# luvk1412/RoaringBitmap

Hardware: AMD Instinct MI355X
Metric: wide-OR/pairwise-AND input GB/s + % of HBM peak at 1/2/4/8 MI355X (higher is better)
Workload: dtype u64; 1 GPU; C2: RoaringBitmap.and(x1, x2), two full 2^32-universe bitmaps of 65536 mixed array/bitmap/run containers each (configs[1]); per_rank=the whole pair, parallelism=key-range sharding over 1 GPU(s)

## Files before the change

roaringbitmap_amd/csrc/engine.cpp:

```cpp
#include <hip/hip_runtime.h>

#include <algorithm>
#include <atomic>
#include <cstdio>
#include <cstdlib>
#include <cstring>
#include <initializer_list>
#include <memory>
#include <mutex>
#include <string>
#include <thread>
#include <chrono>
#include <unordered_map>
#include <vector>

#include <sys/mman.h>

#include "engine.hpp"
#include "format.hpp"

namespace rbg {

static thread_local std::string g_err;
void set_err(const std::string& s) { g_err = s; }

static bool debug_sync() {
  static int v = -1;
  if (v < 0) {
    const char* e = std::getenv("RBG_DEBUG_SYNC");
    v = (e && e[0] == '1') ? 1 : 0;
  }
  return v == 1;
}
void dbg(hipStream_t s, const char* what) {
  if (!debug_sync()) return;
  static auto last = std::chrono::steady_clock::now();
  hipError_t e = hipStreamSynchronize(s);
  const auto now = std::chrono::steady_clock::now();
  std::fprintf(stderr, "[rbg] %s done: %s (+%.3f ms)\n", what, hipGetErrorString(e),
               std::chrono::duration<double, std::milli>(now - last).count());
  last = now;
  std::fflush(stderr);
}

static size_t ro_flags_off(size_t groups) { return (64 + 32 * groups + 255) & ~(size_t)255; }

static std::mutex g_ctx_mu;
static std::vector<Ctx*> g_ctxs;

Ctx::~Ctx() {
  {
    std::lock_guard<std::mutex> g(g_ctx_mu);
    g_ctxs.erase(std::remove(g_ctxs.begin(), g_ctxs.end(), this), g_ctxs.end());
  }
  prof_free();
  if (pinned) (void)hipHostFree(pinned);
  batches.clear();
  if (stream) (void)hipStreamDestroy(stream);
}

size_t pool_clear(Ctx* c) {
  std::lock_guard<std::mutex> g(c->pool_mu);
  const size_t n = c->pool.size();
  c->pool.clear();
  c->pool_bytes = 0;
  return n;
}

static thread_local Ctx* t_cur_ctx = nullptr;
static std::atomic<uint64_t> g_pool_evictions{0};

static size_t release_pools_on(int device, int stage) {
  std::lock_guard<std::mutex> g(g_ctx_mu);
  size_t n = 0;
  const bool own = t_cur_ctx && std::find(g_ctxs.begin(), g_ctxs.end(), t_cur_ctx) != g_ctxs.end();
  if (stage == 0) {
    if (own && t_cur_ctx->device == device) n = pool_clear(t_cur_ctx);
  } else {
    for (Ctx* c : g_ctxs)
      if (c->device == device && !(own && c == t_cur_ctx)) n += pool_clear(c);
  }
  g_pool_evictions += n;
  return n;
}

int DevBuf::ensure(size_t bytes) {
  if (cap >= bytes && p) return RBG_OK;
  if (p) (void)hipFree(p);
  p = nullptr;
  cap = 0;
  hipError_t e = hipMalloc(&p, bytes + kSlack);
  if (e == hipErrorOutOfMemory) {
    int dev = 0;
    (void)hipGetLastError();
    for (int stage = 0; stage < 2 && e == hipErrorOutOfMemory; stage++) {
      if (hipGetDevice(&dev) != hipSuccess) break;
      if (release_pools_on(dev, stage) > 0) {
        e = hipMalloc(&p, bytes + kSlack);
        if (e == hipErrorOutOfMemory) (void)hipGetLastError();
      }
    }
  }
  if (e != hipSuccess) {
    p = nullptr;
    set_err(std::string("hipMalloc(") + std::to_string(bytes) + ") failed: " + hipGetErrorString(e));
    return e == hipErrorOutOfMemory ? RBG_ERR_OUT_OF_MEMORY : RBG_ERR_DEVICE;
  }
  cap = bytes;
  return RBG_OK;
}

int enter(Ctx* c) {
  t_cur_ctx = c;
  HIPCHK(hipSetDevice(c->device));
  return RBG_OK;
}

int ctx_init(Ctx* c, int device) {
  int n = 0;
  HIPCHK(hipGetDeviceCount(&n));
  if (device < 0 || device >= n) {
    set_err("no HIP device " + std::to_string(device));
    return RBG_ERR_DEVICE;
  }
  HIPCHK(hipSetDevice(device));
  hipDeviceProp_t prop;
  HIPCHK(hipGetDeviceProperties(&prop, device));
  if (std::strncmp(prop.gcnArchName, "gfx950", 6) != 0) {
    set_err(std::string("engine is built for gfx950, device is ") + prop.gcnArchName);
    return RBG_ERR_DEVICE;
  }
  c->device = device;
  {
    std::lock_guard<std::mutex> g(g_ctx_mu);
    g_ctxs.push_back(c);
  }
  HIPCHK(hipStreamCreateWithFlags(&c->stream, hipStreamNonBlocking));
  CHK(c->by_key.ensure(sizeof(PTask) * kMaxKeys));
  CHK(c->flag.ensure(kMaxKeys));
  CHK(c->tasks.ensure(sizeof(PTask) * (kMaxKeys + 32768)));
  CHK(c->ntasks.ensure(64));
  CHK(c->wg_count.ensure(4 * 256));
  CHK(c->wg_epoch.ensure(8 * 256));
  HIPCHK(hipMemset(c->wg_epoch.p, 0, 8 * 256));
  CHK(c->lb.ensure(kLbHeader + 8 * (kMaxKeys + 2 * kMaxTiles + kMaxAggTiles)));
  CHK(c->recs.ensure(sizeof(ORec) * kMaxKeys));
  CHK(c->kind_by_out.ensure(kMaxKeys));
  CHK(c->scalar.ensure(64));
  CHK(c->info.ensure(sizeof(ResultInfo)));
  CHK(c->task_card.ensure(4 * kMaxKeys));
  return RBG_OK;
}

int pinned_ensure(Ctx* c, size_t bytes) {
  if (c->pinned_cap >= bytes) return RBG_OK;
  if (c->pinned) (void)hipHostFree(c->pinned);
  c->pinned = nullptr;
  c->pinned_cap = 0;
  HIPCHK(hipHostMalloc(&c->pinned, bytes, hipHostMallocDefault));
  c->pinned_cap = bytes;
  return RBG_OK;
}

static uint32_t next_epoch(Ctx* c) {
  if (++c->epoch == 0) ++c->epoch;
  return c->epoch;
}
static PlanOut plan_out(Ctx* c, bool compacts = true) {
  return PlanOut{c->wg_epoch.as<uint64_t>(), compacts ? next_epoch(c) : 0, c->tasks.as<PTask>(),
                 c->ntasks.as<uint32_t>(), c->zlb, c->ztile};
}

int find_batch(Ctx* c, int32_t id, Batch** out) {
  if (id < 0 || (size_t)id >= c->batches.size() || !c->batches[id] || !c->batches[id]->live) {
    set_err("invalid batch id " + std::to_string(id));
    return RBG_ERR_ILLEGAL_ARGUMENT;
  }
  *out = c->batches[id].get();
  return RBG_OK;
}

static int ensure_stats(Ctx* c, Batch* b) {
  if (!b->stats_pending) return RBG_OK;
  const size_t n = b->n_bm, g = b->ro_groups, foff = ro_flags_off(g);
  uint32_t* flags = reinterpret_cast<uint32_t*>(b->ro_stats.as<uint8_t>() + foff);
  if (n) {
    HIPCHK(hipMemsetAsync(flags, 0, 4 * n, c->stream));
    launch_runopt_flags(c->stream, b->desc.as<CDesc>(), b->bm.as<uint32_t>(), b->n_ctr, flags);
  }
  std::vector<unsigned long long> hs(8 + 4 * g);
  std::vector<uint32_t> hf(n);
  HIPCHK(hipMemcpyAsync(hs.data(), b->ro_stats.p, 8 * hs.size(), hipMemcpyDeviceToHost, c->stream));
  if (n) HIPCHK(hipMemcpyAsync(hf.data(), flags, 4 * n, hipMemcpyDeviceToHost, c->stream));
  HIPCHK(hipStreamSynchronize(c->stream));
  b->stats_pending = false;
  unsigned long long h[4] = {0, 0, 0, 0};
  for (size_t w = 0; w < g; w++)
    for (int k = 0; k < 4; k++) h[k] += hs[8 + 4 * w + k];
  for (int k = 0; k < 3; k++) b->n_kind[k] = (int64_t)h[k];
  int64_t ser = (int64_t)h[3];
  b->h_has_run.assign(n, 0);
  for (size_t i = 0; i < n; i++) {
    const size_t nc = b->h_bm_nctr.empty() ? 0 : b->h_bm_nctr[i];
    ser += (int64_t)header_size(nc, hf[i] != 0);
    b->h_has_run[i] = hf[i] != 0;
  }
  if (b->ser_bytes) b->ser_bytes = ser;
  return RBG_OK;
}

int get_batch(Ctx* c, int32_t id, Batch** out) {
  CHK(find_batch(c, id, out));
  return ensure_stats(c, *out);
}

int32_t new_batch(Ctx* c) {
  for (size_t i = 0; i < c->batches.size(); i++)
    if (!c->batches[i]) {
      c->batches[i].reset(new Batch());
      return (int32_t)i;
    }
  c->batches.emplace_back(new Batch());
  return (int32_t)(c->batches.size() - 1);
}

constexpr size_t kPoolMax = 2ull << 30;
constexpr size_t kPoolMaxBuf = 1ull << 30;

void pool_put(Ctx* c, DevBuf& b) {
  if (!b.p) return;
  std::lock_guard<std::mutex> g(c->pool_mu);
  if (b.cap > kPoolMaxBuf) {
    b = DevBuf();
    return;
  }
  while (!c->pool.empty() && c->pool_bytes + b.cap > kPoolMax) {
    c->pool_bytes -= c->pool.front().cap;
    c->pool.erase(c->pool.begin());
  }
  c->pool_bytes += b.cap;
  c->pool.push_back(std::move(b));
}

int pool_take(Ctx* c, DevBuf& dst, size_t bytes) {
  if (dst.p && dst.cap >= bytes) return RBG_OK;
  std::unique_lock<std::mutex> lk(c->pool_mu);
  size_t best = c->pool.size();
  for (size_t i = 0; i < c->pool.size(); i++) {
    const size_t cap = c->pool[i].cap;
    if (cap >= bytes && cap <= 2 * bytes + (1u << 20) && (best == c->pool.size() || cap < c->pool[best].cap))
      best = i;
  }
  if (best == c->pool.size()) {
    lk.unlock();
    return dst.ensure(bytes);
  }
  c->pool_bytes -= c->pool[best].cap;
  dst = std::move(c->pool[best]);
  c->pool.erase(c->pool.begin() + (std::ptrdiff_t)best);
  return RBG_OK;
}

static uint64_t header_reserve(size_t max_tasks) {
  return round16(8 + (max_tasks + 7) / 8 + 8 * (uint64_t)max_tasks + 16);
}

int grid_for(size_t tasks, size_t cap) {
  size_t g = std::min(tasks, cap);
  return (int)std::max<size_t>(g, 1);
}

int prepare_output(Ctx* c, size_t max_tasks, size_t max_payload, OutCtx* oc, bool card_only) {
  uint8_t* lb = c->lb.as<uint8_t>();
  *oc = OutCtx{};
  oc->err = reinterpret_cast<uint32_t*>(lb + 64);
  oc->status = reinterpret_cast<uint64_t*>(lb + kLbHeader);
  oc->tile_status = reinterpret_cast<uint64_t*>(lb + kLbHeader + 8 * kMaxKeys);
  oc->tile_card = reinterpret_cast<uint64_t*>(lb + kLbHeader + 8 * (kMaxKeys + kMaxTiles));
  oc->recs = c->recs.as<ORec>();
  c->serialized = false;
  c->place_pending = false;
  c->agg_ok = false;
  c->ri_valid = false;
  c->pending_ub = 0;
  c->zlb = c->ztile = nullptr;
  c->pending_src.clear();
  if (card_only) {
    c->zlb = reinterpret_cast<uint64_t*>(lb);
    return RBG_OK;
  }
  const uint64_t P0 = header_reserve(max_tasks);
  CHK(c->result.ensure(P0 + max_payload + 64));
  c->result_cap = P0 + max_payload;
  CHK(c->scratch.ensure((size_t)kSlotBytes * std::max<size_t>(max_tasks, 1) + 64));
  c->zlb = reinterpret_cast<uint64_t*>(lb);
  c->ztile = reinterpret_cast<uint64_t*>(lb + kLbHeader + 8 * kMaxKeys);
  oc->out = c->result.as<uint8_t>();
  oc->payload_base = P0;
  oc->scratch = c->scratch.as<uint8_t>();
  oc->kind_by_out = c->kind_by_out.as<uint8_t>();
  c->pending = *oc;
  c->pending_ub = max_tasks;
  return RBG_OK;
}

void defer_place(Ctx* c) {
  c->place_pending = true;
  c->last = 1;
}
int ensure_placed(Ctx* c) {
  if (!c->place_pending) return RBG_OK;
  launch_place(c->stream, c->ntasks.as<uint32_t>(), c->pending, c->info.as<ResultInfo>());
  HIPCHK(hipGetLastError());
  c->place_pending = false;
  return RBG_OK;
}

int ctx_serialize(Ctx* c) {
  if (c->last != 1) {
    set_err("no materialised result pending");
    return RBG_ERR_ILLEGAL_ARGUMENT;
  }
  if (c->serialized) return RBG_OK;
  if (c->place_pending && c->agg_ok && !c->pending.spec && c->pending_ub <= (size_t)kMaxAggTiles * kAggTile) {
    launch_serialize_agg(c->stream, c->ntasks.as<uint32_t>(), c->pending, c->info.as<ResultInfo>(), c->pending_ub);
    HIPCHK(hipGetLastError());
    c->place_pending = false;
    c->serialized = true;
    return RBG_OK;
  }
  CHK(ensure_placed(c));
  if (c->pending.spec) launch_spec_fix(c->stream, c->ntasks.as<uint32_t>(), c->pending);
  launch_serialize(c->stream, c->ntasks.as<uint32_t>(), c->pending);
  HIPCHK(hipGetLastError());
  c->serialized = true;
  return RBG_OK;
}

int resolve(Ctx* c, int32_t id, size_t i, Operand* op) {
  Batch* b;
  CHK(get_batch(c, id, &b));
  if (i >= b->n_bm) {
    set_err("bitmap index out of range");
    return RBG_ERR_ILLEGAL_ARGUMENT;
  }
  if (b->n_bm != 1 || !b->key_major || b->packed) {
    set_err("pairwise operands must be single-bitmap key-major batches with slot-aligned payloads");
    return RBG_ERR_ILLEGAL_ARGUMENT;
  }
  *op = Operand{{b->key_off.as<uint32_t>(), b->desc.as<CDesc>(), b->payload.as<uint8_t>(), (int)b->n_ctr}, b};
  return RBG_OK;
}

static void op_begin(Ctx* c, std::initializer_list<int32_t> src) {
  c->pending_src = src;
  c->mark(0);
  c->mark(1);
}
int op_end(Ctx* c) {
  c->mark(2);
  defer_place(c);
  c->mark(3);
  HIPCHK(hipGetLastError());
  return RBG_OK;
}

static int ctx_rankdir(Ctx* c, Batch* b) {
  if (b->rd_ready) return RBG_OK;
  const size_t n = b->n_ctr;
  hipStream_t s = c->stream;
  CHK(pool_take(c, b->rd_cum, 8 * (n + 1)));
  CHK(pool_take(c, b->rd_off, 8 * (n + 1)));
  CHK(c->rd_part.ensure(8 * (scan_parts(std::max<uint64_t>(n, 1)) + 1)));
  uint64_t* cum = b->rd_cum.as<uint64_t>();
  uint64_t* off = b->rd_off.as<uint64_t>();
  launch_rd_sizes(s, b->desc.as<CDesc>(), b->payload.as<uint8_t>(), n, cum, off);
  launch_exclusive_scan(s, cum, cum, n, c->rd_part.as<uint64_t>(), cum + n);
  launch_exclusive_scan(s, off, off, n, c->rd_part.as<uint64_t>(), off + n);
  HIPCHK(hipGetLastError());
  uint64_t aux_bytes = 0;
  HIPCHK(hipMemcpyAsync(&aux_bytes, off + n, 8, hipMemcpyDeviceToHost, s));
  HIPCHK(hipStreamSynchronize(s));
  CHK(pool_take(c, b->rd_aux, aux_bytes + 16));
  launch_rd_fill(s, b->desc.as<CDesc>(), b->payload.as<uint8_t>(), n, off, b->rd_aux.as<uint8_t>());
  HIPCHK(hipGetLastError());
  b->rd_ready = true;
  return RBG_OK;
}

int ctx_point(Ctx* c, int op, int32_t batch, size_t i, const uint32_t* q_dev, size_t n, long long* out_dev) {
  Operand o;
  CHK(resolve(c, batch, i, &o));
  Batch* B = o.b;
  CHK(ctx_rankdir(c, B));
  const PointArgs pa{B->key_off.as<uint32_t>(), o.desc, B->payload.as<uint8_t>(), B->rd_cum.as<uint64_t>(),
                     B->rd_off.as<uint64_t>(), B->rd_aux.as<uint8_t>(), (uint32_t)o.n};
  launch_point(c->stream, op, pa, q_dev, n, out_dev);
  HIPCHK(hipGetLastError());
  return RBG_OK;
}

int ctx_point_host(Ctx* c, int op, int32_t batch, size_t i, const uint32_t* q, size_t n, int64_t* out) {
  CHK(pinned_ensure(c, 12 * n + 64));
  CHK(c->pt_q.ensure(4 * n));
  CHK(c->pt_out.ensure(8 * n));
  uint8_t* pin = reinterpret_cast<uint8_t*>(c->pinned);
  hipStream_t s = c->stream;
  HIPCHK(hipStreamSynchronize(s));
  std::memcpy(pin + 8 * n, q, 4 * n);
  HIPCHK(hipMemcpyAsync(c->pt_q.p, pin + 8 * n, 4 * n, hipMemcpyHostToDevice, s));
  CHK(ctx_point(c, op, batch, i, c->pt_q.as<uint32_t>(), n, c->pt_out.as<long long>()));
  HIPCHK(hipMemcpyAsync(pin, c->pt_out.p, 8 * n, hipMemcpyDeviceToHost, s));
  HIPCHK(hipStreamSynchronize(s));
  std::memcpy(out, pin, 8 * n);
  return RBG_OK;
}

int ctx_to_values(Ctx* c, int32_t batch, size_t i, uint64_t first, uint64_t count, bool out64, void* out_dev,
                  uint64_t* n_out) {
  Operand o;
  CHK(resolve(c, batch, i, &o));
  Batch* B = o.b;
  const uint64_t card = (uint64_t)B->long_card;
  const uint64_t cnt = first < card ? std::min<uint64_t>(count, card - first) : 0;
  if (n_out) *n_out = cnt;
  if (!cnt || (!out_dev && n_out)) return RBG_OK;
  if (!out_dev) {
    set_err("to_values: no output buffer");
    return RBG_ERR_ILLEGAL_ARGUMENT;
  }
  CHK(ctx_rankdir(c, B));
  const PointArgs pa{B->key_off.as<uint32_t>(), o.desc, B->payload.as<uint8_t>(), B->rd_cum.as<uint64_t>(),
                     B->rd_off.as<uint64_t>(), B->rd_aux.as<uint8_t>(), (uint32_t)o.n};
  launch_to_values(c->stream, pa, first, cnt, out64, out_dev);
  HIPCHK(hipGetLastError());
  return RBG_OK;
}

// ... 158 lines not shown
  if (layout != RBG_BITS_PACKED && layout != RBG_BITS_BYTES) {
    set_err("bitset: unknown layout (RBG_BITS_PACKED or RBG_BITS_BYTES)");
    return RBG_ERR_ILLEGAL_ARGUMENT;
  }
  if (layout == RBG_BITS_PACKED && (first & 63)) {
    set_err("bitset: a packed window starts at a multiple of 64");
    return RBG_ERR_ILLEGAL_ARGUMENT;
  }
  if (first > kBitsetMaxBits || n > kBitsetMaxBits - first) {
    set_err("bitset: the window reaches past 2^32");
    return RBG_ERR_ILLEGAL_ARGUMENT;
  }
  return RBG_OK;
}

int ctx_from_bitset(Ctx* c, const void* bits_dev, uint64_t n, int layout, bool run_opt, int32_t* out_id) {
  if (!n) return build_batch(c, nullptr, 0, nullptr, 0, run_opt, out_id);
  if (layout == RBG_BITS_PACKED)
    return build_batch(c, nullptr, 0, reinterpret_cast<const uint8_t*>(bits_dev), n, run_opt, out_id);
  const uint64_t nbytes = 8 * ((n + 63) / 64);
  DevBuf words;
  CHK(pool_take(c, words, nbytes + 16));
  launch_bits_pack(c->stream, reinterpret_cast<const uint8_t*>(bits_dev), n, words.as<uint64_t>());
  HIPCHK(hipGetLastError());
  const int st = build_batch(c, nullptr, 0, words.as<uint8_t>(), nbytes, run_opt, out_id);
  pool_put(c, words);
  return st;
}

int ctx_from_bitset_host(Ctx* c, const void* bits, uint64_t n, int layout, bool run_opt, int32_t* out_id) {
  DevBuf in;
  CHK(pool_take(c, in, n + 16));
  CHK(upload_bytes(c, in.p, bits, n));
  const int st = ctx_from_bitset(c, in.p, n, layout, run_opt, out_id);
  pool_put(c, in);
  return st;
}

int ctx_to_bitset(Ctx* c, int32_t batch, size_t i, uint64_t first, uint64_t n, int layout, void* out_dev) {
  Operand o;
  CHK(resolve(c, batch, i, &o));
  if (!n) return RBG_OK;
  if (!out_dev || (layout == RBG_BITS_PACKED && (reinterpret_cast<uintptr_t>(out_dev) & 7))) {
    set_err("bitset: no output buffer, or packed words not 8-byte aligned");
    return RBG_ERR_ILLEGAL_ARGUMENT;
  }
  launch_bits_expand(c->stream, o.key_off, o.desc, o.payload, first, n, layout == RBG_BITS_BYTES, out_dev);
  HIPCHK(hipGetLastError());
  return RBG_OK;
}

int ctx_to_bitset_host(Ctx* c, int32_t batch, size_t i, uint64_t first, uint64_t n, int layout, void* out) {
  CHK(ctx_to_bitset(c, batch, i, first, 0, layout, nullptr));
  if (!n) return RBG_OK;
  if (!out) {
    set_err("bitset: no output buffer");
    return RBG_ERR_ILLEGAL_ARGUMENT;
  }
  const bool mask = layout == RBG_BITS_BYTES;
  const uint64_t window = mask ? 1ull << 28 : 1ull << 31;
  auto bytes_of = [&](uint64_t bits) { return mask ? bits : 8 * ((bits + 63) / 64); };
  CHK(c->tv_out.ensure(bytes_of(std::min(n, window))));
  for (uint64_t done = 0; done < n; done += window) {
    const uint64_t w = std::min(window, n - done);
    CHK(ctx_to_bitset(c, batch, i, first + done, w, layout, c->tv_out.p));
    HIPCHK(hipMemcpyAsync(reinterpret_cast<uint8_t*>(out) + bytes_of(done), c->tv_out.p, bytes_of(w),
                          hipMemcpyDeviceToHost, c->stream));
    HIPCHK(hipStreamSynchronize(c->stream));
  }
  return RBG_OK;
}

static int ctx_pairwise_buffer(Ctx* c, int op, int32_t ia, size_t ma, int32_t ib, size_t mb, int key_lo, int key_hi) {
  key_lo = std::max(0, key_lo);
  key_hi = std::min(kMaxKeys, key_hi);
  Operand A, B;
  CHK(resolve(c, ia, ma, &A));
  CHK(resolve(c, ib, mb, &B));
  hipStream_t s = c->stream;
  const size_t ub = std::max<size_t>(1, op == OP_AND ? (size_t)std::min(A.n, B.n) : (size_t)A.n);
  return with_big_runs(c, true, "buffer and / andNot", [&](const BigRuns& big) -> int {
    OutCtx oc;
    CHK(prepare_output(c, ub, A.b->payload_bytes + B.b->payload_bytes + kStagedMax * ub + big.cap, &oc, false));
    c->pending_src = {ia, ib};
    c->mark(0);
    const PlanOut po = plan_out(c);
    launch_plan_pairwise(s, op, key_lo, key_hi, A, B, po, oc.err);
    c->mark(1);
    launch_pair_buf(s, op, grid_for(ub, 65536), po.tasks, po.n_tasks, A.payload, B.payload, oc, big);
    return op_end(c);
  });
}

int ctx_ornot(Ctx* c, int32_t ia, size_t ma, int32_t ib, size_t mb, int64_t range_end, int flags) {
  if (range_end < 0 || range_end > (int64_t)0x100000000ll) {
    set_err("rangeEnd should be in [0, 0xffffffff + 1]");
    return RBG_ERR_ILLEGAL_ARGUMENT;
  }
  Operand A, B;
  CHK(resolve(c, ia, ma, &A));
  CHK(resolve(c, ib, mb, &B));
  const int max_key = range_end == 0 ? -1 : (int)((range_end - 1) >> 16);
  const int last_run = (range_end & 0xFFFF) == 0 ? 0x10000 : (int)(range_end & 0xFFFF);
  hipStream_t s = c->stream;
  const size_t ub = std::max<size_t>(1, std::min<size_t>(kMaxKeys, (size_t)(max_key + 1) + (size_t)A.n));
  if (!c->ornot_plan.p) CHK(c->ornot_plan.ensure(sizeof(OrNotPlan)));
  OutCtx oc;
  CHK(prepare_output(c, ub, A.b->payload_bytes + B.b->payload_bytes + kStagedMax * ub, &oc, false));
  op_begin(c, {ia, ib});
  launch_ornot(s, A, B, max_key, last_run, flags, c->ornot_plan.as<OrNotPlan>(), plan_out(c), oc,
               grid_for(ub, 65536));
  CHK(op_end(c));
  if (max_key < 0 && A.n == 0 && B.n > 0) {
    OrNotPlan pl;
    HIPCHK(hipMemcpyAsync(&pl, c->ornot_plan.p, sizeof(pl), hipMemcpyDeviceToHost, s));
    HIPCHK(hipStreamSynchronize(s));
    if (pl.neg) {
      c->last = 0;
      set_err("orNot: negative maxSize (the reference throws NegativeArraySizeException)");
      return RBG_ERR_ILLEGAL_ARGUMENT;
    }
  }
  return RBG_OK;
}

int check_range(int64_t start, int64_t end) {
  if (start < 0 || start > 0xFFFFFFFFll || end < 0 || end > 0x100000000ll) {
    set_err("rangeStart=" + std::to_string(start) + " should be in [0, 0xffffffff], rangeEnd=" + std::to_string(end) +
            " in [0, 0xffffffff + 1]");
    return RBG_ERR_ILLEGAL_ARGUMENT;
  }
  return RBG_OK;
}

static int run_rmut(Ctx* c, int32_t ia, const Operand& A, RmutArgs ra, bool buf, size_t ub, bool use_arena,
                    const char* what) {
  return with_big_runs(c, use_arena, what, [&](const BigRuns& big) -> int {
    OutCtx oc;
    CHK(prepare_output(c, ub, A.b->payload_bytes + kStagedMax * ub + big.cap, &oc, false));
    op_begin(c, {ia});
    launch_rmut(c->stream, A, ra, buf, plan_out(c), oc, big, grid_for(ub, 65536));
    return op_end(c);
  });
}

int ctx_range_mut(Ctx* c, int op, int32_t ia, size_t ma, int64_t start, int64_t end, bool buf) {
  if (op < RMUT_ADD || (op > RMUT_ADD_INPLACE && op != RMUT_RANGE)) return RBG_ERR_ILLEGAL_ARGUMENT;
  CHK(check_range(start, end));
  Operand A;
  CHK(resolve(c, ia, ma, &A));
  RmutArgs ra{op, 1, 0, 0, 0};
  if (end > start) {
    ra.hbs = (int)((uint64_t)start >> 16 & 0xFFFF);
    ra.lbs = (int)(start & 0xFFFF);
    ra.hbl = (int)((uint64_t)(end - 1) >> 16 & 0xFFFF);
    ra.lbl = (int)((end - 1) & 0xFFFF);
  }
  const size_t in_range = end > start ? (size_t)(ra.hbl - ra.hbs + 1) : 0;
  const size_t ub = std::max<size_t>(1, std::min<size_t>(kMaxKeys, (size_t)A.n + in_range));
  return run_rmut(c, ia, A, ra, buf, ub, true, "range add / remove");
}

int ctx_remove_run_compression(Ctx* c, int32_t ia, size_t ma) {
  Operand A;
  CHK(resolve(c, ia, ma, &A));
  return run_rmut(c, ia, A, RmutArgs{RMUT_DERUN, 1, 0, 0, 0}, false, std::max<size_t>(1, (size_t)A.n), false,
                  "removeRunCompression");
}

int ctx_limit(Ctx* c, int32_t ia, size_t ma, int cut_key, int leftover) {
  Operand A;
  CHK(resolve(c, ia, ma, &A));
  return run_rmut(c, ia, A, RmutArgs{RMUT_LIMIT, cut_key, leftover, 0, 0}, false, std::max<size_t>(1, (size_t)A.n),
                  true, "limit");
}

int ctx_add_offset(Ctx* c, int32_t ia, size_t ma, int64_t offset) {
  Operand A;
  CHK(resolve(c, ia, ma, &A));
  const int64_t co = offset < 0 ? (offset - 65535) / 65536 : offset / 65536;
  AoffArgs aa{0, 0, 1};
  if (co >= -65536 && co < 65536) aa = AoffArgs{(int)co, (int)(offset - co * 65536), 0};
  const size_t ub = std::max<size_t>(1, std::min<size_t>(kMaxKeys, 2 * (size_t)A.n));
  OutCtx oc;
  CHK(prepare_output(c, ub, A.b->payload_bytes + kStagedMax * ub, &oc, false));
  op_begin(c, {ia});
  launch_aoff(c->stream, A, aa, plan_out(c), oc, grid_for(ub, 65536));
  return op_end(c);
}

int ctx_pairwise(Ctx* c, int op, int32_t ia, size_t ma, int32_t ib, size_t mb, bool card_only, int key_lo,
                 int key_hi) {
  if (op == RBG_AND_BUFFER || op == RBG_ANDNOT_BUFFER) {
    if (card_only) return RBG_ERR_ILLEGAL_ARGUMENT;
    return ctx_pairwise_buffer(c, op == RBG_AND_BUFFER ? OP_AND : OP_ANDNOT, ia, ma, ib, mb, key_lo, key_hi);
  }
  if (op == RBG_OR_INPLACE && !card_only) {
    CHK(ctx_pairwise(c, OP_OR, ia, ma, ib, mb, false, key_lo, key_hi));
    if (!c->ones.p) {
      CHK(c->ones.ensure(8192));
      HIPCHK(hipMemsetAsync(c->ones.p, 0xFF, 8192, c->stream));
    }
    Operand A, B;
    CHK(resolve(c, ia, ma, &A));
    CHK(resolve(c, ib, mb, &B));
    launch_ior_fix(c->stream, c->ntasks.as<uint32_t>(), c->recs.as<ORec>(), A, B, c->ones.as<uint8_t>());
    HIPCHK(hipGetLastError());
    c->agg_ok = false;
    return RBG_OK;
  }
  if (op < 0 || op > 3) return RBG_ERR_ILLEGAL_ARGUMENT;
  key_lo = std::max(0, key_lo);
  key_hi = std::min(kMaxKeys, key_hi);
  Operand A, B;
  CHK(resolve(c, ia, ma, &A));
  CHK(resolve(c, ib, mb, &B));
  hipStream_t s = c->stream;
  const int plan_op = card_only ? OP_AND : op;
  size_t ub;
  switch (plan_op) {
    case OP_AND: ub = std::min(A.n, B.n); break;
    case OP_ANDNOT: ub = A.n; break;
    default: ub = std::min<size_t>((size_t)A.n + B.n, kMaxKeys); break;
  }
  const size_t nkeys = key_hi > key_lo ? (size_t)(key_hi - key_lo) : 0;
  const bool dense = nkeys > 0 && 2 * ub >= nkeys;
  OutCtx oc;
  CHK(prepare_output(c, dense ? std::max(ub, nkeys) : ub, A.b->payload_bytes + B.b->payload_bytes + kStagedMax * ub,
                     &oc, card_only));
  c->pending_src = {ia, ib};
  c->mark(0);
  const PwDirect pd{key_lo};
  const PlanOut po = plan_out(c, !dense);
  if (dense) {
    launch_plan_balanced(s, plan_op, card_only ? 1 : 0, key_lo, (uint32_t)nkeys, A, B, po, oc,
                         c->task_card.as<uint32_t>());
  } else {
    launch_plan_pairwise(s, plan_op, key_lo, key_hi, A, B, po, oc.err);
    dbg(s, "plan");
  }
  c->mark(1);
  if (!card_only) {
    oc.tile_agg = reinterpret_cast<unsigned long long*>(oc.tile_status + 2 * kMaxTiles);
    c->pending.tile_agg = oc.tile_agg;
    c->agg_ok = true;
  }
  const int grid = grid_for(((dense ? nkeys : ub) + 3) / 4, 16384);
  launch_pairwise(s, op, card_only ? 1 : 0, grid, po.tasks, po.n_tasks, A.payload, B.payload, oc,
                  c->task_card.as<uint32_t>(), dense ? &pd : nullptr);
  dbg(s, "pairwise");
  c->mark(2);
  if (card_only) {
    launch_reduce_card(s, c->task_card.as<uint32_t>(), c->ntasks.as<uint32_t>(), c->info.as<ResultInfo>(), oc.err);
    c->last = 2;
  } else {
    defer_place(c);
  }
  c->mark(3);
  HIPCHK(hipGetLastError());
  return RBG_OK;
}


int batch_host_index(Ctx* c, Batch* b) {
  if (b->h_index) return RBG_OK;
  HIPCHK(hipStreamSynchronize(c->stream));
  b->h_desc.resize(b->n_ctr);
  if (b->n_ctr) HIPCHK(hipMemcpy(b->h_desc.data(), b->desc.p, sizeof(CDesc) * b->n_ctr, hipMemcpyDeviceToHost));
  b->h_pos_off.assign(b->n_bm + 1, 0);
  b->h_pos.resize(b->n_ctr);
  if ((b->n_bm == 1 || !b->key_major) && b->h_bm_off.size() == b->n_bm + 1) {
    for (size_t i = 0; i <= b->n_bm; i++) b->h_pos_off[i] = b->h_bm_off[i];
    for (size_t p = 0; p < b->n_ctr; p++) b->h_pos[p] = (uint32_t)p;
  } else {
    std::vector<uint32_t> bm(b->n_ctr);
    if (b->n_ctr) HIPCHK(hipMemcpy(bm.data(), b->bm.p, 4 * b->n_ctr, hipMemcpyDeviceToHost));
    for (uint32_t x : bm) b->h_pos_off[x + 1]++;
    for (size_t i = 0; i < b->n_bm; i++) b->h_pos_off[i + 1] += b->h_pos_off[i];
    std::vector<uint32_t> fill(b->h_pos_off.begin(), b->h_pos_off.end() - 1);
    for (size_t p = 0; p < b->n_ctr; p++) b->h_pos[fill[bm[p]]++] = (uint32_t)p;
  }
  b->h_index = true;
  return RBG_OK;
}

int ctx_info(Ctx* c, ResultInfo* ri) {
  if (c->last == 1) CHK(ensure_placed(c));
  HIPCHK(hipMemcpyAsync(ri, c->info.p, sizeof(ResultInfo), hipMemcpyDeviceToHost, c->stream));
  uint64_t card = 0;
  uint32_t err = 0;
  if (c->last == 1)
    HIPCHK(hipMemcpyAsync(&card, c->lb.as<uint8_t>() + 64 + 8 * kCardWord, 8, hipMemcpyDeviceToHost, c->stream));
  if (c->last == 1 || c->last == 2)
    HIPCHK(hipMemcpyAsync(&err, c->lb.as<uint8_t>() + 64, 4, hipMemcpyDeviceToHost, c->stream));
  HIPCHK(hipStreamSynchronize(c->stream));
  if (c->last == 1) {
    ri->long_card = (int64_t)card;
    ri->card32 = (uint32_t)card;
  }
  ri->err |= err;
  if ((c->last == 1 || c->last == 2) && ri->err) {
    set_err("a look-back spin of the op's plan or placement timed out: the result is invalid");
    return RBG_ERR_DEVICE;
  }
  if (c->last == 1) {
    c->last_ri = *ri;
    c->ri_valid = true;
  }
  return RBG_OK;
}

static int download_staged(Ctx* c, const uint8_t* dev, uint64_t bytes, uint8_t* dst) {
  constexpr uint64_t kGroup = 32ull << 20;
  hipStream_t s = c->stream;
  if (bytes <= kGroup) {
    HIPCHK(hipMemcpyAsync(dst, dev, bytes, hipMemcpyDeviceToHost, s));
    HIPCHK(hipStreamSynchronize(s));
    return RBG_OK;
  }
  CHK(pinned_ensure(c, bytes + 64));
  uint8_t* pin = reinterpret_cast<uint8_t*>(c->pinned);
  const uint32_t groups = (uint32_t)((bytes + kGroup - 1) / kGroup);
  std::vector<hipEvent_t> ev(groups);
  for (auto& e : ev) HIPCHK(hipEventCreateWithFlags(&e, hipEventDisableTiming));
  int st = RBG_OK;
  for (uint32_t g = 0; g < groups; g++) {
    const uint64_t lo = (uint64_t)g * kGroup, hi = std::min<uint64_t>(bytes, lo + kGroup);
    if (hipMemcpyAsync(pin + lo, dev + lo, hi - lo, hipMemcpyDeviceToHost, s) != hipSuccess ||
        hipEventRecord(ev[g], s) != hipSuccess) {
      set_err("device-to-host copy of the result failed");
      st = RBG_ERR_DEVICE;
      break;
    }
  }
  if (st == RBG_OK) {
    std::atomic<uint32_t> next{0};
    std::atomic<int> bad{0};
    const int nthr = (int)std::min<unsigned>(8, std::max(1u, std::thread::hardware_concurrency()));
    std::vector<std::thread> th;
    for (int t = 0; t < nthr; t++)
      th.emplace_back([&]() {
        for (uint32_t g; (g = next.fetch_add(1)) < groups;) {
          if (hipEventSynchronize(ev[g]) != hipSuccess) {
            bad.store(1);
            continue;
          }
          const uint64_t lo = (uint64_t)g * kGroup, hi = std::min<uint64_t>(bytes, lo + kGroup);
          std::memcpy(dst + lo, pin + lo, hi - lo);
        }
      });
    for (auto& x : th) x.join();
    if (bad.load()) {
      set_err("device-to-host copy of the result failed");
      st = RBG_ERR_DEVICE;
    }
  }
  (void)hipStreamSynchronize(s);
  for (auto& e : ev) (void)hipEventDestroy(e);
  return st;
}

static std::mutex g_out_mu;
static std::unordered_map<void*, size_t> g_out_live;
static std::vector<std::pair<void*, size_t>> g_out_cache;
constexpr size_t kOutLarge = 8ull << 20, kOutCacheMax = 2, kOutCacheBytes = 1ull << 30, kOutAlign = 2ull << 20;
static size_t out_cache_bytes() {
  size_t b = 0;
  for (const auto& e : g_out_cache) b += e.second;
  return b;
}
uint8_t* out_alloc(size_t n) {
  if (n < kOutLarge) return (uint8_t*)std::malloc(n ? n : 1);
  std::lock_guard<std::mutex> g(g_out_mu);
  for (size_t i = 0; i < g_out_cache.size(); i++) {
    const auto e = g_out_cache[i];
    if (e.second >= n && e.second <= 2 * n + kOutAlign) {
      g_out_cache.erase(g_out_cache.begin() + (std::ptrdiff_t)i);
      g_out_live[e.first] = e.second;
      return (uint8_t*)e.first;
    }
  }
  const size_t cap = (n + kOutAlign - 1) & ~(kOutAlign - 1);
  void* p = nullptr;
  if (posix_memalign(&p, kOutAlign, cap) != 0) return nullptr;
  (void)madvise(p, cap, MADV_HUGEPAGE);
  g_out_live[p] = cap;
  return (uint8_t*)p;
}

int ctx_fetch(Ctx* c, rbg_buffer* out) {
  if (c->last != 1) {
    set_err("no serialized result pending");
    return RBG_ERR_ILLEGAL_ARGUMENT;
  }
  CHK(ctx_serialize(c));
  ResultInfo ri;
  CHK(ctx_info(c, &ri));
  uint8_t* p = out_alloc(ri.total);
  if (!p) return RBG_ERR_OUT_OF_MEMORY;
  out->data = p;
  out->len = ri.total;
  const int st = download_staged(c, c->result.as<uint8_t>() + ri.start, ri.total, p);
  if (st != RBG_OK) {
    rbg_free(out);
    return st;
  }
  return RBG_OK;
}

int ctx_batch_fetch_range(Ctx* c, int32_t batch, size_t i0, size_t i1, rbg_buffer* outs) {
  Batch* b;
  CHK(get_batch(c, batch, &b));
  if (i0 > i1 || i1 > b->n_bm || (i1 > i0 && !outs)) return RBG_ERR_ILLEGAL_ARGUMENT;
  CHK(batch_host_index(c, b));
  const std::vector<CDesc>& D = b->h_desc;
  auto slot_end = [&](uint32_t p) -> uint64_t { return p + 1 < b->n_ctr ? D[p + 1].slot : b->payload_bytes; };
  std::vector<GatherItem> items;
  uint64_t tot = 0;
  for (size_t i = i0; i < i1; i++)
    for (uint32_t k = b->h_pos_off[i]; k < b->h_pos_off[i + 1]; k++) {
      const uint32_t p = b->h_pos[k];
      const uint64_t len = slot_end(p) - D[p].slot;
      items.push_back(GatherItem{D[p].slot, tot, len});
      tot = round16(tot + len);
    }
  std::vector<uint8_t> pay(tot + 16);
  if (!items.empty()) {
    CHK(c->gather_items.ensure(sizeof(GatherItem) * items.size()));
    CHK(c->gather_out.ensure(tot + 16));
    HIPCHK(hipMemcpyAsync(c->gather_items.p, items.data(), sizeof(GatherItem) * items.size(), hipMemcpyHostToDevice,
                          c->stream));
    launch_gather(c->stream, c->gather_items.as<GatherItem>(), items.size(), b->payload.as<uint8_t>(),
                  c->gather_out.as<uint8_t>());
    HIPCHK(hipGetLastError());
    HIPCHK(hipMemcpyAsync(pay.data(), c->gather_out.p, tot, hipMemcpyDeviceToHost, c->stream));
    HIPCHK(hipStreamSynchronize(c->stream));
  }
  size_t it = 0;
  for (size_t i = i0; i < i1; i++) {
    const uint32_t k0 = b->h_pos_off[i], n = b->h_pos_off[i + 1] - k0;
    bool has_run = false;
    std::vector<uint32_t> lens(n);
    for (uint32_t k = 0; k < n; k++) {
      const CDesc& d = D[b->h_pos[k0 + k]];
      has_run |= d.kind == KR;
      if (d.kind == KA) lens[k] = 2 * d.card;
      else if (d.kind == KB) lens[k] = 8192;
      else {
        const uint8_t* q = pay.data() + items[it + k].dst + 2;
        lens[k] = 2 + 4 * (uint32_t)(q[0] | (q[1] << 8));
      }
    }
    std::vector<uint8_t> o;
    auto put16 = [&](uint32_t v) { o.push_back((uint8_t)v); o.push_back((uint8_t)(v >> 8)); };
    auto put32 = [&](uint32_t v) { for (int j = 0; j < 4; j++) o.push_back((uint8_t)(v >> (8 * j))); };
    if (has_run) {
      put32(12347u | (uint32_t)((n - 1) << 16));
      std::vector<uint8_t> fl((n + 7) / 8, 0);
      for (uint32_t k = 0; k < n; k++)
        if (D[b->h_pos[k0 + k]].kind == KR) fl[k / 8] |= (uint8_t)(1u << (k % 8));
      o.insert(o.end(), fl.begin(), fl.end());
    } else {
      put32(12346u);
      put32(n);
    }
    for (uint32_t k = 0; k < n; k++) {
      const CDesc& d = D[b->h_pos[k0 + k]];
      put16(d.key);
      put16(d.card - 1);
    }
    if (!has_run || n >= 4) {
      uint32_t start = (uint32_t)header_size(n, has_run);
      for (uint32_t k = 0; k < n; k++) {
        put32(start);
        start += lens[k];
      }
    }
    for (uint32_t k = 0; k < n; k++) {
      const uint8_t* q = pay.data() + items[it + k].dst + (D[b->h_pos[k0 + k]].kind == KR ? 2 : 0);
      o.insert(o.end(), q, q + lens[k]);
    }
    it += n;
    const int st = emit_host(o, &outs[i - i0]);
    if (st != RBG_OK) {
      for (size_t j = i0; j < i; j++) rbg_free(&outs[j - i0]);
      return st;
    }
  }
  return RBG_OK;
}

int ctx_batch_card(Ctx* c, int32_t id) {
  Batch* B;
  CHK(get_batch(c, id, &B));
  if (B->packed) {
    set_err("batched andCardinality needs slot-aligned payloads");
    return RBG_ERR_ILLEGAL_ARGUMENT;
  }
  if (B->n_bm % 2 != 0) {
    set_err("batched andCardinality needs an even number of bitmaps");
    return RBG_ERR_ILLEGAL_ARGUMENT;
  }
  const size_t np = B->n_bm / 2;
  CHK(c->cards.ensure(4 * std::max<size_t>(np, 1)));
  if (B->key_major && B->n_bm > 1) {
    set_err("batched andCardinality needs a bitmap-major batch");
    return RBG_ERR_ILLEGAL_ARGUMENT;
  }
  c->mark(0);
  c->mark(1);
  if (!B->pair_cap_known) {
    B->pair_items_cap = batch_pair_items_cap(B->h_bm_nctr.data(), np);
    B->pair_cap_known = true;
  }
  CHK(c->pc_cnt.ensure(8 * ((np + 255) / 256) + std::max<size_t>(np, 1) + 16));
  CHK(c->pc_part.ensure(8 * (scan_parts(std::max<size_t>(np, 1)) + 1)));
  CHK(c->pc_items.ensure(sizeof(PairItem) * std::max<uint64_t>(B->pair_items_cap, 1)));
  CHK(c->pc_large.ensure(4 * std::max<size_t>(np, 1)));
  CHK(c->scalar.ensure(64));
  launch_batch_and_card(c->stream, np, B->bm_off.as<uint32_t>(), B->keys.as<uint16_t>(), B->desc.as<CDesc>(),
                        B->payload.as<uint8_t>(), c->cards.as<int32_t>(), c->pc_cnt.as<uint64_t>(),
                        c->pc_part.as<uint64_t>(), c->scalar.as<uint64_t>() + 7, c->pc_items.as<PairItem>(),
                        c->pc_large.as<uint32_t>());
  c->mark(2);
  c->mark(3);
  HIPCHK(hipGetLastError());
  c->n_cards = np;
  c->last = 3;
  return RBG_OK;
}

int ctx_fetch_shard_device(Ctx* c, int64_t total_containers, int has_run, int64_t payload_base, void* desc_dst,
                           void* offsets_dst, void* runflag_dst, void* payload_dst) {
  if (c->last != 1) {
    set_err("no materialised result pending");
    return RBG_ERR_ILLEGAL_ARGUMENT;
  }
  if (total_containers < 0 || total_containers > kMaxKeys || payload_base < 0 || !desc_dst || !payload_dst) {
    set_err("fetch_shard: bad layout or null destination");
    return RBG_ERR_ILLEGAL_ARGUMENT;
  }
  const bool offsets = !has_run || total_containers >= 4;
  if (offsets && !offsets_dst) {
    set_err("fetch_shard: the global bitmap has an offset table; offsets_dst is required");
    return RBG_ERR_ILLEGAL_ARGUMENT;
  }
  ResultInfo ri;
  if (c->ri_valid) {
    ri = c->last_ri;
    CHK(ensure_placed(c));
  } else {
    CHK(ctx_info(c, &ri));
  }
  const uint64_t off0 = header_size((size_t)total_containers, has_run != 0) + (uint64_t)payload_base;
  if (off0 > 0xFFFFFFFFull) {
    set_err("fetch_shard: payload offsets exceed 32 bits");
    return RBG_ERR_ILLEGAL_ARGUMENT;
  }
  uint8_t* emit_dst = (uint8_t*)payload_dst;
  if (c->serialized) {
    if (ri.payload)
      HIPCHK(hipMemcpyAsync(payload_dst, c->result.as<uint8_t>() + c->pending.payload_base, ri.payload,
                            hipMemcpyDeviceToDevice, c->stream));
    emit_dst = nullptr;
  }
  launch_serialize_shard(c->stream, grid_for((c->pending_ub + 255) / 256, 256), c->ntasks.as<uint32_t>(), c->pending,
                         emit_dst, off0, (uint8_t*)desc_dst, offsets ? (uint8_t*)offsets_dst : nullptr,
                         has_run ? (uint8_t*)runflag_dst : nullptr);
  HIPCHK(hipGetLastError());
  return RBG_OK;
}


int ctx_run_optimize(Ctx* c, int32_t id, int32_t* out_id, uint8_t* answers) {
  Batch* a;
  CHK(get_batch(c, id, &a));
  if (a->packed) {
    set_err("runOptimize needs slot-aligned payloads (not a packed synthetic batch)");
    return RBG_ERR_ILLEGAL_ARGUMENT;
  }
  hipStream_t s = c->stream;
  const size_t C = a->n_ctr, n = a->n_bm;
  const int32_t bid = new_batch(c);
  Batch& b = *c->batches[bid];
  struct Drop {
    Ctx* c;
    int32_t id;
    bool keep = false;
    ~Drop() {
      if (!keep) c->batches[id].reset();
    }
  } drop{c, bid};
  CHK(pool_take(c, b.desc, sizeof(CDesc) * C + 16));
  CHK(pool_take(c, b.payload, a->payload_bytes + 64));
  b.ro_groups = runopt_groups(C);
  CHK(pool_take(c, b.ro_stats, ro_flags_off(b.ro_groups) + 4 * n + 16));
  CHK(pool_take(c, b.keys, a->keys.cap));
  CHK(pool_take(c, b.bm, a->bm.cap));
  CHK(pool_take(c, b.key_off, a->key_off.cap));
  CHK(pool_take(c, b.bm_off, a->bm_off.cap));
  const RoCopy cp{a->keys.as<uint16_t>(), b.keys.as<uint16_t>(), a->bm.as<uint32_t>(), b.bm.as<uint32_t>(),
                  a->key_off.as<uint32_t>(), b.key_off.as<uint32_t>(), a->key_off.cap / 4,
                  a->bm_off.as<uint32_t>(), b.bm_off.as<uint32_t>(), a->bm_off.cap / 4};
  if (C)
    launch_runopt(s, a->desc.as<CDesc>(), a->payload.as<uint8_t>(), C, b.desc.as<CDesc>(), b.payload.as<uint8_t>(), cp,
                  b.ro_stats.as<unsigned long long>() + 8);
  HIPCHK(hipGetLastError());
  b.n_bm = n;
  b.n_ctr = C;
  b.key_major = a->key_major;
  b.h_bm_off = a->h_bm_off;
  b.h_bm_nctr = a->h_bm_nctr;
  b.h_bm_card = a->h_bm_card;
  b.long_card = a->long_card;
  b.bsi_min = a->bsi_min;
  b.bsi_max = a->bsi_max;
  b.payload_bytes = a->payload_bytes;
  b.gapped = a->gapped || a->n_kind[DK_R] > 0;
  b.max_ser = 0;
  b.ser_bytes = a->ser_bytes ? 1 : 0;
  b.stats_pending = true;
  b.live = true;
  drop.keep = true;
  *out_id = bid;
  if (answers) {
    CHK(ensure_stats(c, &b));
    for (size_t i = 0; i < n; i++) answers[i] = b.h_has_run[i];
  }
  return RBG_OK;
}

int ctx_select_range(Ctx* c, int32_t id, int64_t start, int64_t end, int32_t* out_id, bool buf) {
  if (start < 0 || end < 0) {
    set_err("selectRange: rangeStart and rangeEnd must not be negative");
    return RBG_ERR_ILLEGAL_ARGUMENT;
  }
  if (end > start && ((uint64_t)start >> 16 & 0xFFFF) > ((uint64_t)(end - 1) >> 16 & 0xFFFF)) {
    set_err("selectRange: the range's key casts are out of order (the reference would build an unsorted bitmap)");
    return RBG_ERR_ILLEGAL_ARGUMENT;
  }
  Batch* a;
  CHK(get_batch(c, id, &a));
  if (!a->key_major || a->packed) {
    set_err("range selection needs a key-major batch with slot-aligned payloads");
    return RBG_ERR_ILLEGAL_ARGUMENT;
  }
  hipStream_t s = c->stream;
  const size_t C = a->n_ctr, n = a->n_bm;
  RselArgs ra{1, 0, 0, 0, buf ? 1 : 0};
  if (end > start) {
    ra.hbs = (int)((uint64_t)start >> 16 & 0xFFFF);
    ra.lbs = (int)(start & 0xFFFF);
    ra.hbl = (int)((uint64_t)(end - 1) >> 16 & 0xFFFF);
    ra.lbl = (int)((end - 1) & 0xFFFF);
  }
  CHK(c->ro_info.ensure(4 * C + 16));
  CHK(c->ro_size.ensure(8 * C + 16));
  CHK(c->ro_part.ensure(8 * (scan_parts(std::max<size_t>(C, 1)) + 1)));
  CHK(c->rs_card.ensure(4 * C + 16));
  CHK(c->rs_keep.ensure(8 * C + 16));
  CHK(c->rs_bm.ensure(16 * n + 64 + 16));
  const int32_t bid = new_batch(c);
  Batch& b = *c->batches[bid];
  BatchGuard guard{c, {bid}};
  CHK(pool_take(c, b.desc, sizeof(CDesc) * C + 16));
  CHK(pool_take(c, b.payload, a->payload_bytes + 64));
  CHK(b.keys.ensure(2 * C + 16));
  CHK(b.bm.ensure(4 * C + 16));
  CHK(b.key_off.ensure(4 * (kMaxKeys + 1)));
  CHK(b.bm_off.ensure(4 * (n + 1)));
  unsigned long long* bm_cnt = c->rs_bm.as<unsigned long long>();
  unsigned long long* bm_card = bm_cnt + n;
  unsigned long long* tot = bm_cnt + 2 * n;
  HIPCHK(hipMemsetAsync(c->rs_bm.p, 0, 16 * n + 64, s));
  launch_rsel_plan(s, a->desc.as<CDesc>(), a->bm.as<uint32_t>(), a->payload.as<uint8_t>(), C, ra,
                   c->ro_info.as<uint32_t>(), c->rs_card.as<uint32_t>(), c->ro_size.as<uint64_t>(),
                   c->rs_keep.as<uint64_t>(), bm_cnt, bm_card, tot);
  launch_exclusive_scan(s, c->ro_size.as<uint64_t>(), c->ro_size.as<uint64_t>(), C, c->ro_part.as<uint64_t>(),
                        reinterpret_cast<uint64_t*>(tot + 4));
  launch_exclusive_scan(s, c->rs_keep.as<uint64_t>(), c->rs_keep.as<uint64_t>(), C, c->ro_part.as<uint64_t>(),
                        reinterpret_cast<uint64_t*>(tot + 5));
  launch_rsel_write(s, a->desc.as<CDesc>(), a->bm.as<uint32_t>(), a->payload.as<uint8_t>(), C, ra,
                    c->ro_info.as<uint32_t>(), c->rs_card.as<uint32_t>(), c->ro_size.as<uint64_t>(),
                    c->rs_keep.as<uint64_t>(), b.desc.as<CDesc>(), b.keys.as<uint16_t>(), b.bm.as<uint32_t>(),
                    b.payload.as<uint8_t>());
  HIPCHK(hipGetLastError());
  std::vector<unsigned long long> h(2 * n + 8);
  HIPCHK(hipMemcpyAsync(h.data(), c->rs_bm.p, 8 * (2 * n + 6), hipMemcpyDeviceToHost, s));
  HIPCHK(hipStreamSynchronize(s));
  const unsigned long long* t = h.data() + 2 * n;
  const uint64_t C2 = t[5];
  launch_dec_key_off(s, b.keys.as<uint16_t>(), C2, b.key_off.as<uint32_t>());
  b.n_bm = n;
  b.n_ctr = C2;
  b.key_major = true;
  for (int k = 0; k < 3; k++) b.n_kind[k] = (int64_t)t[k];
  b.max_ser = t[3];
  b.payload_bytes = t[4];
  b.h_bm_off.assign(n + 1, 0);
  b.h_bm_nctr.resize(n);
  b.h_bm_card.resize(n);
  for (size_t i = 0; i < n; i++) {
    b.h_bm_nctr[i] = (uint32_t)h[i];
    b.h_bm_off[i + 1] = b.h_bm_off[i] + (uint32_t)h[i];
    b.h_bm_card[i] = (int64_t)h[n + i];
    b.long_card += (int64_t)h[n + i];
  }
  HIPCHK(hipMemcpyAsync(b.bm_off.p, b.h_bm_off.data(), 4 * (n + 1), hipMemcpyHostToDevice, s));
  HIPCHK(hipStreamSynchronize(s));
  HIPCHK(hipGetLastError());
  b.live = true;
  guard.ids.clear();
  *out_id = bid;
  return RBG_OK;
}

int ctx_profile(Ctx* c, int max_ops, bool compute_only) {
  HIPCHK(hipStreamSynchronize(c->stream));
  c->prof_free();
  c->prof_compute_only = compute_only;
  if (max_ops <= 0) return RBG_OK;
  c->prof_ev.resize(4 * (size_t)max_ops);
  for (hipEvent_t& e : c->prof_ev) HIPCHK(hipEventCreate(&e));
  c->prof_cap = (size_t)max_ops;
  c->prof_n = 0;
  CHK(c->rd_ctr.ensure(8));
  HIPCHK(hipMemsetAsync(c->rd_ctr.p, 0, 8, c->stream));
  return RBG_OK;
}

static std::mutex g_dev_mu;
static uint64_t g_dev_mask = 1;

struct TLCtx {
  std::unique_ptr<Ctx> ctx;
  int device = -1;
};
static thread_local TLCtx tl;

int tl_ctx(Ctx** out) {
  int dev;
  {
    std::lock_guard<std::mutex> g(g_dev_mu);
    uint64_t m = g_dev_mask;
    dev = m ? __builtin_ctzll(m) : 0;
  }
  if (!tl.ctx || tl.device != dev) {
    std::unique_ptr<Ctx> c(new Ctx());
    CHK(ctx_init(c.get(), dev));
    tl.ctx = std::move(c);
    tl.device = dev;
  }
  CHK(enter(tl.ctx.get()));
  *out = tl.ctx.get();
  return RBG_OK;
}

}

using namespace rbg;

extern "C" {

void rbg_trim(void) {
  std::lock_guard<std::mutex> g(g_out_mu);
  for (const auto& e : g_out_cache) std::free(e.first);
  g_out_cache.clear();
}

uint64_t rbg_pool_evictions(void) { return g_pool_evictions.load(); }
const char* rbg_last_error(void) { return g_err.c_str(); }

void rbg_free(rbg_buffer* buf) {
  if (!buf) return;
  if (buf->data) {
    std::lock_guard<std::mutex> g(g_out_mu);
    const auto it = g_out_live.find(buf->data);
    if (it != g_out_live.end()) {
      g_out_cache.emplace_back(it->first, it->second);
      g_out_live.erase(it);
      while (g_out_cache.size() > kOutCacheMax || (!g_out_cache.empty() && out_cache_bytes() > kOutCacheBytes)) {
        std::free(g_out_cache.front().first);
        g_out_cache.erase(g_out_cache.begin());
      }
      buf->data = nullptr;
      buf->len = 0;
      return;
    }
  }
  std::free(buf->data);
  buf->data = nullptr;
  buf->len = 0;
}

int rbg_set_devices(uint64_t mask) {
  int n = 0;
  if (hipGetDeviceCount(&n) != hipSuccess || n == 0) {
    set_err("no HIP device");
    return RBG_ERR_DEVICE;
  }
  uint64_t usable = mask & ((n >= 64) ? ~0ULL : ((1ULL << n) - 1));
// ... 11 lines not shown
```

roaringbitmap_amd/csrc/engine.hpp:

```cpp
#pragma once
#include <hip/hip_runtime.h>

#include <cstddef>
#include <cstdint>
#include <cstdlib>
#include <cstring>
#include <memory>
#include <mutex>
#include <string>
#include <vector>

#include "../../include/roaring_mi355x.h"
#include "kernels.hpp"

namespace rbg {

void set_err(const std::string& s);

#define HIPCHK(x)                                                            \
  do {                                                                       \
    hipError_t e_ = (x);                                                     \
    if (e_ != hipSuccess) {                                                  \
      set_err(std::string(#x) + " failed: " + hipGetErrorString(e_));        \
      return e_ == hipErrorOutOfMemory ? RBG_ERR_OUT_OF_MEMORY : RBG_ERR_DEVICE; \
// ... 6 lines not shown
    if (st_ != RBG_OK) return st_; \
  } while (0)

constexpr size_t kSlack = 256;
constexpr int kMaxKeys = 65536;
constexpr size_t kLbHeader = 256;
constexpr size_t kStagedMax = 8194;

struct DevBuf {
  void* p = nullptr;
  size_t cap = 0;
  DevBuf() = default;
  DevBuf(const DevBuf&) = delete;
  DevBuf& operator=(const DevBuf&) = delete;
  DevBuf(DevBuf&& o) noexcept : p(o.p), cap(o.cap) {
    o.p = nullptr;
    o.cap = 0;
  }
  DevBuf& operator=(DevBuf&& o) noexcept {
    if (this != &o) {
      if (p) (void)hipFree(p);
      p = o.p;
      cap = o.cap;
      o.p = nullptr;
      o.cap = 0;
    }
    return *this;
  }
  ~DevBuf() {
    if (p) (void)hipFree(p);
  }
  int ensure(size_t bytes);
  template <class T>
  T* as() const {
    return reinterpret_cast<T*>(p);
  }
};

struct Batch {
  bool live = false;
  bool key_major = false;
  bool gapped = false;
  bool packed = false;
  size_t n_bm = 0, n_ctr = 0;
  DevBuf keys, desc, bm, key_off, bm_off, payload;
  size_t payload_bytes = 0;
  std::vector<uint32_t> h_bm_off;
  std::vector<uint32_t> h_bm_nctr;
  std::vector<int64_t> h_bm_card;
  int64_t n_kind[3] = {0, 0, 0};
  int64_t ser_bytes = 0;
  int64_t long_card = 0;
  size_t max_ser = 0;
  int32_t bsi_min = 0, bsi_max = 0;
  bool pair_cap_known = false;
  bool stats_pending = false;
  DevBuf ro_stats;
  size_t ro_groups = 0;
  std::vector<uint8_t> h_has_run;
  bool bsi_cached = false;
  DevBuf bsi_tasks, bsi_nt, bsi_table;
  bool rd_ready = false;
  DevBuf rd_cum, rd_off, rd_aux;
  uint64_t pair_items_cap = 0;
  bool h_index = false;
  bool h_chain_identity = false;
  std::vector<CDesc> h_desc;
  std::vector<uint32_t> h_pos, h_pos_off;
};

struct RangeIndex {
  uint32_t nslices = 0, n_blocks = 0;
  uint64_t max_rid = 0, mask = 0;
  uint64_t payload_bytes = 0;
  uint64_t arena_bytes = 0;
  DevBuf dir, masks, arena;
};

struct DecBufs {
  DevBuf meta, head, nctr, base, nch, chbase, chmap, flag, err, card, cons, part, q, qkey, sort, skey, iota, perm,
      size, cpart;
};

struct Ctx {
  int device = 0;
  DecBufs dec;
  DevBuf wg_epoch;
  uint32_t epoch = 0;
  DevBuf pc_cnt, pc_part, pc_items, pc_large;
  hipStream_t stream = nullptr;
  std::vector<std::unique_ptr<Batch>> batches;
  std::vector<std::unique_ptr<RangeIndex>> range_indexes;
  uint64_t* zlb = nullptr;
  uint64_t* ztile = nullptr;
  DevBuf bsi_defer, bsi_cnts, bsi_kin, bsi_table;
  DevBuf bsi_claims;
  DevBuf bsi_sums;
  void* bsi_sums_dst = nullptr;
  DevBuf owen_tb, owen_keys, owen_ord, big, big_ctl;
  DevBuf ones;
  DevBuf ornot_plan;
  DevBuf rd_part;
  DevBuf pt_q, pt_out;
  DevBuf bld_info, bld_size, bld_part;
  DevBuf tv_out;
  DevBuf bsib_pkeys, bsib_pkoff, bsib_info, bsib_size, bsib_part, bsib_per;
  DevBuf rbb_info, rbb_size, rbb_part;
  DevBuf bsia_run;
  DevBuf bsit_ckeys, bsit_ckoff, bsit_rflag, bsit_kcard, bsit_full;
  DevBuf bsiv_cards, bsiv_part;
  DevBuf gather_items, gather_out;
  DevBuf order;
  DevBuf ro_info, ro_size, ro_part;
  DevBuf rs_card, rs_keep, rs_bm;
  std::vector<DevBuf> pool;
  size_t pool_bytes = 0;
  std::mutex pool_mu;
  ResultInfo last_ri{};
  bool ri_valid = false;
  int bsi_nbits = 0;
  DevBuf by_key, flag, tasks, ntasks, wg_count, lb, recs, kind_by_out, info, task_card, result, cards, skip, raw,
      scalar, scratch;
  size_t result_cap = 0;
  OutCtx pending{};
  std::vector<int32_t> pending_src;
  size_t pending_ub = 0;
  bool serialized = false;
  bool place_pending = false;
  bool agg_ok = false;
  size_t n_cards = 0;
  int last = 0;
  void* pinned = nullptr;
  size_t pinned_cap = 0;
  std::vector<hipEvent_t> prof_ev;
  size_t prof_cap = 0, prof_n = 0;
  DevBuf rd_ctr;
  void prof_free() {
    for (hipEvent_t e : prof_ev) (void)hipEventDestroy(e);
    prof_ev.clear();
    prof_cap = prof_n = 0;
  }
  bool prof_compute_only = false;
  void mark(int phase) {
    if (prof_compute_only && (phase == 0 || phase == 3)) {
      if (phase == 3 && prof_n < prof_cap) prof_n++;
      return;
    }
    if (prof_n < prof_cap) (void)hipEventRecord(prof_ev[4 * prof_n + phase], stream);
    if (phase == 3 && prof_n < prof_cap) prof_n++;
  }
  ~Ctx();
};

struct BatchGuard {
  Ctx* c;
  std::vector<int32_t> ids;
  ~BatchGuard() {
    for (int32_t id : ids)
      if (id >= 0 && (size_t)id < c->batches.size()) c->batches[id].reset();
  }
};

static inline uint64_t round16(uint64_t x) { return (x + 15) & ~15ULL; }

void dbg(hipStream_t s, const char* what);
int ctx_init(Ctx* c, int device);
int enter(Ctx* c);
int tl_ctx(Ctx** out);
int find_batch(Ctx* c, int32_t id, Batch** out);
int get_batch(Ctx* c, int32_t id, Batch** out);
int32_t new_batch(Ctx* c);
int batch_host_index(Ctx* c, Batch* b);
void pool_put(Ctx* c, DevBuf& b);
int pool_take(Ctx* c, DevBuf& dst, size_t bytes);
size_t pool_clear(Ctx* c);
int pinned_ensure(Ctx* c, size_t bytes);
int upload_words(Ctx* c, void* dst, const void* src, size_t n);
int ctx_profile(Ctx* c, int max_ops, bool compute_only);
int prepare_output(Ctx* c, size_t max_tasks, size_t max_payload, OutCtx* oc, bool card_only);
void defer_place(Ctx* c);
int ensure_placed(Ctx* c);
int grid_for(size_t tasks, size_t cap = 4096);
int op_end(Ctx* c);
int ctx_serialize(Ctx* c);
int ctx_info(Ctx* c, ResultInfo* ri);
uint8_t* out_alloc(size_t n);
int ctx_fetch(Ctx* c, rbg_buffer* out);
int ctx_batch_fetch_range(Ctx* c, int32_t batch, size_t i0, size_t i1, rbg_buffer* outs);
int ctx_fetch_shard_device(Ctx* c, int64_t total_containers, int has_run, int64_t payload_base, void* desc_dst,
                           void* offsets_dst, void* runflag_dst, void* payload_dst);
struct Operand : BmView {
  Batch* b;
};
int resolve(Ctx* c, int32_t id, size_t i, Operand* op);
int ctx_empty_bitmap(Ctx* c, int32_t* out_id);
int ctx_point(Ctx* c, int op, int32_t batch, size_t i, const uint32_t* q_dev, size_t n, long long* out_dev);
int ctx_point_host(Ctx* c, int op, int32_t batch, size_t i, const uint32_t* q, size_t n, int64_t* out);
int ctx_to_values(Ctx* c, int32_t batch, size_t i, uint64_t first, uint64_t count, bool out64, void* out_dev,
                  uint64_t* n_out);
int ctx_to_values_host(Ctx* c, int32_t batch, size_t i, uint64_t first, uint64_t count, uint32_t* out,
                       uint64_t* n_out);
int ctx_from_values(Ctx* c, const uint32_t* v_dev, size_t n, bool run_opt, int32_t* out_id);
int ctx_from_values_host(Ctx* c, const uint32_t* v, size_t n, bool run_opt, int32_t* out_id);
int check_bitset_build(const void* bits, uint64_t n, int layout, bool device);
int check_bitset_window(uint64_t first, uint64_t n, int layout);
int ctx_from_bitset(Ctx* c, const void* bits_dev, uint64_t n, int layout, bool run_opt, int32_t* out_id);
int ctx_from_bitset_host(Ctx* c, const void* bits, uint64_t n, int layout, bool run_opt, int32_t* out_id);
int ctx_to_bitset(Ctx* c, int32_t batch, size_t i, uint64_t first, uint64_t n, int layout, void* out_dev);
int ctx_to_bitset_host(Ctx* c, int32_t batch, size_t i, uint64_t first, uint64_t n, int layout, void* out);
int ctx_pairwise(Ctx* c, int op, int32_t ia, size_t ma, int32_t ib, size_t mb, bool card_only, int key_lo = 0,
                 int key_hi = kMaxKeys);
int ctx_ornot(Ctx* c, int32_t ia, size_t ma, int32_t ib, size_t mb, int64_t range_end, int flags);
int check_range(int64_t start, int64_t end);
int ctx_range_mut(Ctx* c, int op, int32_t ia, size_t ma, int64_t start, int64_t end, bool buf);
int ctx_remove_run_compression(Ctx* c, int32_t ia, size_t ma);
int ctx_limit(Ctx* c, int32_t ia, size_t ma, int cut_key, int leftover);
int ctx_add_offset(Ctx* c, int32_t ia, size_t ma, int64_t offset);
int ctx_batch_card(Ctx* c, int32_t id);
int ctx_run_optimize(Ctx* c, int32_t id, int32_t* out_id, uint8_t* answers);
int ctx_select_range(Ctx* c, int32_t id, int64_t start, int64_t end, int32_t* out_id, bool buf = false);
int ctx_load_impl(Ctx* c, const uint8_t* const* bufs, const size_t* lens, size_t n, bool key_major, int32_t* out_id,
                  bool pack_arrays = false);
int ctx_load(Ctx* c, const uint8_t* const* bufs, const size_t* lens, size_t n, int32_t* out_id,
             bool pack_arrays = false);
int ctx_load_separate(Ctx* c, const uint8_t* const* bufs, const size_t* lens, size_t n, int32_t* ids);
bool wide_reads_packed(int op, size_t n);
int ctx_wide(Ctx* c, int op, int32_t id, int key_lo, int key_hi, const int32_t* ids, bool card_only,
             int* host_card_out, bool* host_card_valid, int32_t start_override = -1);
int check_rb_query(int op, bool has_ctx, bool count);
int ctx_rb_load(Ctx* c, const uint8_t* buf, size_t len, int32_t* out_index);
int check_rb_build(const void* values, uint64_t n, const void* out);
int ctx_rb_build(Ctx* c, const uint64_t* dev_values, uint64_t n, uint64_t max_value, bool max_from_data, int32_t* index);
int ctx_rb_build_host(Ctx* c, const uint64_t* values, uint64_t n, uint64_t max_value, bool max_from_data,
                      int32_t* index);
int ctx_rb_serialize(Ctx* c, int32_t index, rbg_buffer* out);
int ctx_rb_release(Ctx* c, int32_t index);
int ctx_rb_info(Ctx* c, int32_t index, uint64_t* info);
int ctx_rb_query(Ctx* c, int32_t index, int op, uint64_t a, uint64_t b, int32_t ctx_batch, size_t ctx_i,
                 int32_t* out_batch);
int ctx_rb_count(Ctx* c, int32_t index, int op, uint64_t a, uint64_t b, int32_t ctx_batch, size_t ctx_i, int64_t* out);
int synth_c2(Ctx* c, int kind, uint64_t seed, int32_t* out_id);
int synth_c3(Ctx* c, int kind, uint64_t seed, size_t n, int key_lo, int key_hi, int32_t* out_id);
int synth_c4(Ctx* c, uint64_t seed, size_t n_pairs, int32_t* out_id);
int synth_c5(Ctx* c, uint64_t seed, size_t rows, int key_lo, int key_hi, int32_t* out_id);

static int emit_bytes(const uint8_t* src, size_t n, rbg_buffer* out) {
  uint8_t* p = (uint8_t*)std::malloc(n ? n : 1);
  if (!p) return RBG_ERR_OUT_OF_MEMORY;
  if (n) std::memcpy(p, src, n);
  out->data = p;
  out->len = n;
  return RBG_OK;
}
static int emit_host(const std::vector<uint8_t>& v, rbg_buffer* out) { return emit_bytes(v.data(), v.size(), out); }

template <class Pass>
static int with_big_runs(Ctx* c, bool use_arena, const char* what, Pass&& pass) {
  if (!use_arena) return pass(BigRuns{nullptr, nullptr, 0});
  if (!c->big_ctl.p) CHK(c->big_ctl.ensure(16));
  if (!c->big.p) CHK(c->big.ensure(16ull << 20));
  for (int attempt = 0;; attempt++) {
    HIPCHK(hipMemsetAsync(c->big_ctl.p, 0, 16, c->stream));
    CHK(pass(BigRuns{c->big.as<uint8_t>(), c->big_ctl.as<unsigned long long>(), c->big.cap}));
    unsigned long long used[2] = {0, 0};
    HIPCHK(hipMemcpyAsync(used, c->big_ctl.p, 16, hipMemcpyDeviceToHost, c->stream));
    HIPCHK(hipStreamSynchronize(c->stream));
    if (!used[1]) return RBG_OK;
    if (attempt) {
      set_err(std::string(what) + ": the run-container arena overflowed twice");
      return RBG_ERR_DEVICE;
    }
    CHK(c->big.ensure(used[0] + (used[0] >> 3) + 4096));
  }
}

namespace {
struct HPtr {
  uint32_t bm, i, key, card, pos;
};
static int hcmp(const HPtr& x, const HPtr& y) {
  if (x.key != y.key) return (int)x.key - (int)y.key;
  return (int)y.card - (int)x.card;
}
struct JHeap {
  std::vector<HPtr> q;
  void add(const HPtr& x) {
    size_t k = q.size();
    q.push_back(x);
    while (k > 0) {
      const size_t p = (k - 1) >> 1;
      if (hcmp(x, q[p]) >= 0) break;
      q[k] = q[p];
      k = p;
    }
    q[k] = x;
  }
  HPtr poll() {
    const HPtr r = q[0];
    const HPtr x = q.back();
    q.pop_back();
    const size_t n = q.size();
    if (n) {
      size_t k = 0;
      const size_t half = n >> 1;
      while (k < half) {
        size_t ch = 2 * k + 1;
        if (ch + 1 < n && hcmp(q[ch], q[ch + 1]) > 0) ch++;
        if (hcmp(x, q[ch]) <= 0) break;
        q[k] = q[ch];
        k = ch;
      }
      q[k] = x;
    }
    return r;
  }
};
}

struct OneShot {
  Ctx* c = nullptr;
  BatchGuard g{nullptr, {}};
  int open() {
    CHK(tl_ctx(&c));
    g.c = c;
    return RBG_OK;
  }
  void adopt(int32_t id) { g.ids.push_back(id); }
  int load(const uint8_t* const* bufs, const size_t* lens, size_t n, int32_t* id, bool pack_arrays = false,
           bool key_major = true) {
    CHK(ctx_load_impl(c, bufs, lens, n, key_major, id, pack_arrays));
    adopt(*id);
    return RBG_OK;
  }
  int load_separate(const uint8_t* const* bufs, const size_t* lens, size_t n, int32_t* ids) {
    CHK(ctx_load_separate(c, bufs, lens, n, ids));
    g.ids.insert(g.ids.end(), ids, ids + n);
    return RBG_OK;
  }
};

}

struct __attribute__((visibility("hidden"))) rbg_ctx {
  rbg::Ctx c;
};

namespace rbg {
int session(rbg_ctx* ctx, Ctx** c);
}
```

roaringbitmap_amd/csrc/engine_api.cpp:

```cpp
#include <algorithm>

#include "engine.hpp"
#include "format.hpp"

namespace rbg {

static const uint8_t kEmpty[8] = {0x3A, 0x30, 0, 0, 0, 0, 0, 0};
static int emit_empty(rbg_buffer* out) { return emit_bytes(kEmpty, sizeof(kEmpty), out); }

static int ctx_batch_fetch(Ctx* c, int32_t batch, size_t i, rbg_buffer* out) {
  if (!out) return RBG_ERR_ILLEGAL_ARGUMENT;
  return ctx_batch_fetch_range(c, batch, i, i + 1, out);
}

static bool point_op_ok(int op) { return op >= RBG_PQ_RANK && op <= RBG_PQ_PREV; }

template <class Op>
static int one_shot_unary(const uint8_t* a, size_t a_len, rbg_buffer* out, Op&& op) {
  OneShot os;
  CHK(os.open());
  int32_t id;
  CHK(os.load_separate(&a, &a_len, 1, &id));
  CHK(op(os.c, id));
  return ctx_fetch(os.c, out);
}

template <class Op>
static int one_shot_binary(const uint8_t* a, size_t a_len, const uint8_t* b, size_t b_len, rbg_buffer* out, Op&& op) {
  OneShot os;
  CHK(os.open());
  const uint8_t* bufs[2] = {a, b};
  const size_t lens[2] = {a_len, b_len};
  int32_t ids[2];
  CHK(os.load_separate(bufs, lens, 2, ids));
  CHK(op(os.c, ids[0], ids[1]));
  return ctx_fetch(os.c, out);
}

}

using namespace rbg;

int rbg::session(rbg_ctx* ctx, Ctx** c) {
  if (!ctx) return RBG_ERR_ILLEGAL_ARGUMENT;
  *c = &ctx->c;
  return enter(*c);
}

extern "C" {

int rbg_version(void) { return 1; }

int rbg_pairwise(int op, const uint8_t* a, size_t a_len, const uint8_t* b, size_t b_len, rbg_buffer* out) {
  if (!out || op < 0 || op > RBG_ANDNOT_BUFFER) return RBG_ERR_ILLEGAL_ARGUMENT;
  return one_shot_binary(a, a_len, b, b_len, out, [&](Ctx* c, int32_t ia, int32_t ib) {
    return ctx_pairwise(c, op, ia, 0, ib, 0, false);
  });
}

int rbg_pairwise_inplace(int op, const uint8_t* a, size_t a_len, const uint8_t* b, size_t b_len, int same_object,
                         rbg_buffer* out) {
  if (!out || op < 0 || op > 3) return RBG_ERR_ILLEGAL_ARGUMENT;
  if (same_object) {
    if (op == RBG_XOR || op == RBG_ANDNOT) return emit_empty(out);
    HostBitmap hb;
    std::string err;
    const int st = parse(a, a_len, &hb, &err);
    if (st) {
      set_err(err);
      return st;
    }
    uint8_t* p = out_alloc(hb.consumed);
    if (!p) return RBG_ERR_OUT_OF_MEMORY;
    std::memcpy(p, a, hb.consumed);
    out->data = p;
    out->len = hb.consumed;
    return RBG_OK;
  }
  return rbg_pairwise(op == RBG_OR ? RBG_OR_INPLACE : op, a, a_len, b, b_len, out);
}

int rbg_ornot(const uint8_t* a, size_t a_len, const uint8_t* b, size_t b_len, int64_t range_end, int flags,
              rbg_buffer* out) {
  if (!out || flags < 0 || flags > 3) return RBG_ERR_ILLEGAL_ARGUMENT;
  return one_shot_binary(a, a_len, b, b_len, out, [&](Ctx* c, int32_t ia, int32_t ib) {
    return ctx_ornot(c, ia, 0, ib, 0, range_end, flags);
  });
}

int rbg_ctx_ornot(rbg_ctx* ctx, int32_t a, size_t ia, int32_t b, size_t ib, int64_t range_end, int flags) {
  Ctx* c;
  CHK(session(ctx, &c));
  if (flags < 0 || flags > 3) return RBG_ERR_ILLEGAL_ARGUMENT;
  return ctx_ornot(c, a, ia, b, ib, range_end, flags);
}

int rbg_range_mut(int op, const uint8_t* a, size_t a_len, int64_t range_start, int64_t range_end, rbg_buffer* out) {
  if (!out || op < 0 || op > (RBG_RMUT_ADD_INPLACE | RBG_RMUT_BUFFER))
    return RBG_ERR_ILLEGAL_ARGUMENT;
  return one_shot_unary(a, a_len, out, [&](Ctx* c, int32_t id) {
    return ctx_range_mut(c, op & 3, id, 0, range_start, range_end, (op & RBG_RMUT_BUFFER) != 0);
  });
}

int rbg_ctx_range_mut(rbg_ctx* ctx, int op, int32_t batch, size_t i, int64_t range_start, int64_t range_end) {
  Ctx* c;
  CHK(session(ctx, &c));
  if (op < 0 || op > (RBG_RMUT_ADD_INPLACE | RBG_RMUT_BUFFER)) return RBG_ERR_ILLEGAL_ARGUMENT;
  return ctx_range_mut(c, op & 3, batch, i, range_start, range_end, (op & RBG_RMUT_BUFFER) != 0);
}

int rbg_add_offset(const uint8_t* a, size_t a_len, int64_t offset, rbg_buffer* out) {
  if (!out) return RBG_ERR_ILLEGAL_ARGUMENT;
  return one_shot_unary(a, a_len, out, [&](Ctx* c, int32_t id) { return ctx_add_offset(c, id, 0, offset); });
}


int rbg_ctx_point_query(rbg_ctx* ctx, int op, int32_t batch, size_t i, const uint32_t* q, size_t n, int64_t* out) {
  Ctx* c;
  CHK(session(ctx, &c));
  if (!point_op_ok(op)) return RBG_ERR_ILLEGAL_ARGUMENT;
  if (n == 0) return RBG_OK;
  if (!q || !out) return RBG_ERR_ILLEGAL_ARGUMENT;
  return ctx_point_host(c, op, batch, i, q, n, out);
}

int rbg_ctx_point_query_device(rbg_ctx* ctx, int op, int32_t batch, size_t i, const void* q_dev, size_t n,
                               void* out_dev) {
  Ctx* c;
// ... 329 lines not shown
    lens[2 * i] = a_lens[i];
    bufs[2 * i + 1] = b_bufs[i];
    lens[2 * i + 1] = b_lens[i];
  }
  int32_t id;
  CHK(os.load(bufs.data(), lens.data(), 2 * n_pairs, &id, false, false));
  CHK(ctx_batch_card(c, id));
  HIPCHK(hipMemcpyAsync(out, c->cards.p, 4 * n_pairs, hipMemcpyDeviceToHost, c->stream));
  HIPCHK(hipStreamSynchronize(c->stream));
  return RBG_OK;
}


int rbg_from_values(const uint32_t* values, size_t n, int run_optimize, rbg_buffer* out) {
  if (!out || (n && !values)) return RBG_ERR_ILLEGAL_ARGUMENT;
  return emit_host(build_from_values(values, n, run_optimize != 0), out);
}

int rbg_run_optimize(const uint8_t* buf, size_t len, rbg_buffer* out) {
  if (!out || (!buf && len)) return RBG_ERR_ILLEGAL_ARGUMENT;
  uint8_t answer = 0;
  return rbg_run_optimize_many(&buf, &len, 1, out, &answer);
}

int rbg_to_values(const uint8_t* buf, size_t len, rbg_buffer* out) {
  if (!out) return RBG_ERR_ILLEGAL_ARGUMENT;
  std::vector<uint32_t> v;
  std::string err;
  int st = values_of_serialized(buf, len, &v, &err);
  if (st) {
    set_err(err);
    return st;
  }
  return emit_bytes(reinterpret_cast<const uint8_t*>(v.data()), v.size() * 4, out);
}

int rbg_inspect(const uint8_t* buf, size_t len, size_t* consumed, int64_t* cardinality, int64_t* stats3) {
  HostBitmap hb;
  std::string err;
  int st = parse(buf, len, &hb, &err);
  if (st) {
    set_err(err);
    return st;
  }
  if (consumed) *consumed = hb.consumed;
  if (cardinality) *cardinality = hb.card;
  if (stats3) {
    stats3[0] = stats3[1] = stats3[2] = 0;
    for (const HostCtr& c : hb.ctrs) stats3[c.kind]++;
  }
  return RBG_OK;
}

int rbg_ctx_create(int device, rbg_ctx** out) {
  if (!out) return RBG_ERR_ILLEGAL_ARGUMENT;
  std::unique_ptr<rbg_ctx> c(new rbg_ctx());
  CHK(ctx_init(&c->c, device));
  *out = c.release();
  return RBG_OK;
}
void rbg_ctx_destroy(rbg_ctx* ctx) {
  if (!ctx) return;
  (void)hipSetDevice(ctx->c.device);
  delete ctx;
}
void* rbg_ctx_stream(rbg_ctx* ctx) { return ctx ? (void*)ctx->c.stream : nullptr; }
int rbg_ctx_profile(rbg_ctx* ctx, int max_ops) {
  Ctx* c;
  CHK(session(ctx, &c));
  return ctx_profile(c, max_ops, false);
}
int rbg_ctx_profile_compute(rbg_ctx* ctx, int max_ops) {
  Ctx* c;
  CHK(session(ctx, &c));
  return ctx_profile(c, max_ops, true);
}
int rbg_ctx_profile_bytes(rbg_ctx* ctx, int64_t* bytes) {
  if (!ctx || !bytes) {
    set_err("profile_bytes: null argument");
    return RBG_ERR_ILLEGAL_ARGUMENT;
  }
  Ctx* c;
  CHK(session(ctx, &c));
  HIPCHK(hipStreamSynchronize(c->stream));
  unsigned long long v = 0;
  if (c->rd_ctr.p) HIPCHK(hipMemcpy(&v, c->rd_ctr.p, 8, hipMemcpyDeviceToHost));
  *bytes = (int64_t)v;
  return RBG_OK;
}
int rbg_ctx_profile_read(rbg_ctx* ctx, double* ms3, int* n_ops) {
  Ctx* c;
  CHK(session(ctx, &c));
  HIPCHK(hipStreamSynchronize(c->stream));
  ms3[0] = ms3[1] = ms3[2] = 0.0;
  for (size_t i = 0; i < c->prof_n; i++) {
    for (int ph = 0; ph < 3; ph++) {
      if (c->prof_compute_only && ph != 1) continue;
      float ms = 0.f;
      HIPCHK(hipEventElapsedTime(&ms, c->prof_ev[4 * i + ph], c->prof_ev[4 * i + ph + 1]));
      ms3[ph] += ms;
    }
  }
  *n_ops = (int)c->prof_n;
  c->prof_n = 0;
  return RBG_OK;
}
int rbg_ctx_sync(rbg_ctx* ctx) {
  Ctx* c;
  CHK(session(ctx, &c));
  HIPCHK(hipStreamSynchronize(c->stream));
  return RBG_OK;
}
int rbg_ctx_load_separate(rbg_ctx* ctx, const uint8_t* const* bufs, const size_t* lens, size_t n, int32_t* ids) {
  Ctx* c;
  CHK(session(ctx, &c));
  if (!ids) return RBG_ERR_ILLEGAL_ARGUMENT;
  return ctx_load_separate(c, bufs, lens, n, ids);
}
int rbg_ctx_load(rbg_ctx* ctx, const uint8_t* const* bufs, const size_t* lens, size_t n, int32_t* batch) {
  Ctx* c;
  CHK(session(ctx, &c));
  return ctx_load(c, bufs, lens, n, batch);
}
int rbg_ctx_load_packed(rbg_ctx* ctx, const uint8_t* const* bufs, const size_t* lens, size_t n, int32_t* batch) {
  Ctx* c;
  CHK(session(ctx, &c));
  if (!batch) return RBG_ERR_ILLEGAL_ARGUMENT;
  return ctx_load(c, bufs, lens, n, batch, true);
}
int rbg_ctx_release(rbg_ctx* ctx, int32_t batch) {
  if (!ctx) return RBG_ERR_ILLEGAL_ARGUMENT;
  Ctx& c = ctx->c;
  Batch* b;
  CHK(find_batch(&c, batch, &b));
  CHK(enter(&c));
  if (c.last == 1 && !c.serialized &&
      std::find(c.pending_src.begin(), c.pending_src.end(), batch) != c.pending_src.end())
    CHK(ctx_serialize(&c));
  for (DevBuf* d : {&b->keys, &b->desc, &b->bm, &b->key_off, &b->bm_off, &b->payload, &b->ro_stats,
                    &b->bsi_tasks, &b->bsi_nt, &b->bsi_table, &b->rd_cum, &b->rd_off, &b->rd_aux})
    pool_put(&c, *d);
  c.batches[batch].reset();
  return RBG_OK;
}
int rbg_ctx_batch_stats(rbg_ctx* ctx, int32_t batch, int64_t* st) {
  if (!ctx) return RBG_ERR_ILLEGAL_ARGUMENT;
  Batch* b;
  CHK(get_batch(&ctx->c, batch, &b));
  st[0] = (int64_t)b->n_bm;
  st[1] = (int64_t)b->n_ctr;
  st[2] = b->n_kind[0];
  st[3] = b->n_kind[1];
  st[4] = b->n_kind[2];
  st[5] = 0;
  st[6] = b->long_card;
  st[7] = b->ser_bytes;
  if (b->n_ctr) {
    CHK(enter(&ctx->c));
    hipStream_t s = ctx->c.stream;
    HIPCHK(hipMemsetAsync(ctx->c.scalar.p, 0, 8, s));
    launch_batch_bytes(s, b->desc.as<CDesc>(), b->n_ctr, b->payload.as<uint8_t>(),
                       ctx->c.scalar.as<unsigned long long>());
    unsigned long long pay = 0;
    HIPCHK(hipMemcpyAsync(&pay, ctx->c.scalar.p, 8, hipMemcpyDeviceToHost, s));
    HIPCHK(hipStreamSynchronize(s));
    st[5] = (int64_t)pay;
  }
  return RBG_OK;
}
int rbg_ctx_batch_fetch(rbg_ctx* ctx, int32_t batch, size_t i, rbg_buffer* out) {
  Ctx* c;
  CHK(session(ctx, &c));
  return ctx_batch_fetch(c, batch, i, out);
}
int rbg_ctx_batch_fetch_range(rbg_ctx* ctx, int32_t batch, size_t first, size_t count, rbg_buffer* outs) {
  Ctx* c;
  CHK(session(ctx, &c));
  return ctx_batch_fetch_range(c, batch, first, first + count, outs);
}
int rbg_ctx_pairwise(rbg_ctx* ctx, int op, int32_t a, size_t ia, int32_t b, size_t ib) {
  Ctx* c;
  CHK(session(ctx, &c));
  return ctx_pairwise(c, op, a, ia, b, ib, false);
}
int rbg_ctx_pairwise_serialized(rbg_ctx* ctx, int op, int32_t a, size_t ia, int32_t b, size_t ib) {
  Ctx* c;
  CHK(session(ctx, &c));
  if (op < 0 || op > 3) return RBG_ERR_ILLEGAL_ARGUMENT;
  CHK(ctx_pairwise(c, op, a, ia, b, ib, false));
  return ctx_serialize(c);
}
int rbg_ctx_pairwise_range(rbg_ctx* ctx, int op, int32_t a, size_t ia, int32_t b, size_t ib, int key_lo, int key_hi) {
  Ctx* c;
  CHK(session(ctx, &c));
  if (key_lo > key_hi) return RBG_ERR_ILLEGAL_ARGUMENT;
  return ctx_pairwise(c, op, a, ia, b, ib, false, key_lo, key_hi);
}
int rbg_ctx_pairwise_card(rbg_ctx* ctx, int op, int32_t a, size_t ia, int32_t b, size_t ib) {
  Ctx* c;
  CHK(session(ctx, &c));
  if (op != RBG_CARD_AND) {
    set_err("the session API computes andCardinality; derive the others from the input cardinalities");
    return RBG_ERR_ILLEGAL_ARGUMENT;
  }
  return ctx_pairwise(c, OP_AND, a, ia, b, ib, true);
}
int rbg_ctx_wide(rbg_ctx* ctx, int op, int32_t batch, int key_lo, int key_hi, const int32_t* ids) {
  Ctx* c;
  CHK(session(ctx, &c));
  return ctx_wide(c, op, batch, key_lo, key_hi, ids, false, nullptr, nullptr);
}
int rbg_ctx_wide_start(rbg_ctx* ctx, int op, int32_t batch, int key_lo, int key_hi, const int32_t* ids,
                       int32_t start_bm) {
  Ctx* c;
  CHK(session(ctx, &c));
  return ctx_wide(c, op, batch, key_lo, key_hi, ids, false, nullptr, nullptr, start_bm);
}
int rbg_ctx_batch_counts(rbg_ctx* ctx, int32_t batch, uint32_t* out, size_t n) {
  if (!ctx) return RBG_ERR_ILLEGAL_ARGUMENT;
  Batch* b;
  CHK(get_batch(&ctx->c, batch, &b));
  if (!out || n != b->n_bm) return RBG_ERR_ILLEGAL_ARGUMENT;
  for (size_t i = 0; i < n; i++) out[i] = b->h_bm_nctr[i];
  return RBG_OK;
}
int rbg_ctx_pair_bytes(rbg_ctx* ctx, int32_t batch, int64_t* out2) {
  if (!ctx) return RBG_ERR_ILLEGAL_ARGUMENT;
  Batch* b;
  CHK(get_batch(&ctx->c, batch, &b));
  if (!out2 || b->key_major || b->n_bm % 2) {
    set_err("needs a bitmap-major batch of pairs");
    return RBG_ERR_ILLEGAL_ARGUMENT;
  }
  CHK(enter(&ctx->c));
  HIPCHK(hipStreamSynchronize(ctx->c.stream));
  std::vector<CDesc> d(b->n_ctr);
  if (b->n_ctr) HIPCHK(hipMemcpy(d.data(), b->desc.p, sizeof(CDesc) * b->n_ctr, hipMemcpyDeviceToHost));
  auto pay = [](const CDesc& x) -> int64_t { return x.kind == KA ? 2 * (int64_t)x.card : x.kind == KB ? 8192 : 0; };
  int64_t matched = 0, all = 0;
  for (size_t p = 0; p < b->n_bm / 2; p++) {
    uint32_t i = b->h_bm_off[2 * p], ie = b->h_bm_off[2 * p + 1], j = ie, je = b->h_bm_off[2 * p + 2];
    all += 4 * (int64_t)(je - i);
    while (i < ie && j < je) {
      if (d[i].key == d[j].key) {
        matched += pay(d[i++]) + pay(d[j++]);
      } else if (d[i].key < d[j].key) {
        i++;
      } else {
        j++;
      }
    }
  }
  out2[0] = matched + all;
  int64_t tot = 0;
  for (const CDesc& x : d) tot += pay(x) + 4;
  out2[1] = tot;
  return RBG_OK;
}
int rbg_ctx_wide_card(rbg_ctx* ctx, int op, int32_t batch, int key_lo, int key_hi) {
  Ctx* c;
  CHK(session(ctx, &c));
  int hc;
  bool hv;
  CHK(ctx_wide(c, op, batch, key_lo, key_hi, nullptr, true, &hc, &hv));
  if (hv) {
    ResultInfo ri = {};
    ri.card32 = (uint32_t)hc;
    ri.long_card = hc;
    HIPCHK(hipMemcpyAsync(c->info.p, &ri, sizeof(ri), hipMemcpyHostToDevice, c->stream));
    HIPCHK(hipStreamSynchronize(c->stream));
  }
  return RBG_OK;
}
int rbg_ctx_batch_and_card(rbg_ctx* ctx, int32_t batch) {
  Ctx* c;
  CHK(session(ctx, &c));
  return ctx_batch_card(c, batch);
}
int rbg_ctx_card(rbg_ctx* ctx, int32_t* out) {
  Ctx* c;
  CHK(session(ctx, &c));
  ResultInfo ri;
  CHK(ctx_info(c, &ri));
  *out = (int32_t)ri.card32;
  return RBG_OK;
}
int rbg_ctx_cards(rbg_ctx* ctx, int32_t* out, size_t n) {
  Ctx* c;
  CHK(session(ctx, &c));
  if (n > c->n_cards) return RBG_ERR_ILLEGAL_ARGUMENT;
  HIPCHK(hipMemcpyAsync(out, c->cards.p, 4 * n, hipMemcpyDeviceToHost, c->stream));
  HIPCHK(hipStreamSynchronize(c->stream));
  return RBG_OK;
}
int rbg_ctx_result_stats(rbg_ctx* ctx, int64_t* st) {
  Ctx* c;
  CHK(session(ctx, &c));
  ResultInfo ri;
  CHK(ctx_info(c, &ri));
  st[0] = ri.n_out;
  st[1] = (int64_t)ri.payload;
  st[2] = ri.has_run;
  st[3] = ri.long_card;
  return RBG_OK;
}
int rbg_ctx_serialize(rbg_ctx* ctx) {
  Ctx* c;
  CHK(session(ctx, &c));
  return ctx_serialize(c);
}
int rbg_ctx_fetch(rbg_ctx* ctx, rbg_buffer* out) {
  Ctx* c;
  CHK(session(ctx, &c));
  return ctx_fetch(c, out);
}
int rbg_ctx_result_layout_device(rbg_ctx* ctx, void* dst3) {
  Ctx* c;
  CHK(session(ctx, &c));
  if (!dst3) return RBG_ERR_ILLEGAL_ARGUMENT;
  if (c->last != 1) {
    set_err("no materialised result pending");
    return RBG_ERR_ILLEGAL_ARGUMENT;
  }
  if (c->place_pending) {
    OutCtx o = c->pending;
    o.layout_out = reinterpret_cast<int64_t*>(dst3);
    launch_place(c->stream, c->ntasks.as<uint32_t>(), o, c->info.as<ResultInfo>());
    c->place_pending = false;
  } else {
    launch_layout_out(c->stream, c->info.as<ResultInfo>(), reinterpret_cast<int64_t*>(dst3));
  }
  HIPCHK(hipGetLastError());
  return RBG_OK;
}
int rbg_ctx_fetch_shard_device_dyn(rbg_ctx* ctx, const void* layout, int rank, int world, void* out, void* runb) {
  Ctx* c;
  CHK(session(ctx, &c));
  if (!layout || !out || world < 1 || world > 1024 || rank < 0 || rank >= world)
    return RBG_ERR_ILLEGAL_ARGUMENT;
  if (c->last != 1) {
    set_err("no materialised result pending");
    return RBG_ERR_ILLEGAL_ARGUMENT;
  }
  CHK(ensure_placed(c));
  if (c->serialized) {
    set_err("fetch_shard_device_dyn: the result was already serialized; fetch it before releasing operands "
            "or use rbg_ctx_fetch_shard_device");
    return RBG_ERR_ILLEGAL_ARGUMENT;
  }
  launch_serialize_shard_dyn(c->stream, grid_for((c->pending_ub + 255) / 256, 256), c->ntasks.as<uint32_t>(), c->pending,
                             reinterpret_cast<const int64_t*>(layout), rank, world, (uint8_t*)out, (uint8_t*)runb, true);
  HIPCHK(hipGetLastError());
  return RBG_OK;
}
int rbg_ctx_fetch_shard_device(rbg_ctx* ctx, int64_t total_containers, int has_run, int64_t payload_base,
                               void* desc_dst, void* offsets_dst, void* runflag_dst, void* payload_dst) {
  Ctx* c;
  CHK(session(ctx, &c));
  return ctx_fetch_shard_device(c, total_containers, has_run, payload_base, desc_dst, offsets_dst, runflag_dst,
                                payload_dst);
}

int rbg_ctx_fetch_shard(rbg_ctx* ctx, int64_t total_containers, int has_run, int64_t first_container,
                        int64_t payload_base, rbg_buffer* out_desc, rbg_buffer* out_offsets, rbg_buffer* out_payload) {
  Ctx* c;
  CHK(session(ctx, &c));
  if (!out_desc || !out_offsets || !out_payload) return RBG_ERR_ILLEGAL_ARGUMENT;
  (void)first_container;
  ResultInfo ri;
  CHK(ctx_info(c, &ri));
  const size_t n = ri.n_out;
  const bool offsets = !has_run || total_containers >= 4;
  DevBuf d;
  CHK(d.ensure(9 * n + ri.payload + 64));
  uint8_t* base = d.as<uint8_t>();
  CHK(ctx_fetch_shard_device(c, total_containers, has_run, payload_base, base, base + 4 * n, base + 8 * n,
                             base + 9 * n));
  std::vector<uint8_t> h(9 * n + ri.payload);
  if (!h.empty()) HIPCHK(hipMemcpyAsync(h.data(), base, h.size(), hipMemcpyDeviceToHost, c->stream));
  HIPCHK(hipStreamSynchronize(c->stream));
  CHK(emit_bytes(h.data(), 4 * n, out_desc));
  CHK(emit_bytes(h.data() + 4 * n, offsets ? 4 * n : 0, out_offsets));
  return emit_bytes(h.data() + 9 * n, ri.payload, out_payload);
}

int rbg_run_optimize_many(const uint8_t* const* bufs, const size_t* lens, size_t n, rbg_buffer* outs,
                          uint8_t* answers) {
  if (n && !outs) return RBG_ERR_ILLEGAL_ARGUMENT;
  OneShot os;
  CHK(os.open());
  Ctx* c = os.c;
  int32_t in = -1, opt = -1;
  CHK(os.load(bufs, lens, n, &in));
  CHK(ctx_run_optimize(c, in, &opt, answers));
  os.adopt(opt);
  for (size_t i = 0; i < n; i++) {
    outs[i] = rbg_buffer{};
    const int st = ctx_batch_fetch(c, opt, i, &outs[i]);
    if (st) {
      for (size_t j = 0; j < i; j++) rbg_free(&outs[j]);
      return st;
    }
  }
  return RBG_OK;
}

int rbg_ctx_run_optimize(rbg_ctx* ctx, int32_t batch, int32_t* out_batch, uint8_t* answers) {
  Ctx* c;
  CHK(session(ctx, &c));
  if (!out_batch) return RBG_ERR_ILLEGAL_ARGUMENT;
  return ctx_run_optimize(c, batch, out_batch, answers);
}

int rbg_ctx_batch_minmax(rbg_ctx* ctx, int32_t batch, int32_t* out2) {
  if (!ctx) return RBG_ERR_ILLEGAL_ARGUMENT;
  Batch* b;
  CHK(get_batch(&ctx->c, batch, &b));
  if (!out2) return RBG_ERR_ILLEGAL_ARGUMENT;
  out2[0] = b->bsi_min;
  out2[1] = b->bsi_max;
  return RBG_OK;
}

int rbg_ctx_synth(rbg_ctx* ctx, int kind, uint64_t seed, size_t n, int key_lo, int key_hi, int32_t* batch) {
  Ctx* c;
  CHK(session(ctx, &c));
  if (kind == 4) return synth_c5(c, seed, n, key_lo, key_hi, batch);
  if (kind == 1 || kind == 2) return synth_c3(c, kind, seed, n, key_lo, key_hi, batch);
  if (kind == 3) return synth_c4(c, seed, n, batch);
  if (kind == 0 || (kind >= 16 && kind <= 18)) return synth_c2(c, kind, seed, batch);
  set_err("synthetic kind not available");
  return RBG_ERR_ILLEGAL_ARGUMENT;
}
// ... 3 lines not shown
```

roaringbitmap_amd/csrc/engine_bsi.cpp:

```cpp
#include <algorithm>
#include <cstdlib>
#include <cstring>

#include "engine.hpp"
#include "format.hpp"

namespace rbg {

static const int32_t kMinMaxSeedI32[2] = {INT32_MAX, INT32_MIN};
static const uint32_t kMinMaxSeedU32[2] = {0xFFFFFFFFu, 0u};

constexpr size_t kBsibBudget = 1ull << 30;
static size_t bsib_budget() {
  const char* e = std::getenv("RBG_BSI_BUILD_WS");
  const unsigned long long v = e ? std::strtoull(e, nullptr, 10) : 0;
  return (size_t)std::min<unsigned long long>(v ? v : kBsibBudget, 4ull << 30);
}

struct BsibPlan {
  Ctx* c;
  size_t K = 0;
  int m = 0;
  size_t key_bytes = 0;
  size_t P = 0;
// ... 692 lines not shown
      p.n_pairs = sc + 4;
      p.out_rank = dr.as<uint32_t>();
      p.out_val = dv.as<uint32_t>();
      p.cap = cap;
      launch_bsitr_sweep(s, 2, a, has_found, c->bsit_ckeys.as<uint16_t>(), sc, grid, p);
      HIPCHK(hipGetLastError());
      unsigned long long np = 0;
      std::vector<uint16_t> rkeys(K);
      std::vector<uint8_t> run(K, 0);
      HIPCHK(hipMemcpyAsync(&np, sc + 4, 8, hipMemcpyDeviceToHost, s));
      HIPCHK(hipMemcpyAsync(rkeys.data(), c->bsib_pkeys.p, 2 * K, hipMemcpyDeviceToHost, s));
      HIPCHK(hipStreamSynchronize(s));
      const size_t n = (size_t)std::min<unsigned long long>(np, cap);
      std::vector<uint32_t> hr(n), hv(n);
      if (n) {
        HIPCHK(hipMemcpyAsync(hr.data(), dr.p, 4 * n, hipMemcpyDeviceToHost, s));
        HIPCHK(hipMemcpyAsync(hv.data(), dv.p, 4 * n, hipMemcpyDeviceToHost, s));
        HIPCHK(hipStreamSynchronize(s));
      }
      pool_put(c, dr);
      pool_put(c, dv);
      std::vector<int32_t> slot(65536, -1);
      for (size_t ki = 0; ki < K; ki++)
        if (isfull[ki]) slot[rkeys[ki]] = (int32_t)ki;
      bsit_full_runs(hr, hv, n, slot, (uint64_t)batch_size, run);
      if (std::find(run.begin(), run.end(), (uint8_t)1) != run.end()) {
        CHK(pinned_ensure(c, K));
        std::memcpy(c->pinned, run.data(), K);
        HIPCHK(hipMemcpyAsync(c->bsia_run.p, c->pinned, K, hipMemcpyHostToDevice, s));
        CHK(plan.sweep(false, fill));
        dbg(s, "bsi_transpose: full keys (host)");
      }
    }
  }
  const uint32_t mn = (uint32_t)h3[0], mx = (uint32_t)(h3[0] >> 32);
  const int nb = mx ? 32 - __builtin_clz(mx) : 0;
  CHK(plan.emit(1 + nb, fill, "bsi_transpose: write", out_id));
  out3[0] = nb;
  out3[1] = (int32_t)mn;
  out3[2] = (int32_t)mx;
  return RBG_OK;
}

static int bsi_minmax(int op, int32_t s, int32_t e, int32_t lo, int32_t hi) {
  switch (op) {
    case BSI_LT: return s > hi ? 1 : s <= lo ? 2 : 0;
    case BSI_LE: return s >= hi ? 1 : s < lo ? 2 : 0;
    case BSI_GT: return s < lo ? 1 : s >= hi ? 2 : 0;
    case BSI_GE: return s <= lo ? 1 : s > hi ? 2 : 0;
    case BSI_EQ:
      if (lo == hi && lo == s) return 1;
      return (s < lo || s > hi) ? 2 : 0;
    case BSI_NEQ:
      if (lo == hi) return lo == s ? 2 : 1;
      return 0;
    case BSI_RANGE:
      if (s <= lo && e >= hi) return 1;
      return (s > hi || e < lo) ? 2 : 0;
    default: return 0;
  }
}

static int ctx_bsi(Ctx* c, int32_t id, int op, int nbits, int has_found, int32_t start, int32_t end,
                   int32_t min_value, int32_t max_value, int want_sum) {
  Batch* B;
  CHK(get_batch(c, id, &B));
  if (!B->key_major || B->packed || nbits < 0 || nbits + 2 > kBsiMaxInputs || B->n_bm != (size_t)(1 + nbits + (has_found ? 1 : 0)) ||
      op < 0 || op > BSI_SUM_ONLY || (op == BSI_SUM_ONLY && !has_found)) {
    set_err("bsi: batch must hold ebM, nbits slices and the optional foundSet; bad op");
    return RBG_ERR_ILLEGAL_ARGUMENT;
  }
  hipStream_t s = c->stream;
  CHK(c->bsi_sums.ensure(8 * kBsiSumAll));
  c->bsi_nbits = nbits;
  int mode = op;
  if (op != BSI_SUM_ONLY) {
    const int mm = bsi_minmax(op, start, end, min_value, max_value);
    if (mm == 1) mode = BSI_ALL;
    if (mm == 2) mode = -1;
  }
  const size_t ub = std::min<size_t>(kMaxKeys, std::max<size_t>(B->n_ctr, 1));
  OutCtx oc;
  CHK(prepare_output(c, ub, kStagedMax * ub + B->max_ser, &oc, op == BSI_SUM_ONLY));
  c->pending_src = {id};
  const uint32_t need = mode == -1 ? 0xFFFFFFFFu : (op == BSI_SUM_ONLY ? (uint32_t)(nbits + 1) : 0u);
  BsiScratch sc{};
  if (mode >= 0 && mode <= BSI_RANGE) {
    CHK(c->bsi_defer.ensure(4 * (ub + 1)));
    CHK(c->bsi_cnts.ensure((size_t)4 * 128 * 4 * ub));
    CHK(c->bsi_kin.ensure((size_t)16 * 34 * ub));
    CHK(c->bsi_table.ensure((size_t)16 * 34 * ub));
    sc = BsiScratch{c->bsi_defer.as<uint32_t>(), c->bsi_cnts.as<int>(), c->bsi_kin.p, ub, c->bsi_table.p};
    if (!c->bsi_claims.p) {
      CHK(c->bsi_claims.ensure(4 * kBsiClaimWords));
      HIPCHK(hipMemsetAsync(c->bsi_claims.p, 0, 4 * kBsiClaimWords, s));
    }
    sc.claims = c->bsi_claims.as<unsigned int>();
  }
  WideArgs wa{};
  wa.desc = B->desc.as<CDesc>();
  wa.bm = B->bm.as<uint32_t>();
  wa.payload = B->payload.as<uint8_t>();
  c->mark(0);
  Task* tasks = c->tasks.as<Task>();
  uint32_t* nt = c->ntasks.as<uint32_t>();
  if (sc.defer && bsi_reg_path(mode, nbits)) {
    if (!B->bsi_cached) {
      CHK(B->bsi_tasks.ensure(sizeof(Task) * kMaxKeys));
      CHK(B->bsi_nt.ensure(64));
      CHK(B->bsi_table.ensure((size_t)16 * 34 * ub));
      launch_plan_bsi(s, B->key_off.as<uint32_t>(), B->bm.as<uint32_t>(), need, c->by_key.as<Task>(),
                      c->flag.as<uint8_t>(), c->wg_count.as<uint32_t>(), nullptr, nullptr, nullptr, nullptr);
      launch_compact(s, c->flag.as<uint8_t>(), c->by_key.as<Task>(), c->wg_count.as<uint32_t>(),
                     B->bsi_tasks.as<Task>(), B->bsi_nt.as<uint32_t>());
      launch_bsi_table(s, B->bsi_tasks.as<Task>(), B->bsi_nt.as<uint32_t>(), wa, B->bsi_table.p, ub);
      B->bsi_cached = true;
    }
    tasks = B->bsi_tasks.as<Task>();
    nt = B->bsi_nt.as<uint32_t>();
    sc.table = B->bsi_table.p;
    sc.table_ready = true;
    sc.zlb = c->zlb;
    sc.ztile = c->ztile;
    sc.zsums = c->bsi_sums.as<unsigned long long>();
    sc.nt_src = nt;
    sc.nt_dst = c->ntasks.as<uint32_t>();
  } else {
    launch_plan_bsi(s, B->key_off.as<uint32_t>(), B->bm.as<uint32_t>(), need, c->by_key.as<Task>(),
                    c->flag.as<uint8_t>(), c->wg_count.as<uint32_t>(), c->zlb, c->ztile,
                    c->bsi_sums.as<unsigned long long>(), sc.defer);
    launch_compact(s, c->flag.as<uint8_t>(), c->by_key.as<Task>(), c->wg_count.as<uint32_t>(), tasks, nt);
  }
  c->mark(1);
  BsiArgs p{mode < 0 ? BSI_EQ : mode, nbits, has_found, (uint32_t)start, (uint32_t)end};
  launch_bsi(s, grid_for(ub, 65536), tasks, nt, wa, p, oc, want_sum ? c->bsi_sums.as<unsigned long long>() : nullptr,
             sc.defer ? &sc : nullptr, want_sum ? c->bsi_sums_dst : nullptr);
  c->mark(2);
  if (op == BSI_SUM_ONLY) {
    c->last = 0;
  } else {
    defer_place(c);
  }
  c->mark(3);
  HIPCHK(hipGetLastError());
  return RBG_OK;
}


static int owen_order(Ctx* c, int M, uint32_t nt) {
  hipStream_t s = c->stream;
  std::vector<uint32_t> keys(nt);
  std::vector<int32_t> tb((size_t)nt * 32 * 4);
  if (nt) {
    HIPCHK(hipMemcpyAsync(keys.data(), c->owen_keys.p, 4 * (size_t)nt, hipMemcpyDeviceToHost, s));
    HIPCHK(hipMemcpyAsync(tb.data(), c->owen_tb.p, 16 * 32 * (size_t)nt, hipMemcpyDeviceToHost, s));
  }
  HIPCHK(hipStreamSynchronize(s));
  std::vector<std::vector<uint32_t>> lists(M);
  for (uint32_t t = 0; t < nt; t++)
    for (int j = 0; j < M; j++)
      if (tb[((size_t)t * 32 + j) * 4 + 1] > 0) lists[j].push_back(t);
  std::vector<uint8_t> ord((size_t)std::max<uint32_t>(nt, 1) * kOwenOrder, 0);
  auto ptr = [&](uint32_t j, uint32_t i) {
    const uint32_t t = lists[j][i];
    return HPtr{j, i, keys[t], (uint32_t)tb[((size_t)t * 32 + j) * 4 + 1], t};
  };
  auto push = [&](const HPtr& x) {
    uint8_t* o = ord.data() + (size_t)x.pos * kOwenOrder;
    o[1 + o[0]++] = (uint8_t)x.bm;
  };
  JHeap pq;
  for (int j = 0; j < M; j++)
    if (!lists[j].empty()) pq.add(ptr((uint32_t)j, 0));
  auto advance_add = [&](const HPtr& x) {
    if (x.i + 1 < lists[x.bm].size()) pq.add(ptr(x.bm, x.i + 1));
  };
  while (!pq.q.empty()) {
    const HPtr x1 = pq.poll();
    push(x1);
    if (pq.q.empty() || pq.q[0].key != x1.key) {
      advance_add(x1);
      continue;
    }
    const HPtr x2 = pq.poll();
    push(x2);
    while (!pq.q.empty() && pq.q[0].key == x1.key) {
      const HPtr x = pq.poll();
      push(x);
      if (x.i + 1 < lists[x.bm].size()) pq.add(ptr(x.bm, x.i + 1));
      else if (pq.q.empty()) break;
    }
    advance_add(x1);
    advance_add(x2);
  }
  CHK(c->owen_ord.ensure(ord.size()));
  HIPCHK(hipMemcpyAsync(c->owen_ord.p, ord.data(), ord.size(), hipMemcpyHostToDevice, s));
  HIPCHK(hipStreamSynchronize(s));
  return RBG_OK;
}

static int ctx_bsi_buffer(Ctx* c, int32_t id, int op, int nbits, int has_found, int32_t start, int32_t end,
                          int32_t min_value, int32_t max_value) {
  Batch* B;
  CHK(get_batch(c, id, &B));
  if (!B->key_major || B->packed || nbits < 0 || nbits + 2 > kBsiMaxInputs ||
      B->n_bm != (size_t)(1 + nbits + (has_found ? 1 : 0)) || op < 0 || op > RBG_BSI_RANGE_NEQ_DIRECT) {
    set_err("bsi: batch must hold ebM, nbits slices and the optional foundSet; bad op");
    return RBG_ERR_ILLEGAL_ARGUMENT;
  }
  hipStream_t s = c->stream;
  int mode, nb_eff = nbits, found_eff = has_found;
  if (op == RBG_BSI_RANGE_NEQ_DIRECT || op == BSI_NEQ) {
    const int mm = op == BSI_NEQ ? bsi_minmax(BSI_NEQ, start, end, min_value, max_value) : 0;
    if (mm) {
      mode = mm == 1 ? BSI_ALL : -1;
    } else {
      const int em = bsi_minmax(BSI_EQ, start, 0, min_value, max_value);
      mode = BSI_NEQ;
      if (em == 2) {
        mode = BSI_ALL;
        found_eff = 0;
      } else if (em == 1) {
        nb_eff = 0;
      }
    }
  } else {
    const int mm = bsi_minmax(op, start, end, min_value, max_value);
    mode = mm == 1 ? BSI_ALL : mm == 2 ? -1 : op;
  }
  uint32_t zeros = 0, ones = 0;
  if (mode == BSI_GE || mode == BSI_RANGE) {
    const int32_t b = (int32_t)((uint32_t)start - 1u);
    const uint32_t nbx = ~(uint32_t)b;
    const int lsz = nbx == 0 ? 64 : __builtin_ctz(nbx);
    for (int w = nbits - 1; w >= lsz; w--) {
      if ((((uint32_t)b >> w) & 1u) == 0) zeros |= 1u << w;
      else ones |= 1u << w;
    }
  }
  const int M = __builtin_popcount(zeros);
  const size_t ub = std::min<size_t>(kMaxKeys, std::max<size_t>(B->n_ctr, 1));
  return with_big_runs(c, true, "bsi", [&](const BigRuns& big) -> int {
    OutCtx oc;
    CHK(prepare_output(c, ub, kStagedMax * ub + B->max_ser + big.cap, &oc, false));
    c->pending_src = {id};
    const uint32_t need = mode == -1 ? 0xFFFFFFFFu : 0xFFFFFFFEu;
    c->mark(0);
    launch_plan_bsi(s, B->key_off.as<uint32_t>(), B->bm.as<uint32_t>(), need, c->by_key.as<Task>(),
                    c->flag.as<uint8_t>(), c->wg_count.as<uint32_t>(), c->zlb, c->ztile, nullptr, nullptr);
    launch_compact(s, c->flag.as<uint8_t>(), c->by_key.as<Task>(), c->wg_count.as<uint32_t>(), c->tasks.as<Task>(),
                   c->ntasks.as<uint32_t>());
    c->mark(1);
    WideArgs wa{};
    wa.desc = B->desc.as<CDesc>();
    wa.bm = B->bm.as<uint32_t>();
    wa.payload = B->payload.as<uint8_t>();
    BsiArgs p{};
    p.op = mode < 0 ? BSI_EQ : mode;
    p.nbits = nb_eff;
    p.has_found = found_eff;
    p.pred0 = (uint32_t)start;
    p.pred1 = (uint32_t)end;
    p.buffer = 1;
    p.found_input = nbits + 1;
    p.owen_zeros = zeros;
    p.owen_ones = ones;
    p.big = big;
    const int grid = grid_for(ub, 65536);
    if (mode >= 0 && M >= 3) {
      CHK(c->owen_tb.ensure((size_t)16 * 32 * ub));
      CHK(c->owen_keys.ensure(4 * ub));
      p.owen_tb = c->owen_tb.p;
      p.task_keys = c->owen_keys.as<uint32_t>();
      launch_bsi_owen_pre(s, grid, c->tasks.as<Task>(), c->ntasks.as<uint32_t>(), wa, p);
      HIPCHK(hipGetLastError());
      uint32_t nt = 0;
      HIPCHK(hipMemcpyAsync(&nt, c->ntasks.p, 4, hipMemcpyDeviceToHost, s));
      HIPCHK(hipStreamSynchronize(s));
      CHK(owen_order(c, M, nt));
      p.owen_order = c->owen_ord.as<uint8_t>();
    }
    if (mode >= 0) launch_bsi_buf(s, grid, c->tasks.as<Task>(), c->ntasks.as<uint32_t>(), wa, p, oc);
    return op_end(c);
  });
}

static int ctx_bsi_sums(Ctx* c, int64_t* out2) {
  if (!c->bsi_sums.p) {
    out2[0] = out2[1] = 0;
    return RBG_OK;
  }
  HIPCHK(hipMemcpyAsync(out2, c->bsi_sums.as<uint64_t>() + kBsiSumOut, 16, hipMemcpyDeviceToHost, c->stream));
  HIPCHK(hipStreamSynchronize(c->stream));
  return RBG_OK;
}

static int bsi_load(OneShot& os, const uint8_t* ebm, size_t ebm_len, const uint8_t* const* slices, const size_t* lens,
                    size_t nbits, const uint8_t* found, size_t found_len, int32_t* id) {
  if (!ebm || (nbits && (!slices || !lens)) || nbits + 2 > (size_t)kBsiMaxInputs) return RBG_ERR_ILLEGAL_ARGUMENT;
  std::vector<const uint8_t*> bufs{ebm};
  std::vector<size_t> ls{ebm_len};
  for (size_t i = 0; i < nbits; i++) {
    bufs.push_back(slices[i]);
    ls.push_back(lens[i]);
  }
  if (found) {
    bufs.push_back(found);
    ls.push_back(found_len);
  }
  return os.load(bufs.data(), ls.data(), bufs.size(), id);
}

static int oneshot_fetch(OneShot& os, int32_t id, size_t n, rbg_buffer* outs) {
  os.adopt(id);
  return ctx_batch_fetch_range(os.c, id, 0, n, outs);
}

}

using namespace rbg;

extern "C" {

int rbg_ctx_bsi(rbg_ctx* ctx, int32_t batch, int op, int nbits, int has_found, int32_t start, int32_t end,
                int32_t min_value, int32_t max_value, int want_sum) {
  Ctx* c;
  CHK(session(ctx, &c));
  return ctx_bsi(c, batch, op, nbits, has_found, start, end, min_value, max_value, want_sum);
}
int rbg_ctx_bsi_sums(rbg_ctx* ctx, int64_t* out2) {
  Ctx* c;
  CHK(session(ctx, &c));
  if (!out2) return RBG_ERR_ILLEGAL_ARGUMENT;
  return ctx_bsi_sums(c, out2);
}
int rbg_ctx_bsi_sums_target(rbg_ctx* ctx, void* dst2) {
  if (!ctx) return RBG_ERR_ILLEGAL_ARGUMENT;
  ctx->c.bsi_sums_dst = dst2;
  return RBG_OK;
}
int rbg_ctx_bsi_sums_device(rbg_ctx* ctx, void* dst2) {
  Ctx* c;
  CHK(session(ctx, &c));
  if (!dst2 || !c->bsi_sums.p) return RBG_ERR_ILLEGAL_ARGUMENT;
  launch_bsi_sums_out(c->stream, c->bsi_sums.as<unsigned long long>(), dst2);
  HIPCHK(hipGetLastError());
  return RBG_OK;
}
int rbg_bsi_compare(int op, int32_t start, int32_t end, const uint8_t* ebm, size_t ebm_len,
                    const uint8_t* const* slices, const size_t* slice_lens, size_t nbits, int32_t min_value,
                    int32_t max_value, const uint8_t* found, size_t found_len, rbg_buffer* out) {
  if (!out || op < 0 || op > BSI_RANGE) return RBG_ERR_ILLEGAL_ARGUMENT;
  OneShot os;
  CHK(os.open());
  Ctx* c = os.c;
  int32_t id;
  CHK(bsi_load(os, ebm, ebm_len, slices, slice_lens, nbits, found, found_len, &id));
  CHK(ctx_bsi(c, id, op, (int)nbits, found ? 1 : 0, start, end, min_value, max_value, 0));
  return ctx_fetch(c, out);
}
int rbg_bsi_compare_buffer(int op, int32_t start, int32_t end, const uint8_t* ebm, size_t ebm_len,
                           const uint8_t* const* slices, const size_t* slice_lens, size_t nbits, int32_t min_value,
                           int32_t max_value, const uint8_t* found, size_t found_len, rbg_buffer* out) {
  if (!out || op < 0 || op > RBG_BSI_RANGE_NEQ_DIRECT) return RBG_ERR_ILLEGAL_ARGUMENT;
  OneShot os;
// ... 211 lines not shown
```

roaringbitmap_amd/csrc/engine_synth.cpp:

```cpp
#include <algorithm>

#include "engine.hpp"

namespace rbg {

int synth_c2(Ctx* c, int kind, uint64_t seed, int32_t* out_id) {
  const int32_t id = new_batch(c);
  Batch& b = *c->batches[id];
  const size_t C = kMaxKeys;
  b.n_bm = 1;
  b.n_ctr = C;
  b.key_major = true;
  b.payload_bytes = (size_t)kSlotBytes * C;
  CHK(b.keys.ensure(2 * C + 16));
  CHK(b.desc.ensure(sizeof(CDesc) * C + 16));
  CHK(b.bm.ensure(4 * C + 16));
  CHK(b.key_off.ensure(4 * (kMaxKeys + 1)));
  CHK(b.bm_off.ensure(8));
  CHK(b.payload.ensure(b.payload_bytes + 64));
  std::vector<uint32_t> key_off(kMaxKeys + 1);
  for (int k = 0; k <= kMaxKeys; k++) key_off[k] = (uint32_t)k;
  b.h_bm_off = {0u, (uint32_t)C};
  b.h_bm_nctr = {(uint32_t)C};
  hipStream_t s = c->stream;
  HIPCHK(hipMemsetAsync(b.bm.p, 0, 4 * C, s));
  HIPCHK(hipMemcpyAsync(b.key_off.p, key_off.data(), 4 * (kMaxKeys + 1), hipMemcpyHostToDevice, s));
  HIPCHK(hipMemcpyAsync(b.bm_off.p, b.h_bm_off.data(), 8, hipMemcpyHostToDevice, s));
  launch_synth_c2(s, seed, kind == 0 ? -1 : kind - 16, b.desc.as<CDesc>(), b.keys.as<uint16_t>(), b.payload.as<uint8_t>());
  HIPCHK(hipGetLastError());
  std::vector<CDesc> d(C);
  HIPCHK(hipMemcpyAsync(d.data(), b.desc.p, sizeof(CDesc) * C, hipMemcpyDeviceToHost, s));
  HIPCHK(hipStreamSynchronize(s));
  int64_t card = 0;
  for (const CDesc& x : d) {
    b.n_kind[x.kind]++;
    card += x.card;
  }
  b.long_card = card;
  b.h_bm_card = {card};
  b.ser_bytes = 0;
  b.live = true;
  *out_id = id;
  return RBG_OK;
}

int synth_c3(Ctx* c, int kind, uint64_t seed, size_t n, int key_lo, int key_hi, int32_t* out_id) {
  key_lo = std::max(0, key_lo);
  key_hi = std::min(kMaxKeys, key_hi);
  if (n == 0 || n > 0x7FFFFFFF || key_hi < key_lo) {
    set_err("synthetic C3 needs 0 < n and key_lo <= key_hi");
    return RBG_ERR_ILLEGAL_ARGUMENT;
  }
  const int nkeys = key_hi - key_lo;
  hipStream_t s = c->stream;
  std::vector<uint32_t> key_off(kMaxKeys + 1, 0);
  std::vector<uint16_t> h_keys;
  std::vector<uint32_t> h_bm, nctr(n, 0);
  if (kind == 1) {
    for (int k = 0; k < kMaxKeys; k++) {
      const bool in = k >= key_lo && k < key_hi;
      key_off[k + 1] = key_off[k] + (in ? (uint32_t)n : 0u);
    }
    for (size_t i = 0; i < n; i++) nctr[i] = (uint32_t)nkeys;
  } else {
    std::vector<uint32_t> base(n);
    for (size_t i = 0; i < n; i++) {
      base[i] = c3c_base(seed, (uint32_t)i);
      for (uint32_t k = base[i]; k < base[i] + 16; k++)
        if ((int)k >= key_lo && (int)k < key_hi) {
          key_off[k + 1]++;
          nctr[i]++;
        }
    }
    for (int k = 0; k < kMaxKeys; k++) key_off[k + 1] += key_off[k];
    h_keys.resize(key_off[kMaxKeys]);
    h_bm.resize(key_off[kMaxKeys]);
    std::vector<uint32_t> cur(key_off.begin(), key_off.end() - 1);
    for (size_t i = 0; i < n; i++)
      for (uint32_t k = base[i]; k < base[i] + 16; k++)
        if ((int)k >= key_lo && (int)k < key_hi) {
          h_keys[cur[k]] = (uint16_t)k;
          h_bm[cur[k]++] = (uint32_t)i;
        }
  }
  const size_t C = key_off[kMaxKeys];
  const int32_t id = new_batch(c);
  Batch& b = *c->batches[id];
  b.n_bm = n;
  b.n_ctr = C;
  b.key_major = true;
  b.h_bm_nctr = nctr;
  b.h_bm_card.assign(n, 0);
  CHK(b.keys.ensure(2 * C + 16));
  CHK(b.desc.ensure(sizeof(CDesc) * C + 16));
  CHK(b.bm.ensure(4 * C + 16));
  CHK(b.key_off.ensure(4 * (kMaxKeys + 1)));
  CHK(b.bm_off.ensure(8));
  HIPCHK(hipMemcpyAsync(b.key_off.p, key_off.data(), 4 * (kMaxKeys + 1), hipMemcpyHostToDevice, s));
  if (kind == 1) {
    CHK(c->scratch.ensure(16 * (size_t)kMaxKeys));
    unsigned long long* kb = c->scratch.as<unsigned long long>();
    launch_synth_c3u(s, seed, (uint32_t)n, key_lo, nkeys, kb, nullptr, nullptr, nullptr, nullptr, nullptr, 0);
    std::vector<unsigned long long> bytes(nkeys + 1, 0);
    if (nkeys) HIPCHK(hipMemcpyAsync(bytes.data(), kb, 8 * nkeys, hipMemcpyDeviceToHost, s));
    HIPCHK(hipStreamSynchronize(s));
    unsigned long long tot = 0;
    for (int k = 0; k < nkeys; k++) {
      const unsigned long long x = bytes[k];
      bytes[k] = tot;
      tot += x;
    }
    b.payload_bytes = tot;
    CHK(b.payload.ensure(tot + 64));
    HIPCHK(hipMemcpyAsync(kb, bytes.data(), 8 * std::max(nkeys, 1), hipMemcpyHostToDevice, s));
    launch_synth_c3u(s, seed, (uint32_t)n, key_lo, nkeys, nullptr, kb, b.desc.as<CDesc>(), b.keys.as<uint16_t>(),
                     b.bm.as<uint32_t>(), b.payload.as<uint8_t>(), 1);
    b.n_kind[DK_A] = (int64_t)C;
    b.packed = true;
  } else {
    b.payload_bytes = 8192 * C;
    CHK(b.payload.ensure(b.payload_bytes + 64));
    if (C) {
      HIPCHK(hipMemcpyAsync(b.keys.p, h_keys.data(), 2 * C, hipMemcpyHostToDevice, s));
      HIPCHK(hipMemcpyAsync(b.bm.p, h_bm.data(), 4 * C, hipMemcpyHostToDevice, s));
    }
    launch_synth_c3c(s, seed, C, b.keys.as<uint16_t>(), b.bm.as<uint32_t>(), b.desc.as<CDesc>(),
                     b.payload.as<uint8_t>());
    b.n_kind[DK_B] = (int64_t)C;
  }
  HIPCHK(hipGetLastError());
  HIPCHK(hipMemsetAsync(c->scalar.p, 0, 8, s));
  launch_sum_cards(s, b.desc.as<CDesc>(), C, c->scalar.as<unsigned long long>());
  unsigned long long card = 0;
  HIPCHK(hipMemcpyAsync(&card, c->scalar.p, 8, hipMemcpyDeviceToHost, s));
  HIPCHK(hipStreamSynchronize(s));
  b.long_card = (int64_t)card;
  b.ser_bytes = 0;
  b.live = true;
  *out_id = id;
  return RBG_OK;
}

int synth_c4(Ctx* c, uint64_t seed, size_t n_pairs, int32_t* out_id) {
  const size_t nb = 2 * n_pairs;
  if (nb == 0 || nb > 0x7FFFFFFF) return RBG_ERR_ILLEGAL_ARGUMENT;
  const int32_t id = new_batch(c);
  Batch& b = *c->batches[id];
  b.n_bm = nb;
  b.key_major = false;
  b.h_bm_off.assign(nb + 1, 0);
  b.h_bm_nctr.resize(nb);
  b.h_bm_card.resize(nb);
  std::vector<CDesc> d;
  d.reserve(nb * 5 / 2 + 16);
  uint64_t off = 0;
  for (size_t j = 0; j < nb; j++) {
    const uint64_t h = splitmix64(seed ^ (0xC4000000ULL + j));
    const int K = 1 + (int)(h % 4);
    uint64_t used = 0;
    int got = 0;
    for (uint64_t t = 1; got < K; t++) {
      const int k = (int)(splitmix64(h + t) & 63);
      if (!((used >> k) & 1)) {
        used |= 1ULL << k;
        got++;
      }
    }
    int64_t card_sum = 0;
    for (int k = 0; k < 64; k++)
      if ((used >> k) & 1) {
        const uint32_t card = 16 + (uint32_t)(splitmix64(h ^ ((uint64_t)k << 40)) % 497);
        d.push_back(CDesc{off, card, (uint16_t)k, DK_A, 0});
        off += (2 * card + 15) & ~15ull;
        card_sum += card;
      }
    b.h_bm_nctr[j] = (uint32_t)K;
    b.h_bm_off[j + 1] = b.h_bm_off[j] + (uint32_t)K;
    b.h_bm_card[j] = card_sum;
    b.long_card += card_sum;
  }
  const size_t C = d.size();
  b.n_ctr = C;
  b.n_kind[DK_A] = (int64_t)C;
  b.payload_bytes = off;
  CHK(b.desc.ensure(sizeof(CDesc) * C + 16));
  CHK(b.keys.ensure(2 * C + 16));
  CHK(b.bm.ensure(4 * C + 16));
  CHK(b.bm_off.ensure(4 * (nb + 1)));
  CHK(b.payload.ensure(off + 64));
  hipStream_t s = c->stream;
  std::vector<uint16_t> hk(C);
  std::vector<uint32_t> hbm(C);
  for (size_t j = 0; j < nb; j++)
    for (uint32_t p = b.h_bm_off[j]; p < b.h_bm_off[j + 1]; p++) {
      hk[p] = d[p].key;
      hbm[p] = (uint32_t)j;
    }
  HIPCHK(hipMemcpyAsync(b.desc.p, d.data(), sizeof(CDesc) * C, hipMemcpyHostToDevice, s));
  HIPCHK(hipMemcpyAsync(b.keys.p, hk.data(), 2 * C, hipMemcpyHostToDevice, s));
  HIPCHK(hipMemcpyAsync(b.bm.p, hbm.data(), 4 * C, hipMemcpyHostToDevice, s));
  HIPCHK(hipMemcpyAsync(b.bm_off.p, b.h_bm_off.data(), 4 * (nb + 1), hipMemcpyHostToDevice, s));
  launch_synth_arrays(s, seed, b.desc.as<CDesc>(), C, b.payload.as<uint8_t>());
  HIPCHK(hipGetLastError());
  HIPCHK(hipStreamSynchronize(s));
  b.live = true;
  *out_id = id;
  return RBG_OK;
}

int synth_c5(Ctx* c, uint64_t seed, size_t rows, int key_lo, int key_hi, int32_t* out_id) {
  const int nbits = 31, nin = nbits + 1;
  if (rows == 0 || rows > (1ull << 32)) return RBG_ERR_ILLEGAL_ARGUMENT;
  key_lo = std::max(0, key_lo);
  key_hi = (int)std::min<uint64_t>((uint64_t)std::min(key_hi, kMaxKeys), (rows + 65535) / 65536);
  const int nkeys = std::max(0, key_hi - key_lo);
  hipStream_t s = c->stream;
  const size_t G = (size_t)nkeys * nin;
  CHK(c->scratch.ensure(8 * G + 64));
  uint32_t* cards = c->scratch.as<uint32_t>();
  uint32_t* pos = cards + G;
  unsigned int* mm = reinterpret_cast<unsigned int*>(c->scalar.p);
  const unsigned int mm0[2] = {0xFFFFFFFFu, 0u};
  HIPCHK(hipMemcpyAsync(mm, mm0, 8, hipMemcpyHostToDevice, s));
  launch_synth_c5(s, seed, rows, key_lo, nbits, nkeys, 0, cards, nullptr, mm, nullptr, nullptr, nullptr, nullptr);
  std::vector<uint32_t> h(G);
  unsigned int mmh[2];
  HIPCHK(hipMemcpyAsync(h.data(), cards, 4 * G, hipMemcpyDeviceToHost, s));
  HIPCHK(hipMemcpyAsync(mmh, mm, 8, hipMemcpyDeviceToHost, s));
  HIPCHK(hipStreamSynchronize(s));
  std::vector<uint32_t> key_off(kMaxKeys + 1, 0), hp(G, 0);
  uint32_t C = 0;
  for (int k = 0; k < kMaxKeys; k++) {
    const int j = k - key_lo;
    if (j >= 0 && j < nkeys)
      for (int i = 0; i < nin; i++)
        if (h[(size_t)j * nin + i]) hp[(size_t)j * nin + i] = C++;
    key_off[k + 1] = C;
  }
  const int32_t id = new_batch(c);
  Batch& b = *c->batches[id];
  b.n_bm = nin;
  b.n_ctr = C;
  b.key_major = true;
  b.payload_bytes = (size_t)kSlotBytes * C;
  b.h_bm_nctr.assign(nin, 0);
  b.h_bm_card.assign(nin, 0);
  for (int k = 0; k < nkeys; k++)
    for (int i = 0; i < nin; i++)
      if (h[(size_t)k * nin + i]) {
        b.h_bm_nctr[i]++;
        b.h_bm_card[i] += h[(size_t)k * nin + i];
      }
  for (int i = 0; i < nin; i++) b.long_card += b.h_bm_card[i];
  CHK(b.keys.ensure(2 * (size_t)C + 16));
  CHK(b.desc.ensure(sizeof(CDesc) * (size_t)C + 16));
  CHK(b.bm.ensure(4 * (size_t)C + 16));
  CHK(b.key_off.ensure(4 * (kMaxKeys + 1)));
  CHK(b.bm_off.ensure(8));
  CHK(b.payload.ensure(b.payload_bytes + 64));
  HIPCHK(hipMemcpyAsync(b.key_off.p, key_off.data(), 4 * (kMaxKeys + 1), hipMemcpyHostToDevice, s));
  HIPCHK(hipMemcpyAsync(pos, hp.data(), 4 * G, hipMemcpyHostToDevice, s));
  launch_synth_c5(s, seed, rows, key_lo, nbits, nkeys, 1, nullptr, pos, nullptr, b.desc.as<CDesc>(),
                  b.keys.as<uint16_t>(),
                  b.bm.as<uint32_t>(), b.payload.as<uint8_t>());
  HIPCHK(hipGetLastError());
  std::vector<CDesc> d(C);
  if (C) HIPCHK(hipMemcpyAsync(d.data(), b.desc.p, sizeof(CDesc) * C, hipMemcpyDeviceToHost, s));
  HIPCHK(hipStreamSynchronize(s));
  for (const CDesc& x : d) b.n_kind[x.kind]++;
  b.bsi_min = (int32_t)mmh[0];
  b.bsi_max = (int32_t)mmh[1];
  b.live = true;
  *out_id = id;
  return RBG_OK;
}

}

using namespace rbg;

extern "C" {

int rbg_synth_key_bytes(int kind, uint64_t seed, size_t n, uint64_t* out) {
  if (!out || (kind != 1 && kind != 2)) return RBG_ERR_ILLEGAL_ARGUMENT;
  for (int k = 0; k < kMaxKeys; k++) out[k] = 0;
  for (size_t i = 0; i < n; i++) {
    if (kind == 1) {
      for (int k = 0; k < kMaxKeys; k++) out[k] += 4 + 2 * (uint64_t)c3u_card(seed, (uint32_t)i, (uint32_t)k);
    } else {
      const uint32_t b0 = c3c_base(seed, (uint32_t)i);
      for (uint32_t k = b0; k < b0 + 16; k++) out[k] += 4 + 8192;
    }
  }
  return RBG_OK;
}

}
```

roaringbitmap_amd/csrc/engine_wide.cpp:

```cpp
#include <algorithm>
#include <utility>

#include "engine.hpp"

namespace rbg {

static int horizontal_order(Ctx* c, Batch* B, bool* identity) {
  *identity = B->h_chain_identity;
  if (*identity) return RBG_OK;
  CHK(batch_host_index(c, B));
  std::vector<uint32_t> order;
  if (B->key_major || B->n_bm == 1) {
    const std::vector<CDesc>& D = B->h_desc;
    const size_t n = B->n_ctr;
    std::vector<std::pair<uint32_t, uint32_t>> rkeys;
    std::vector<uint32_t> seg;
    bool tie = false;
    for (size_t p = 0; p < n && !tie;) {
      size_t e = p;
      bool has_r = false;
      while (e < n && D[e].key == D[p].key) has_r |= D[e++].kind == DK_R;
      if (has_r && e - p > 1) {
        seg.resize(e - p);
        for (size_t q = p; q < e; q++) seg[q - p] = D[q].card;
// ... 34 lines not shown
    if (has(x.bm, x.i + 1)) pq.add(ptr(x.bm, x.i + 1));
  };
  while (!pq.q.empty()) {
    const HPtr x1 = pq.poll();
    order.push_back(x1.pos);
    if (pq.q.empty() || pq.q[0].key != x1.key) {
      advance_add(x1);
      continue;
    }
    const HPtr x2 = pq.poll();
    order.push_back(x2.pos);
    while (!pq.q.empty() && pq.q[0].key == x1.key) {
      const HPtr x = pq.poll();
      order.push_back(x.pos);
      if (has(x.bm, x.i + 1)) pq.add(ptr(x.bm, x.i + 1));
      else if (pq.q.empty()) break;
    }
    advance_add(x1);
    advance_add(x2);
  }
  if (order.size() != B->n_ctr) {
    set_err("horizontal order: container table inconsistent");
    return RBG_ERR_DEVICE;
  }
  CHK(c->order.ensure(4 * std::max<size_t>(order.size(), 1)));
  if (!order.empty())
    HIPCHK(hipMemcpyAsync(c->order.p, order.data(), 4 * order.size(), hipMemcpyHostToDevice, c->stream));
  HIPCHK(hipStreamSynchronize(c->stream));
  return RBG_OK;
}

namespace {
struct PQHost {
  std::vector<PQEnt>& heap;
  std::vector<int32_t>& nodes;
  std::vector<uint8_t>& tmp;
  std::vector<int32_t>& slots;
  void add(PQStep& c, PQEnt x) {
    int k = c.heap_n++;
    while (k > 0) {
      const int p = (k - 1) >> 1;
      if (pq_cmp(x.size, heap[p].size) >= 0) break;
      heap[k] = heap[p];
      k = p;
    }
    heap[k] = x;
  }
  PQEnt poll(PQStep& c) {
    const PQEnt r = heap[0];
    const int n = --c.heap_n;
    if (n == 0) return r;
    const PQEnt x = heap[n];
    int k = 0;
    const int half = n >> 1;
    while (k < half) {
      int ch = 2 * k + 1;
      if (ch + 1 < n && pq_cmp(heap[ch].size, heap[ch + 1].size) > 0) ch++;
      if (pq_cmp(x.size, heap[ch].size) <= 0) break;
      heap[k] = heap[ch];
      k = ch;
    }
    heap[k] = x;
    return r;
  }
  int32_t node(int i) { return nodes[i]; }
  void set_node(int i, int32_t v) { nodes[i] = v; }
  bool istmp(int i) { return tmp[i] != 0; }
  void set_istmp(int i) { tmp[i] = 1; }
  int slot_pop(PQStep& c) { return slots[--c.slot_top]; }
  void slot_push(PQStep& c, int s) { slots[c.slot_top++] = s; }
};
}

static int ctx_pq(Ctx* c, int op, Batch* B, int32_t id, int key_lo, int key_hi) {
  if (key_lo != 0 || key_hi != kMaxKeys) {
    set_err("priorityqueue aggregations need the full key range (the queue order depends on every key)");
    return RBG_ERR_ILLEGAL_ARGUMENT;
  }
  hipStream_t s = c->stream;
  const size_t N = B->n_bm;
  const size_t ub = std::min<size_t>(kMaxKeys, std::max<size_t>(B->n_ctr, 1));
  OutCtx oc;
  CHK(prepare_output(c, ub, kStagedMax * ub + B->max_ser, &oc, false));
  c->pending_src = {id};
  c->mark(0);
  launch_plan_wide(s, N ? 0 : 1, B->key_off.as<uint32_t>(), N ? (uint32_t)N : 0xFFFFFFFFu, 0, kMaxKeys,
                   c->by_key.as<Task>(), c->flag.as<uint8_t>(), c->wg_count.as<uint32_t>(), c->zlb, c->ztile);
  launch_compact(s, c->flag.as<uint8_t>(), c->by_key.as<Task>(), c->wg_count.as<uint32_t>(), c->tasks.as<Task>(),
                 c->ntasks.as<uint32_t>());
  c->mark(1);
  if (!N) {
    c->mark(2);
    launch_place(s, c->ntasks.as<uint32_t>(), oc, c->info.as<ResultInfo>());
    c->last = 1;
    c->mark(3);
    HIPCHK(hipGetLastError());
    return RBG_OK;
  }
  uint32_t h_nt = 0;
  HIPCHK(hipMemcpyAsync(&h_nt, c->ntasks.p, 4, hipMemcpyDeviceToHost, s));
  std::vector<unsigned long long> leaf(N);
  DevBuf dsz;
  CHK(dsz.ensure(8 * N));
  HIPCHK(hipMemsetAsync(dsz.p, 0, 8 * N, s));
  launch_pq_leaf_sizes(s, B->desc.as<CDesc>(), B->bm.as<uint32_t>(), B->payload.as<uint8_t>(), B->n_ctr,
                       dsz.as<unsigned long long>());
  HIPCHK(hipMemcpyAsync(leaf.data(), dsz.p, 8 * N, hipMemcpyDeviceToHost, s));
  HIPCHK(hipStreamSynchronize(s));

  const size_t n_slots = N / 2 + 2;
  const size_t stride = std::max<uint32_t>(h_nt, 1);
  const size_t st_bytes = n_slots * stride * sizeof(PQState);
  std::vector<Task> h_tasks(h_nt);
  if (h_nt) HIPCHK(hipMemcpyAsync(h_tasks.data(), c->tasks.p, sizeof(Task) * h_nt, hipMemcpyDeviceToHost, s));
  HIPCHK(hipStreamSynchronize(s));
  std::vector<uint32_t> kbase(stride, 0);
  std::vector<int32_t> ktop(stride, 0);
  size_t free_b = 0, total_b = 0;
  pool_clear(c);
  HIPCHK(hipMemGetInfo(&free_b, &total_b));
  const size_t budget = free_b / 10 * 9;
  auto pool_blocks = [&](int32_t cap) {
    size_t n = 0;
    for (uint32_t t = 0; t < h_nt; t++) n += (size_t)std::min(h_tasks[t].b / 2, cap);
    return n;
  };
  int32_t cap = 0;
  for (uint32_t t = 0; t < h_nt; t++) cap = std::max(cap, h_tasks[t].b / 2);
  if (st_bytes + pool_blocks(cap) * 8192 > budget) {
    int32_t lo = 0, hi = cap;
    while (lo < hi) {
      const int32_t mid = lo + (hi - lo + 1) / 2;
      if (st_bytes + pool_blocks(mid) * 8192 <= budget) lo = mid;
      else hi = mid - 1;
    }
    if (lo < 1 && cap >= 1) {
      set_err("priorityqueue: " + std::to_string(n_slots) + " temps x " + std::to_string(stride) +
              " union keys need more than the free device memory; use FastAggregation.or / xor");
      return RBG_ERR_OUT_OF_MEMORY;
    }
    cap = lo;
  }
  size_t n_blk = 0;
  for (uint32_t t = 0; t < h_nt; t++) {
    kbase[t] = (uint32_t)n_blk;
    ktop[t] = std::min(h_tasks[t].b / 2, cap);
    n_blk += (size_t)ktop[t];
  }
  n_blk = std::max<size_t>(n_blk, 1);
  std::vector<PQEnt> heap(N);
  std::vector<int32_t> nodes(2 * N);
  std::vector<uint8_t> tmp(2 * N, 0);
  std::vector<int32_t> slots(n_slots);
  for (size_t k = 0; k < N; k++) nodes[k] = (int32_t)k;
  for (size_t k = 0; k < n_slots; k++) slots[k] = (int32_t)(n_slots - 1 - k);
  PQCtl ctl{};
  ctl.step.or_mode = op == RBG_WIDE_PQ_OR;
  ctl.step.n_nodes = (int32_t)N;
  ctl.step.slot_top = (int32_t)n_slots;
  ctl.step.rel1 = ctl.step.rel2 = -1;
  PQHost hm{heap, nodes, tmp, slots};
  for (size_t k = 0; k < N; k++) hm.add(ctl.step, PQEnt{8 + (int64_t)leaf[k], (int32_t)k, 0});
  pq_plan(hm, ctl.step);
  std::vector<uint32_t> order(h_nt);
  for (uint32_t t = 0; t < h_nt; t++) order[t] = t;
  std::stable_sort(order.begin(), order.end(), [&](uint32_t x, uint32_t y) { return ktop[x] > ktop[y]; });
  std::vector<uint32_t> rank(h_nt);
  for (uint32_t i = 0; i < h_nt; i++) rank[order[i]] = i;
  const int32_t max_cap = h_nt ? ktop[order[0]] : 0;
  std::vector<size_t> lvl(max_cap + 1, 0);
  for (int32_t j = 0, i = (int32_t)h_nt; j < max_cap; j++) {
    while (i > 0 && ktop[order[i - 1]] <= j) i--;
    lvl[j + 1] = lvl[j] + (size_t)i;
  }
  std::vector<int32_t> stack(n_blk);
  for (uint32_t t = 0; t < h_nt; t++)
    for (int32_t i = 0; i < ktop[t]; i++) stack[kbase[t] + i] = (int32_t)(lvl[ktop[t] - 1 - i] + rank[t]);
  auto al = [](size_t x) { return (x + 255) & ~(size_t)255; };
  const size_t o_heap = al(sizeof(PQCtl)), o_node = o_heap + al(16 * N), o_tmp = o_node + al(8 * N),
               o_slots = o_tmp + al(2 * N), o_stack = o_slots + al(4 * n_slots), o_base = o_stack + al(4 * n_blk),
               o_top = o_base + al(4 * stride), o_end = o_top + al(4 * stride);
  DevBuf meta, states, arena;
  CHK(meta.ensure(o_end));
  CHK(states.ensure(st_bytes));
  CHK(arena.ensure(n_blk * 8192));
  uint8_t* mb = meta.as<uint8_t>();
  HIPCHK(hipMemcpyAsync(mb, &ctl, sizeof(ctl), hipMemcpyHostToDevice, s));
  HIPCHK(hipMemcpyAsync(mb + o_heap, heap.data(), 16 * N, hipMemcpyHostToDevice, s));
  HIPCHK(hipMemcpyAsync(mb + o_node, nodes.data(), 8 * N, hipMemcpyHostToDevice, s));
  HIPCHK(hipMemcpyAsync(mb + o_tmp, tmp.data(), 2 * N, hipMemcpyHostToDevice, s));
  HIPCHK(hipMemcpyAsync(mb + o_slots, slots.data(), 4 * n_slots, hipMemcpyHostToDevice, s));
  HIPCHK(hipMemcpyAsync(mb + o_stack, stack.data(), 4 * n_blk, hipMemcpyHostToDevice, s));
  HIPCHK(hipMemcpyAsync(mb + o_base, kbase.data(), 4 * stride, hipMemcpyHostToDevice, s));
  HIPCHK(hipMemcpyAsync(mb + o_top, ktop.data(), 4 * stride, hipMemcpyHostToDevice, s));
  const PQDev D{reinterpret_cast<PQCtl*>(mb), reinterpret_cast<PQEnt*>(mb + o_heap),
                reinterpret_cast<int32_t*>(mb + o_node), mb + o_tmp, reinterpret_cast<int32_t*>(mb + o_slots),
                states.as<PQState>(), stride, arena.as<uint64_t>(), reinterpret_cast<int32_t*>(mb + o_stack),
                reinterpret_cast<const uint32_t*>(mb + o_base), reinterpret_cast<int32_t*>(mb + o_top)};
  const PQArgs pa{B->desc.as<CDesc>(), B->bm.as<uint32_t>(), B->payload.as<uint8_t>()};
  const int grid = grid_for(h_nt, 65536);
  for (size_t k = 0; k + 1 < N; k++) {
    launch_pq_step(s, grid, c->tasks.as<Task>(), c->ntasks.as<uint32_t>(), pa, D);
    if ((k & 1023) == 1023) HIPCHK(hipGetLastError());
  }
  c->mark(2);
  launch_pq_final(s, grid, c->tasks.as<Task>(), c->ntasks.as<uint32_t>(), pa, op == RBG_WIDE_PQ_OR ? 1 : 0, D, oc);
  HIPCHK(hipGetLastError());
  launch_place(s, c->ntasks.as<uint32_t>(), oc, c->info.as<ResultInfo>());
  PQCtl done{};
  HIPCHK(hipMemcpyAsync(&done, mb, sizeof(done), hipMemcpyDeviceToHost, s));
  HIPCHK(hipStreamSynchronize(s));
  if (done.err || !done.step.final_step) {
    set_err(done.err ? "priorityqueue: a key's block pool ran out (" + std::to_string(n_blk) + " x 8 KiB in all)"
                     : std::string("priorityqueue: the device queue did not finish"));
    return done.err ? RBG_ERR_OUT_OF_MEMORY : RBG_ERR_DEVICE;
  }
  c->last = 1;
  c->mark(3);
  HIPCHK(hipGetLastError());
  return RBG_OK;
}

bool wide_reads_packed(int op, size_t n) {
  switch (op) {
    case RBG_WIDE_OR:
    case RBG_WIDE_XOR:
    case RBG_WIDE_WORKSHY_AND:
    case RBG_WIDE_PARALLEL_OR:
    case RBG_WIDE_PARALLEL_XOR:
    case RBG_WIDE_BUFFER_OR_MUTABLE:
    case RBG_WIDE_HORIZONTAL_OR:
    case RBG_WIDE_HORIZONTAL_XOR:
    case RBG_WIDE_PQ_OR:
    case RBG_WIDE_PQ_XOR: return true;
    case RBG_WIDE_AND: return n > 10;
    default: return false;
  }
}

int ctx_wide(Ctx* c, int op, int32_t id, int key_lo, int key_hi, const int32_t* ids, bool card_only,
             int* host_card_out, bool* host_card_valid, int32_t start_override) {
  Batch* B;
  CHK(get_batch(c, id, &B));
  if (!B->key_major) {
    set_err("wide ops need a key-major batch");
    return RBG_ERR_ILLEGAL_ARGUMENT;
  }
  if (B->packed && !card_only && !wide_reads_packed(op, B->n_bm)) {
    set_err("this wide op needs slot-aligned payloads (load the batch without packing)");
    return RBG_ERR_ILLEGAL_ARGUMENT;
  }
  key_lo = std::max(0, key_lo);
  key_hi = std::min(kMaxKeys, key_hi);
  if (host_card_valid) *host_card_valid = false;
  if (!card_only && (op == RBG_WIDE_PQ_OR || op == RBG_WIDE_PQ_XOR)) {
    if (B->n_kind[DK_R] != 0 || key_lo != 0 || key_hi != kMaxKeys) return ctx_pq(c, op, B, id, key_lo, key_hi);
    op = op == RBG_WIDE_PQ_OR ? RBG_WIDE_OR : RBG_WIDE_XOR;
  }
  bool buffer = false;
  if (!card_only && op >= RBG_WIDE_BUFFER_AND && op <= RBG_WIDE_BUFFER_AND_ITER) {
    buffer = true;
    op = op == RBG_WIDE_BUFFER_AND ? RBG_WIDE_AND : op == RBG_WIDE_BUFFER_NAIVE_AND ? RBG_WIDE_NAIVE_AND : RBG_WIDE_AND_ITER;
  }
  hipStream_t s = c->stream;
  const size_t N = B->n_bm;
  int mode = WIDE_OR, plan_mode = 0;
  uint32_t start_bm = 0, chain = 0;
  const uint32_t* order = nullptr;
  std::vector<uint8_t> skip;
  if (card_only) {
    if (op != RBG_WIDE_CARD_AND && op != RBG_WIDE_CARD_OR) return RBG_ERR_ILLEGAL_ARGUMENT;
    const bool full_range = key_lo == 0 && key_hi == kMaxKeys;
    if (N == 0 || (N == 1 && full_range)) {
      const int64_t cc = N ? B->h_bm_card[0] : 0;
      *host_card_out = (int32_t)(uint32_t)(uint64_t)cc;
      *host_card_valid = true;
      c->last = 2;
      return RBG_OK;
    }
    if (op == RBG_WIDE_CARD_AND && N >= 2) {
      mode = WIDE_AND_SHY_CARD;
      plan_mode = 1;
    } else {
      mode = WIDE_OR_CARD;
    }
  } else {
    switch (op) {
      case RBG_WIDE_OR: mode = WIDE_OR; break;
      case RBG_WIDE_XOR: mode = WIDE_XOR; break;
      case RBG_WIDE_AND:
      case RBG_WIDE_AND_ITER:
      case RBG_WIDE_NAIVE_AND:
      case RBG_WIDE_WORKSHY_AND:
        plan_mode = 1;
        if (op == RBG_WIDE_WORKSHY_AND && N == 0) {
          set_err("workShyAnd needs at least one bitmap");
          return RBG_ERR_ILLEGAL_ARGUMENT;
        }
        if ((op == RBG_WIDE_AND && N > 10) || op == RBG_WIDE_WORKSHY_AND) {
          mode = WIDE_AND_SHY;
        } else {
          mode = WIDE_AND_NAIVE;
          skip.assign(std::max<size_t>(N, 1), 0);
          if (op != RBG_WIDE_AND_ITER) {
            if (start_override >= 0 && (size_t)start_override < N) {
              start_bm = (uint32_t)start_override;
            } else {
              for (size_t i = 1; i < N; i++)
                if (B->h_bm_nctr[i] < B->h_bm_nctr[start_bm]) start_bm = (uint32_t)i;
            }
            for (size_t i = 0; i < N; i++)
              skip[i] = (i == start_bm) || (ids && ids[i] == ids[start_bm]);
          } else {
            start_bm = 0;
            skip[0] = 1;
          }
        }
        break;
      case RBG_WIDE_PARALLEL_OR: mode = WIDE_LAZY_CHAIN; chain = kChainLimit16; break;
      case RBG_WIDE_PARALLEL_XOR: mode = WIDE_XOR_CHAIN; break;
      case RBG_WIDE_BUFFER_OR_MUTABLE: mode = WIDE_LAZY_CHAIN; break;
      case RBG_WIDE_HORIZONTAL_OR:
      case RBG_WIDE_HORIZONTAL_XOR:
        mode = op == RBG_WIDE_HORIZONTAL_OR ? WIDE_LAZY_CHAIN : WIDE_XOR_CHAIN;
        chain = op == RBG_WIDE_HORIZONTAL_OR ? kChainN1Clone : kChainKeepEmpty;
        bool identity;
        CHK(horizontal_order(c, B, &identity));
        order = identity ? nullptr : c->order.as<uint32_t>();
        break;
      default: return RBG_ERR_ILLEGAL_ARGUMENT;
    }
  }
  if (N == 0) {
    plan_mode = 2;
  }
  const bool big_runs = buffer && mode == WIDE_AND_NAIVE && N > 0;
  return with_big_runs(c, big_runs, "naive_and", [&](const BigRuns& big) -> int {
    const size_t ub = std::min<size_t>(kMaxKeys, std::max<size_t>(B->n_ctr, 1));
    OutCtx oc;
    CHK(prepare_output(c, ub, kStagedMax * ub + B->max_ser + big.cap, &oc, card_only));
    if (!card_only && (mode == WIDE_OR || mode == WIDE_LAZY_CHAIN)) oc.spec = c->pending.spec = 1;
    c->pending_src = {id};
    if (!skip.empty()) {
      CHK(c->skip.ensure(skip.size()));
      HIPCHK(hipMemcpyAsync(c->skip.p, skip.data(), skip.size(), hipMemcpyHostToDevice, s));
    }
    const uint32_t n_req = plan_mode == 2 ? 0xFFFFFFFFu : (uint32_t)N;
    c->mark(0);
    launch_plan_wide(s, plan_mode == 0 ? 0 : 1, B->key_off.as<uint32_t>(), n_req, key_lo, key_hi,
                     c->by_key.as<Task>(), c->flag.as<uint8_t>(), c->wg_count.as<uint32_t>(), c->zlb, c->ztile);
    launch_compact(s, c->flag.as<uint8_t>(), c->by_key.as<Task>(), c->wg_count.as<uint32_t>(), c->tasks.as<Task>(),
                   c->ntasks.as<uint32_t>());
    WideArgs wa{};
    wa.desc = B->desc.as<CDesc>();
    wa.bm = B->bm.as<uint32_t>();
    wa.payload = B->payload.as<uint8_t>();
    wa.skip = skip.empty() ? nullptr : c->skip.as<uint8_t>();
    wa.start_bm = start_bm;
    wa.all_array = (B->n_kind[DK_B] == 0 && B->n_kind[DK_R] == 0 && !B->gapped) ? 1u : 0u;
    wa.slot32 = B->payload_bytes < (1ull << 36) ? 1u : 0u;
    wa.order = order;
    wa.chain = chain;
    wa.rd_bytes = c->prof_cap > 0 && c->rd_ctr.p ? c->rd_ctr.as<unsigned long long>() : nullptr;
    wa.buffer = buffer ? 1u : 0u;
    wa.big = big;
    c->mark(1);
    launch_wide(s, mode, grid_for(ub, 65536), c->tasks.as<Task>(), c->ntasks.as<uint32_t>(), wa, oc,
                c->task_card.as<uint32_t>());
    c->mark(2);
    if (card_only) {
      launch_reduce_card(s, c->task_card.as<uint32_t>(), c->ntasks.as<uint32_t>(), c->info.as<ResultInfo>(), oc.err);
      c->last = 2;
    } else {
      defer_place(c);
    }
    c->mark(3);
    HIPCHK(hipGetLastError());
    return RBG_OK;
  });
}

}
```

Baseline: 2316 GB/s.

## Double-buffer result sets on a second stream so pairwise ops overlap

Result: faster. 2471 GB/s (median of 6 runs) (+6.7%).

```diff
diff --git a/roaringbitmap_amd/csrc/engine.cpp b/roaringbitmap_amd/csrc/engine.cpp
--- a/roaringbitmap_amd/csrc/engine.cpp
+++ b/roaringbitmap_amd/csrc/engine.cpp
@@ -54,8 +54,15 @@
     g_ctxs.erase(std::remove(g_ctxs.begin(), g_ctxs.end(), this), g_ctxs.end());
   }
   prof_free();
+  if (rs[1].stream) {
+    (void)hipStreamSynchronize(rs[1].stream);
+    if (stream) (void)hipStreamSynchronize(stream);
+  }
   if (pinned) (void)hipHostFree(pinned);
   batches.clear();
+  if (rs[1].done) (void)hipEventDestroy(rs[1].done);
+  if (rs[1].main_done) (void)hipEventDestroy(rs[1].main_done);
+  if (rs[1].stream) (void)hipStreamDestroy(rs[1].stream);
   if (stream) (void)hipStreamDestroy(stream);
 }
 
@@ -110,11 +117,14 @@
   return RBG_OK;
 }
 
-int enter(Ctx* c) {
+int enter(Ctx* c, bool counts) {
   t_cur_ctx = c;
+  if (counts) c->seq++;
   HIPCHK(hipSetDevice(c->device));
   return RBG_OK;
 }
+
+static int rs_alloc(Ctx* c, ResultSet& r);
 
 int ctx_init(Ctx* c, int device) {
   int n = 0;
@@ -138,17 +148,66 @@
   HIPCHK(hipStreamCreateWithFlags(&c->stream, hipStreamNonBlocking));
   CHK(c->by_key.ensure(sizeof(PTask) * kMaxKeys));
   CHK(c->flag.ensure(kMaxKeys));
-  CHK(c->tasks.ensure(sizeof(PTask) * (kMaxKeys + 32768)));
-  CHK(c->ntasks.ensure(64));
   CHK(c->wg_count.ensure(4 * 256));
-  CHK(c->wg_epoch.ensure(8 * 256));
-  HIPCHK(hipMemset(c->wg_epoch.p, 0, 8 * 256));
-  CHK(c->lb.ensure(kLbHeader + 8 * (kMaxKeys + 2 * kMaxTiles + kMaxAggTiles)));
-  CHK(c->recs.ensure(sizeof(ORec) * kMaxKeys));
-  CHK(c->kind_by_out.ensure(kMaxKeys));
   CHK(c->scalar.ensure(64));
-  CHK(c->info.ensure(sizeof(ResultInfo)));
-  CHK(c->task_card.ensure(4 * kMaxKeys));
+  return rs_alloc(c, c->rs[0]);
+}
+
+static int join_set(Ctx* c, ResultSet& r) {
+  r.in_flight = false;
+  if (r.stream == c->stream || !r.touched) return RBG_OK;
+  HIPCHK(hipEventRecord(r.done, r.stream));
+  HIPCHK(hipStreamWaitEvent(c->stream, r.done, 0));
+  r.touched = false;
+  return RBG_OK;
+}
+int join_result(Ctx* c) { return join_set(c, c->r()); }
+int join_all(Ctx* c) {
+  CHK(join_set(c, c->rs[0]));
+  return join_set(c, c->rs[1]);
+}
+int main_set(Ctx* c) {
+  CHK(join_all(c));
+  c->cur = 0;
+  c->seq++;
+  return RBG_OK;
+}
+static int lane_sync(Ctx* c) {
+  ResultSet& r = c->r();
+  if (r.stream == c->stream) return RBG_OK;
+  if (r.synced_seq != c->seq) {
+    HIPCHK(hipEventRecord(r.main_done, c->stream));
+    HIPCHK(hipStreamWaitEvent(r.stream, r.main_done, 0));
+    r.synced_seq = c->seq;
+  }
+  r.touched = true;
+  return RBG_OK;
+}
+int sync_streams(Ctx* c) {
+  if (c->rs[1].stream) HIPCHK(hipStreamSynchronize(c->rs[1].stream));
+  HIPCHK(hipStreamSynchronize(c->stream));
+  for (ResultSet& r : c->rs) r.in_flight = r.touched = false;
+  return RBG_OK;
+}
+static int rs_alloc(Ctx* c, ResultSet& r) {
+  if (r.ready) return RBG_OK;
+  if (&r == &c->rs[0]) {
+    r.stream = c->stream;
+  } else {
+    if (!r.stream) HIPCHK(hipStreamCreateWithFlags(&r.stream, hipStreamNonBlocking));
+    if (!r.done) HIPCHK(hipEventCreateWithFlags(&r.done, hipEventDisableTiming));
+    if (!r.main_done) HIPCHK(hipEventCreateWithFlags(&r.main_done, hipEventDisableTiming));
+  }
+  CHK(r.tasks.ensure(sizeof(PTask) * (kMaxKeys + 32768)));
+  CHK(r.ntasks.ensure(64));
+  CHK(r.wg_epoch.ensure(8 * 256));
+  HIPCHK(hipMemsetAsync(r.wg_epoch.p, 0, 8 * 256, r.stream));
+  CHK(r.lb.ensure(kLbHeader + 8 * (kMaxKeys + 2 * kMaxTiles + kMaxAggTiles)));
+  CHK(r.recs.ensure(sizeof(ORec) * kMaxKeys));
+  CHK(r.kind_by_out.ensure(kMaxKeys));
+  CHK(r.info.ensure(sizeof(ResultInfo)));
+  CHK(r.task_card.ensure(4 * kMaxKeys));
+  r.ready = true;
   return RBG_OK;
 }
 
@@ -163,12 +222,12 @@
 }
 
 static uint32_t next_epoch(Ctx* c) {
-  if (++c->epoch == 0) ++c->epoch;
-  return c->epoch;
+  if (++c->r().epoch == 0) ++c->r().epoch;
+  return c->r().epoch;
 }
 static PlanOut plan_out(Ctx* c, bool compacts = true) {
-  return PlanOut{c->wg_epoch.as<uint64_t>(), compacts ? next_epoch(c) : 0, c->tasks.as<PTask>(),
-                 c->ntasks.as<uint32_t>(), c->zlb, c->ztile};
+  return PlanOut{c->r().wg_epoch.as<uint64_t>(), compacts ? next_epoch(c) : 0, c->r().tasks.as<PTask>(),
+                 c->r().ntasks.as<uint32_t>(), c->zlb, c->ztile};
 }
 
 int find_batch(Ctx* c, int32_t id, Batch** out) {
@@ -270,70 +329,93 @@
   return (int)std::max<size_t>(g, 1);
 }
 
-int prepare_output(Ctx* c, size_t max_tasks, size_t max_payload, OutCtx* oc, bool card_only) {
-  uint8_t* lb = c->lb.as<uint8_t>();
+int prepare_output(Ctx* c, size_t max_tasks, size_t max_payload, OutCtx* oc, bool card_only, bool lanes) {
+  if (!lanes || card_only) {
+    CHK(main_set(c));
+  } else {
+    if (c->r().in_flight) {
+      ResultSet& o = c->rs[c->cur ^ 1];
+      CHK(rs_alloc(c, o));
+      c->cur ^= 1;
+      o.in_flight = false;
+      o.last = 0;
+    } else if (c->cur != 0) {
+      CHK(main_set(c));
+    }
+    CHK(lane_sync(c));
+  }
+  uint8_t* lb = c->r().lb.as<uint8_t>();
   *oc = OutCtx{};
   oc->err = reinterpret_cast<uint32_t*>(lb + 64);
   oc->status = reinterpret_cast<uint64_t*>(lb + kLbHeader);
   oc->tile_status = reinterpret_cast<uint64_t*>(lb + kLbHeader + 8 * kMaxKeys);
   oc->tile_card = reinterpret_cast<uint64_t*>(lb + kLbHeader + 8 * (kMaxKeys + kMaxTiles));
-  oc->recs = c->recs.as<ORec>();
-  c->serialized = false;
-  c->place_pending = false;
-  c->agg_ok = false;
-  c->ri_valid = false;
-  c->pending_ub = 0;
+  oc->recs = c->r().recs.as<ORec>();
+  c->r().serialized = false;
+  c->r().place_pending = false;
+  c->r().agg_ok = false;
+  c->r().ri_valid = false;
+  c->r().pending_ub = 0;
   c->zlb = c->ztile = nullptr;
-  c->pending_src.clear();
+  c->r().pending_src.clear();
   if (card_only) {
     c->zlb = reinterpret_cast<uint64_t*>(lb);
     return RBG_OK;
   }
   const uint64_t P0 = header_reserve(max_tasks);
-  CHK(c->result.ensure(P0 + max_payload + 64));
-  c->result_cap = P0 + max_payload;
-  CHK(c->scratch.ensure((size_t)kSlotBytes * std::max<size_t>(max_tasks, 1) + 64));
+  CHK(c->r().result.ensure(P0 + max_payload + 64));
+  c->r().result_cap = P0 + max_payload;
+  CHK(c->r().scratch.ensure((size_t)kSlotBytes * std::max<size_t>(max_tasks, 1) + 64));
   c->zlb = reinterpret_cast<uint64_t*>(lb);
   c->ztile = reinterpret_cast<uint64_t*>(lb + kLbHeader + 8 * kMaxKeys);
-  oc->out = c->result.as<uint8_t>();
+  oc->out = c->r().result.as<uint8_t>();
   oc->payload_base = P0;
-  oc->scratch = c->scratch.as<uint8_t>();
-  oc->kind_by_out = c->kind_by_out.as<uint8_t>();
-  c->pending = *oc;
-  c->pending_ub = max_tasks;
+  oc->scratch = c->r().scratch.as<uint8_t>();
+  oc->kind_by_out = c->r().kind_by_out.as<uint8_t>();
+  c->r().pending = *oc;
+  c->r().pending_ub = max_tasks;
   return RBG_OK;
 }
 
 void defer_place(Ctx* c) {
-  c->place_pending = true;
-  c->last = 1;
-}
-int ensure_placed(Ctx* c) {
-  if (!c->place_pending) return RBG_OK;
-  launch_place(c->stream, c->ntasks.as<uint32_t>(), c->pending, c->info.as<ResultInfo>());
-  HIPCHK(hipGetLastError());
-  c->place_pending = false;
-  return RBG_OK;
-}
-
-int ctx_serialize(Ctx* c) {
-  if (c->last != 1) {
+  c->r().place_pending = true;
+  c->r().last = 1;
+}
+static int place_on(Ctx* c, hipStream_t s) {
+  if (!c->r().place_pending) return RBG_OK;
+  launch_place(s, c->r().ntasks.as<uint32_t>(), c->r().pending, c->r().info.as<ResultInfo>());
+  HIPCHK(hipGetLastError());
+  c->r().place_pending = false;
+  return RBG_OK;
+}
+int ensure_placed(Ctx* c) { return place_on(c, c->stream); }
+
+int ctx_serialize(Ctx* c, bool on_main) {
+  ResultSet& r = c->r();
+  if (r.last != 1) {
     set_err("no materialised result pending");
     return RBG_ERR_ILLEGAL_ARGUMENT;
   }
-  if (c->serialized) return RBG_OK;
-  if (c->place_pending && c->agg_ok && !c->pending.spec && c->pending_ub <= (size_t)kMaxAggTiles * kAggTile) {
-    launch_serialize_agg(c->stream, c->ntasks.as<uint32_t>(), c->pending, c->info.as<ResultInfo>(), c->pending_ub);
-    HIPCHK(hipGetLastError());
-    c->place_pending = false;
-    c->serialized = true;
-    return RBG_OK;
-  }
-  CHK(ensure_placed(c));
-  if (c->pending.spec) launch_spec_fix(c->stream, c->ntasks.as<uint32_t>(), c->pending);
-  launch_serialize(c->stream, c->ntasks.as<uint32_t>(), c->pending);
-  HIPCHK(hipGetLastError());
-  c->serialized = true;
+  if (r.serialized) return RBG_OK;
+  hipStream_t s = r.stream;
+  if (on_main) {
+    CHK(join_result(c));
+    c->seq++;
+    s = c->stream;
+  } else {
+    CHK(lane_sync(c));
+  }
+  if (r.place_pending && r.agg_ok && !r.pending.spec && r.pending_ub <= (size_t)kMaxAggTiles * kAggTile) {
+    launch_serialize_agg(s, r.ntasks.as<uint32_t>(), r.pending, r.info.as<ResultInfo>(), r.pending_ub);
+    r.place_pending = false;
+  } else {
+    CHK(place_on(c, s));
+    if (r.pending.spec) launch_spec_fix(s, r.ntasks.as<uint32_t>(), r.pending);
+    launch_serialize(s, r.ntasks.as<uint32_t>(), r.pending);
+  }
+  HIPCHK(hipGetLastError());
+  r.serialized = true;
+  r.in_flight = !on_main;
   return RBG_OK;
 }
 
@@ -353,7 +435,7 @@
 }
 
 static void op_begin(Ctx* c, std::initializer_list<int32_t> src) {
-  c->pending_src = src;
+  c->r().pending_src = src;
   c->mark(0);
   c->mark(1);
 }
@@ -678,7 +760,7 @@
   return with_big_runs(c, true, "buffer and / andNot", [&](const BigRuns& big) -> int {
     OutCtx oc;
     CHK(prepare_output(c, ub, A.b->payload_bytes + B.b->payload_bytes + kStagedMax * ub + big.cap, &oc, false));
-    c->pending_src = {ia, ib};
+    c->r().pending_src = {ia, ib};
     c->mark(0);
     const PlanOut po = plan_out(c);
     launch_plan_pairwise(s, op, key_lo, key_hi, A, B, po, oc.err);
@@ -712,7 +794,7 @@
     HIPCHK(hipMemcpyAsync(&pl, c->ornot_plan.p, sizeof(pl), hipMemcpyDeviceToHost, s));
     HIPCHK(hipStreamSynchronize(s));
     if (pl.neg) {
-      c->last = 0;
+      c->r().last = 0;
       set_err("orNot: negative maxSize (the reference throws NegativeArraySizeException)");
       return RBG_ERR_ILLEGAL_ARGUMENT;
     }
@@ -786,13 +868,13 @@
 }
 
 int ctx_pairwise(Ctx* c, int op, int32_t ia, size_t ma, int32_t ib, size_t mb, bool card_only, int key_lo,
-                 int key_hi) {
+                 int key_hi, bool lanes) {
   if (op == RBG_AND_BUFFER || op == RBG_ANDNOT_BUFFER) {
     if (card_only) return RBG_ERR_ILLEGAL_ARGUMENT;
     return ctx_pairwise_buffer(c, op == RBG_AND_BUFFER ? OP_AND : OP_ANDNOT, ia, ma, ib, mb, key_lo, key_hi);
   }
   if (op == RBG_OR_INPLACE && !card_only) {
-    CHK(ctx_pairwise(c, OP_OR, ia, ma, ib, mb, false, key_lo, key_hi));
+    CHK(ctx_pairwise(c, OP_OR, ia, ma, ib, mb, false, key_lo, key_hi, false));
     if (!c->ones.p) {
       CHK(c->ones.ensure(8192));
       HIPCHK(hipMemsetAsync(c->ones.p, 0xFF, 8192, c->stream));
@@ -800,9 +882,10 @@
     Operand A, B;
     CHK(resolve(c, ia, ma, &A));
     CHK(resolve(c, ib, mb, &B));
-    launch_ior_fix(c->stream, c->ntasks.as<uint32_t>(), c->recs.as<ORec>(), A, B, c->ones.as<uint8_t>());
+    CHK(join_result(c));
+    launch_ior_fix(c->stream, c->r().ntasks.as<uint32_t>(), c->r().recs.as<ORec>(), A, B, c->ones.as<uint8_t>());
     HIPCHK(hipGetLastError());
-    c->agg_ok = false;
+    c->r().agg_ok = false;
     return RBG_OK;
   }
   if (op < 0 || op > 3) return RBG_ERR_ILLEGAL_ARGUMENT;
@@ -811,7 +894,6 @@
   Operand A, B;
   CHK(resolve(c, ia, ma, &A));
   CHK(resolve(c, ib, mb, &B));
-  hipStream_t s = c->stream;
   const int plan_op = card_only ? OP_AND : op;
   size_t ub;
   switch (plan_op) {
@@ -823,14 +905,15 @@
   const bool dense = nkeys > 0 && 2 * ub >= nkeys;
   OutCtx oc;
   CHK(prepare_output(c, dense ? std::max(ub, nkeys) : ub, A.b->payload_bytes + B.b->payload_bytes + kStagedMax * ub,
-                     &oc, card_only));
-  c->pending_src = {ia, ib};
+                     &oc, card_only, lanes));
+  hipStream_t s = c->r().stream;
+  c->r().pending_src = {ia, ib};
   c->mark(0);
   const PwDirect pd{key_lo};
   const PlanOut po = plan_out(c, !dense);
   if (dense) {
     launch_plan_balanced(s, plan_op, card_only ? 1 : 0, key_lo, (uint32_t)nkeys, A, B, po, oc,
-                         c->task_card.as<uint32_t>());
+                         c->r().task_card.as<uint32_t>());
   } else {
     launch_plan_pairwise(s, plan_op, key_lo, key_hi, A, B, po, oc.err);
     dbg(s, "plan");
@@ -838,17 +921,17 @@
   c->mark(1);
   if (!card_only) {
     oc.tile_agg = reinterpret_cast<unsigned long long*>(oc.tile_status + 2 * kMaxTiles);
-    c->pending.tile_agg = oc.tile_agg;
-    c->agg_ok = true;
+    c->r().pending.tile_agg = oc.tile_agg;
+    c->r().agg_ok = true;
   }
   const int grid = grid_for(((dense ? nkeys : ub) + 3) / 4, 16384);
   launch_pairwise(s, op, card_only ? 1 : 0, grid, po.tasks, po.n_tasks, A.payload, B.payload, oc,
-                  c->task_card.as<uint32_t>(), dense ? &pd : nullptr);
+                  c->r().task_card.as<uint32_t>(), dense ? &pd : nullptr);
   dbg(s, "pairwise");
   c->mark(2);
   if (card_only) {
-    launch_reduce_card(s, c->task_card.as<uint32_t>(), c->ntasks.as<uint32_t>(), c->info.as<ResultInfo>(), oc.err);
-    c->last = 2;
+    launch_reduce_card(s, c->r().task_card.as<uint32_t>(), c->r().ntasks.as<uint32_t>(), c->r().info.as<ResultInfo>(), oc.err);
+    c->r().last = 2;
   } else {
     defer_place(c);
   }
@@ -881,27 +964,28 @@
 }
 
 int ctx_info(Ctx* c, ResultInfo* ri) {
-  if (c->last == 1) CHK(ensure_placed(c));
-  HIPCHK(hipMemcpyAsync(ri, c->info.p, sizeof(ResultInfo), hipMemcpyDeviceToHost, c->stream));
+  CHK(join_result(c));
+  if (c->r().last == 1) CHK(ensure_placed(c));
+  HIPCHK(hipMemcpyAsync(ri, c->r().info.p, sizeof(ResultInfo), hipMemcpyDeviceToHost, c->stream));
   uint64_t card = 0;
   uint32_t err = 0;
-  if (c->last == 1)
-    HIPCHK(hipMemcpyAsync(&card, c->lb.as<uint8_t>() + 64 + 8 * kCardWord, 8, hipMemcpyDeviceToHost, c->stream));
-  if (c->last == 1 || c->last == 2)
-    HIPCHK(hipMemcpyAsync(&err, c->lb.as<uint8_t>() + 64, 4, hipMemcpyDeviceToHost, c->stream));
+  if (c->r().last == 1)
+    HIPCHK(hipMemcpyAsync(&card, c->r().lb.as<uint8_t>() + 64 + 8 * kCardWord, 8, hipMemcpyDeviceToHost, c->stream));
+  if (c->r().last == 1 || c->r().last == 2)
+    HIPCHK(hipMemcpyAsync(&err, c->r().lb.as<uint8_t>() + 64, 4, hipMemcpyDeviceToHost, c->stream));
   HIPCHK(hipStreamSynchronize(c->stream));
-  if (c->last == 1) {
+  if (c->r().last == 1) {
     ri->long_card = (int64_t)card;
     ri->card32 = (uint32_t)card;
   }
   ri->err |= err;
-  if ((c->last == 1 || c->last == 2) && ri->err) {
+  if ((c->r().last == 1 || c->r().last == 2) && ri->err) {
     set_err("a look-back spin of the op's plan or placement timed out: the result is invalid");
     return RBG_ERR_DEVICE;
   }
-  if (c->last == 1) {
-    c->last_ri = *ri;
-    c->ri_valid = true;
+  if (c->r().last == 1) {
+    c->r().last_ri = *ri;
+    c->r().ri_valid = true;
   }
   return RBG_OK;
 }
@@ -985,18 +1069,18 @@
 }
 
 int ctx_fetch(Ctx* c, rbg_buffer* out) {
-  if (c->last != 1) {
+  if (c->r().last != 1) {
     set_err("no serialized result pending");
     return RBG_ERR_ILLEGAL_ARGUMENT;
   }
-  CHK(ctx_serialize(c));
+  CHK(ctx_serialize(c, true));
   ResultInfo ri;
   CHK(ctx_info(c, &ri));
   uint8_t* p = out_alloc(ri.total);
   if (!p) return RBG_ERR_OUT_OF_MEMORY;
   out->data = p;
   out->len = ri.total;
-  const int st = download_staged(c, c->result.as<uint8_t>() + ri.start, ri.total, p);
+  const int st = download_staged(c, c->r().result.as<uint8_t>() + ri.start, ri.total, p);
   if (st != RBG_OK) {
     rbg_free(out);
     return st;
@@ -1098,6 +1182,7 @@
     return RBG_ERR_ILLEGAL_ARGUMENT;
   }
   const size_t np = B->n_bm / 2;
+  CHK(main_set(c));
   CHK(c->cards.ensure(4 * std::max<size_t>(np, 1)));
   if (B->key_major && B->n_bm > 1) {
     set_err("batched andCardinality needs a bitmap-major batch");
@@ -1122,13 +1207,13 @@
   c->mark(3);
   HIPCHK(hipGetLastError());
   c->n_cards = np;
-  c->last = 3;
+  c->r().last = 3;
   return RBG_OK;
 }
 
 int ctx_fetch_shard_device(Ctx* c, int64_t total_containers, int has_run, int64_t payload_base, void* desc_dst,
                            void* offsets_dst, void* runflag_dst, void* payload_dst) {
-  if (c->last != 1) {
+  if (c->r().last != 1) {
     set_err("no materialised result pending");
     return RBG_ERR_ILLEGAL_ARGUMENT;
   }
@@ -1142,8 +1227,9 @@
     return RBG_ERR_ILLEGAL_ARGUMENT;
   }
   ResultInfo ri;
-  if (c->ri_valid) {
-    ri = c->last_ri;
+  CHK(join_result(c));
+  if (c->r().ri_valid) {
+    ri = c->r().last_ri;
     CHK(ensure_placed(c));
   } else {
     CHK(ctx_info(c, &ri));
@@ -1154,13 +1240,13 @@
     return RBG_ERR_ILLEGAL_ARGUMENT;
   }
   uint8_t* emit_dst = (uint8_t*)payload_dst;
-  if (c->serialized) {
+  if (c->r().serialized) {
     if (ri.payload)
-      HIPCHK(hipMemcpyAsync(payload_dst, c->result.as<uint8_t>() + c->pending.payload_base, ri.payload,
+      HIPCHK(hipMemcpyAsync(payload_dst, c->r().result.as<uint8_t>() + c->r().pending.payload_base, ri.payload,
                             hipMemcpyDeviceToDevice, c->stream));
     emit_dst = nullptr;
   }
-  launch_serialize_shard(c->stream, grid_for((c->pending_ub + 255) / 256, 256), c->ntasks.as<uint32_t>(), c->pending,
+  launch_serialize_shard(c->stream, grid_for((c->r().pending_ub + 255) / 256, 256), c->r().ntasks.as<uint32_t>(), c->r().pending,
                          emit_dst, off0, (uint8_t*)desc_dst, offsets ? (uint8_t*)offsets_dst : nullptr,
                          has_run ? (uint8_t*)runflag_dst : nullptr);
   HIPCHK(hipGetLastError());
@@ -1312,7 +1398,7 @@
 }
 
 int ctx_profile(Ctx* c, int max_ops, bool compute_only) {
-  HIPCHK(hipStreamSynchronize(c->stream));
+  CHK(sync_streams(c));
   c->prof_free();
   c->prof_compute_only = compute_only;
   if (max_ops <= 0) return RBG_OK;
diff --git a/roaringbitmap_amd/csrc/engine.hpp b/roaringbitmap_amd/csrc/engine.hpp
--- a/roaringbitmap_amd/csrc/engine.hpp
+++ b/roaringbitmap_amd/csrc/engine.hpp
@@ -112,13 +112,39 @@
       size, cpart;
 };
 
+struct ResultSet {
+  hipStream_t stream = nullptr;
+  DevBuf tasks;
+  DevBuf wg_epoch;
+  uint32_t epoch = 0;
+  DevBuf lb;
+  DevBuf recs, scratch, result, kind_by_out, info, ntasks, task_card;
+  size_t result_cap = 0;
+  OutCtx pending{};
+  std::vector<int32_t> pending_src;
+  size_t pending_ub = 0;
+  bool serialized = false;
+  bool place_pending = false;
+  bool agg_ok = false;
+  ResultInfo last_ri{};
+  bool ri_valid = false;
+  int last = 0;
+  bool ready = false;
+  bool in_flight = false;
+  bool touched = false;
+  uint64_t synced_seq = 0;
+  hipEvent_t done = nullptr, main_done = nullptr;
+};
+
 struct Ctx {
   int device = 0;
   DecBufs dec;
-  DevBuf wg_epoch;
-  uint32_t epoch = 0;
   DevBuf pc_cnt, pc_part, pc_items, pc_large;
   hipStream_t stream = nullptr;
+  ResultSet rs[2];
+  int cur = 0;
+  ResultSet& r() { return rs[cur]; }
+  uint64_t seq = 1;
   std::vector<std::unique_ptr<Batch>> batches;
   std::vector<std::unique_ptr<RangeIndex>> range_indexes;
   uint64_t* zlb = nullptr;
@@ -146,20 +172,9 @@
   std::vector<DevBuf> pool;
   size_t pool_bytes = 0;
   std::mutex pool_mu;
-  ResultInfo last_ri{};
-  bool ri_valid = false;
   int bsi_nbits = 0;
-  DevBuf by_key, flag, tasks, ntasks, wg_count, lb, recs, kind_by_out, info, task_card, result, cards, skip, raw,
-      scalar, scratch;
-  size_t result_cap = 0;
-  OutCtx pending{};
-  std::vector<int32_t> pending_src;
-  size_t pending_ub = 0;
-  bool serialized = false;
-  bool place_pending = false;
-  bool agg_ok = false;
+  DevBuf by_key, flag, wg_count, cards, skip, raw, scalar;
   size_t n_cards = 0;
-  int last = 0;
   void* pinned = nullptr;
   size_t pinned_cap = 0;
   std::vector<hipEvent_t> prof_ev;
@@ -176,7 +191,7 @@
       if (phase == 3 && prof_n < prof_cap) prof_n++;
       return;
     }
-    if (prof_n < prof_cap) (void)hipEventRecord(prof_ev[4 * prof_n + phase], stream);
+    if (prof_n < prof_cap) (void)hipEventRecord(prof_ev[4 * prof_n + phase], r().stream);
     if (phase == 3 && prof_n < prof_cap) prof_n++;
   }
   ~Ctx();
@@ -195,7 +210,7 @@
 
 void dbg(hipStream_t s, const char* what);
 int ctx_init(Ctx* c, int device);
-int enter(Ctx* c);
+int enter(Ctx* c, bool counts = true);
 int tl_ctx(Ctx** out);
 int find_batch(Ctx* c, int32_t id, Batch** out);
 int get_batch(Ctx* c, int32_t id, Batch** out);
@@ -207,12 +222,16 @@
 int pinned_ensure(Ctx* c, size_t bytes);
 int upload_words(Ctx* c, void* dst, const void* src, size_t n);
 int ctx_profile(Ctx* c, int max_ops, bool compute_only);
-int prepare_output(Ctx* c, size_t max_tasks, size_t max_payload, OutCtx* oc, bool card_only);
+int prepare_output(Ctx* c, size_t max_tasks, size_t max_payload, OutCtx* oc, bool card_only, bool lanes = false);
 void defer_place(Ctx* c);
 int ensure_placed(Ctx* c);
 int grid_for(size_t tasks, size_t cap = 4096);
 int op_end(Ctx* c);
-int ctx_serialize(Ctx* c);
+int ctx_serialize(Ctx* c, bool on_main = false);
+int join_result(Ctx* c);
+int join_all(Ctx* c);
+int main_set(Ctx* c);
+int sync_streams(Ctx* c);
 int ctx_info(Ctx* c, ResultInfo* ri);
 uint8_t* out_alloc(size_t n);
 int ctx_fetch(Ctx* c, rbg_buffer* out);
@@ -239,7 +258,7 @@
 int ctx_to_bitset(Ctx* c, int32_t batch, size_t i, uint64_t first, uint64_t n, int layout, void* out_dev);
 int ctx_to_bitset_host(Ctx* c, int32_t batch, size_t i, uint64_t first, uint64_t n, int layout, void* out);
 int ctx_pairwise(Ctx* c, int op, int32_t ia, size_t ma, int32_t ib, size_t mb, bool card_only, int key_lo = 0,
-                 int key_hi = kMaxKeys);
+                 int key_hi = kMaxKeys, bool lanes = true);
 int ctx_ornot(Ctx* c, int32_t ia, size_t ma, int32_t ib, size_t mb, int64_t range_end, int flags);
 int check_range(int64_t start, int64_t end);
 int ctx_range_mut(Ctx* c, int op, int32_t ia, size_t ma, int64_t start, int64_t end, bool buf);
@@ -287,6 +306,7 @@
 template <class Pass>
 static int with_big_runs(Ctx* c, bool use_arena, const char* what, Pass&& pass) {
   if (!use_arena) return pass(BigRuns{nullptr, nullptr, 0});
+  CHK(main_set(c));
   if (!c->big_ctl.p) CHK(c->big_ctl.ensure(16));
   if (!c->big.p) CHK(c->big.ensure(16ull << 20));
   for (int attempt = 0;; attempt++) {
@@ -376,5 +396,5 @@
 };
 
 namespace rbg {
-int session(rbg_ctx* ctx, Ctx** c);
-}
+int session(rbg_ctx* ctx, Ctx** c, bool counts = true);
+}
diff --git a/roaringbitmap_amd/csrc/engine_api.cpp b/roaringbitmap_amd/csrc/engine_api.cpp
--- a/roaringbitmap_amd/csrc/engine_api.cpp
+++ b/roaringbitmap_amd/csrc/engine_api.cpp
@@ -41,10 +41,10 @@
 
 using namespace rbg;
 
-int rbg::session(rbg_ctx* ctx, Ctx** c) {
+int rbg::session(rbg_ctx* ctx, Ctx** c, bool counts) {
   if (!ctx) return RBG_ERR_ILLEGAL_ARGUMENT;
   *c = &ctx->c;
-  return enter(*c);
+  return enter(*c, counts);
 }
 
 extern "C" {
@@ -540,7 +540,7 @@
   }
   Ctx* c;
   CHK(session(ctx, &c));
-  HIPCHK(hipStreamSynchronize(c->stream));
+  CHK(sync_streams(c));
   unsigned long long v = 0;
   if (c->rd_ctr.p) HIPCHK(hipMemcpy(&v, c->rd_ctr.p, 8, hipMemcpyDeviceToHost));
   *bytes = (int64_t)v;
@@ -549,7 +549,7 @@
 int rbg_ctx_profile_read(rbg_ctx* ctx, double* ms3, int* n_ops) {
   Ctx* c;
   CHK(session(ctx, &c));
-  HIPCHK(hipStreamSynchronize(c->stream));
+  CHK(sync_streams(c));
   ms3[0] = ms3[1] = ms3[2] = 0.0;
   for (size_t i = 0; i < c->prof_n; i++) {
     for (int ph = 0; ph < 3; ph++) {
@@ -566,8 +566,7 @@
 int rbg_ctx_sync(rbg_ctx* ctx) {
   Ctx* c;
   CHK(session(ctx, &c));
-  HIPCHK(hipStreamSynchronize(c->stream));
-  return RBG_OK;
+  return sync_streams(c);
 }
 int rbg_ctx_load_separate(rbg_ctx* ctx, const uint8_t* const* bufs, const size_t* lens, size_t n, int32_t* ids) {
   Ctx* c;
@@ -592,9 +591,10 @@
   Batch* b;
   CHK(find_batch(&c, batch, &b));
   CHK(enter(&c));
-  if (c.last == 1 && !c.serialized &&
-      std::find(c.pending_src.begin(), c.pending_src.end(), batch) != c.pending_src.end())
-    CHK(ctx_serialize(&c));
+  if (c.r().last == 1 && !c.r().serialized &&
+      std::find(c.r().pending_src.begin(), c.r().pending_src.end(), batch) != c.r().pending_src.end())
+    CHK(ctx_serialize(&c, true));
+  CHK(join_all(&c));
   for (DevBuf* d : {&b->keys, &b->desc, &b->bm, &b->key_off, &b->bm_off, &b->payload, &b->ro_stats,
                     &b->bsi_tasks, &b->bsi_nt, &b->bsi_table, &b->rd_cum, &b->rd_off, &b->rd_aux})
     pool_put(&c, *d);
@@ -638,19 +638,19 @@
 }
 int rbg_ctx_pairwise(rbg_ctx* ctx, int op, int32_t a, size_t ia, int32_t b, size_t ib) {
   Ctx* c;
-  CHK(session(ctx, &c));
+  CHK(session(ctx, &c, false));
   return ctx_pairwise(c, op, a, ia, b, ib, false);
 }
 int rbg_ctx_pairwise_serialized(rbg_ctx* ctx, int op, int32_t a, size_t ia, int32_t b, size_t ib) {
   Ctx* c;
-  CHK(session(ctx, &c));
+  CHK(session(ctx, &c, false));
   if (op < 0 || op > 3) return RBG_ERR_ILLEGAL_ARGUMENT;
   CHK(ctx_pairwise(c, op, a, ia, b, ib, false));
   return ctx_serialize(c);
 }
 int rbg_ctx_pairwise_range(rbg_ctx* ctx, int op, int32_t a, size_t ia, int32_t b, size_t ib, int key_lo, int key_hi) {
   Ctx* c;
-  CHK(session(ctx, &c));
+  CHK(session(ctx, &c, false));
   if (key_lo > key_hi) return RBG_ERR_ILLEGAL_ARGUMENT;
   return ctx_pairwise(c, op, a, ia, b, ib, false, key_lo, key_hi);
 }
@@ -725,7 +725,7 @@
     ResultInfo ri = {};
     ri.card32 = (uint32_t)hc;
     ri.long_card = hc;
-    HIPCHK(hipMemcpyAsync(c->info.p, &ri, sizeof(ri), hipMemcpyHostToDevice, c->stream));
+    HIPCHK(hipMemcpyAsync(c->r().info.p, &ri, sizeof(ri), hipMemcpyHostToDevice, c->stream));
     HIPCHK(hipStreamSynchronize(c->stream));
   }
   return RBG_OK;
@@ -764,7 +764,7 @@
 }
 int rbg_ctx_serialize(rbg_ctx* ctx) {
   Ctx* c;
-  CHK(session(ctx, &c));
+  CHK(session(ctx, &c, false));
   return ctx_serialize(c);
 }
 int rbg_ctx_fetch(rbg_ctx* ctx, rbg_buffer* out) {
@@ -776,17 +776,18 @@
   Ctx* c;
   CHK(session(ctx, &c));
   if (!dst3) return RBG_ERR_ILLEGAL_ARGUMENT;
-  if (c->last != 1) {
+  if (c->r().last != 1) {
     set_err("no materialised result pending");
     return RBG_ERR_ILLEGAL_ARGUMENT;
   }
-  if (c->place_pending) {
-    OutCtx o = c->pending;
+  CHK(join_result(c));
+  if (c->r().place_pending) {
+    OutCtx o = c->r().pending;
     o.layout_out = reinterpret_cast<int64_t*>(dst3);
-    launch_place(c->stream, c->ntasks.as<uint32_t>(), o, c->info.as<ResultInfo>());
-    c->place_pending = false;
+    launch_place(c->stream, c->r().ntasks.as<uint32_t>(), o, c->r().info.as<ResultInfo>());
+    c->r().place_pending = false;
   } else {
-    launch_layout_out(c->stream, c->info.as<ResultInfo>(), reinterpret_cast<int64_t*>(dst3));
+    launch_layout_out(c->stream, c->r().info.as<ResultInfo>(), reinterpret_cast<int64_t*>(dst3));
   }
   HIPCHK(hipGetLastError());
   return RBG_OK;
@@ -796,17 +797,18 @@
   CHK(session(ctx, &c));
   if (!layout || !out || world < 1 || world > 1024 || rank < 0 || rank >= world)
     return RBG_ERR_ILLEGAL_ARGUMENT;
-  if (c->last != 1) {
+  if (c->r().last != 1) {
     set_err("no materialised result pending");
     return RBG_ERR_ILLEGAL_ARGUMENT;
   }
+  CHK(join_result(c));
   CHK(ensure_placed(c));
-  if (c->serialized) {
+  if (c->r().serialized) {
     set_err("fetch_shard_device_dyn: the result was already serialized; fetch it before releasing operands "
             "or use rbg_ctx_fetch_shard_device");
     return RBG_ERR_ILLEGAL_ARGUMENT;
   }
-  launch_serialize_shard_dyn(c->stream, grid_for((c->pending_ub + 255) / 256, 256), c->ntasks.as<uint32_t>(), c->pending,
+  launch_serialize_shard_dyn(c->stream, grid_for((c->r().pending_ub + 255) / 256, 256), c->r().ntasks.as<uint32_t>(), c->r().pending,
                              reinterpret_cast<const int64_t*>(layout), rank, world, (uint8_t*)out, (uint8_t*)runb, true);
   HIPCHK(hipGetLastError());
   return RBG_OK;
diff --git a/roaringbitmap_amd/csrc/engine_bsi.cpp b/roaringbitmap_amd/csrc/engine_bsi.cpp
--- a/roaringbitmap_amd/csrc/engine_bsi.cpp
+++ b/roaringbitmap_amd/csrc/engine_bsi.cpp
@@ -798,7 +798,7 @@
   const size_t ub = std::min<size_t>(kMaxKeys, std::max<size_t>(B->n_ctr, 1));
   OutCtx oc;
   CHK(prepare_output(c, ub, kStagedMax * ub + B->max_ser, &oc, op == BSI_SUM_ONLY));
-  c->pending_src = {id};
+  c->r().pending_src = {id};
   const uint32_t need = mode == -1 ? 0xFFFFFFFFu : (op == BSI_SUM_ONLY ? (uint32_t)(nbits + 1) : 0u);
   BsiScratch sc{};
   if (mode >= 0 && mode <= BSI_RANGE) {
@@ -818,8 +818,8 @@
   wa.bm = B->bm.as<uint32_t>();
   wa.payload = B->payload.as<uint8_t>();
   c->mark(0);
-  Task* tasks = c->tasks.as<Task>();
-  uint32_t* nt = c->ntasks.as<uint32_t>();
+  Task* tasks = c->r().tasks.as<Task>();
+  uint32_t* nt = c->r().ntasks.as<uint32_t>();
   if (sc.defer && bsi_reg_path(mode, nbits)) {
     if (!B->bsi_cached) {
       CHK(B->bsi_tasks.ensure(sizeof(Task) * kMaxKeys));
@@ -840,7 +840,7 @@
     sc.ztile = c->ztile;
     sc.zsums = c->bsi_sums.as<unsigned long long>();
     sc.nt_src = nt;
-    sc.nt_dst = c->ntasks.as<uint32_t>();
+    sc.nt_dst = c->r().ntasks.as<uint32_t>();
   } else {
     launch_plan_bsi(s, B->key_off.as<uint32_t>(), B->bm.as<uint32_t>(), need, c->by_key.as<Task>(),
                     c->flag.as<uint8_t>(), c->wg_count.as<uint32_t>(), c->zlb, c->ztile,
@@ -853,7 +853,7 @@
              sc.defer ? &sc : nullptr, want_sum ? c->bsi_sums_dst : nullptr);
   c->mark(2);
   if (op == BSI_SUM_ONLY) {
-    c->last = 0;
+    c->r().last = 0;
   } else {
     defer_place(c);
   }
@@ -959,13 +959,13 @@
   return with_big_runs(c, true, "bsi", [&](const BigRuns& big) -> int {
     OutCtx oc;
     CHK(prepare_output(c, ub, kStagedMax * ub + B->max_ser + big.cap, &oc, false));
-    c->pending_src = {id};
+    c->r().pending_src = {id};
     const uint32_t need = mode == -1 ? 0xFFFFFFFFu : 0xFFFFFFFEu;
     c->mark(0);
     launch_plan_bsi(s, B->key_off.as<uint32_t>(), B->bm.as<uint32_t>(), need, c->by_key.as<Task>(),
                     c->flag.as<uint8_t>(), c->wg_count.as<uint32_t>(), c->zlb, c->ztile, nullptr, nullptr);
-    launch_compact(s, c->flag.as<uint8_t>(), c->by_key.as<Task>(), c->wg_count.as<uint32_t>(), c->tasks.as<Task>(),
-                   c->ntasks.as<uint32_t>());
+    launch_compact(s, c->flag.as<uint8_t>(), c->by_key.as<Task>(), c->wg_count.as<uint32_t>(), c->r().tasks.as<Task>(),
+                   c->r().ntasks.as<uint32_t>());
     c->mark(1);
     WideArgs wa{};
     wa.desc = B->desc.as<CDesc>();
@@ -988,15 +988,15 @@
       CHK(c->owen_keys.ensure(4 * ub));
       p.owen_tb = c->owen_tb.p;
       p.task_keys = c->owen_keys.as<uint32_t>();
-      launch_bsi_owen_pre(s, grid, c->tasks.as<Task>(), c->ntasks.as<uint32_t>(), wa, p);
+      launch_bsi_owen_pre(s, grid, c->r().tasks.as<Task>(), c->r().ntasks.as<uint32_t>(), wa, p);
       HIPCHK(hipGetLastError());
       uint32_t nt = 0;
-      HIPCHK(hipMemcpyAsync(&nt, c->ntasks.p, 4, hipMemcpyDeviceToHost, s));
+      HIPCHK(hipMemcpyAsync(&nt, c->r().ntasks.p, 4, hipMemcpyDeviceToHost, s));
       HIPCHK(hipStreamSynchronize(s));
       CHK(owen_order(c, M, nt));
       p.owen_order = c->owen_ord.as<uint8_t>();
     }
-    if (mode >= 0) launch_bsi_buf(s, grid, c->tasks.as<Task>(), c->ntasks.as<uint32_t>(), wa, p, oc);
+    if (mode >= 0) launch_bsi_buf(s, grid, c->r().tasks.as<Task>(), c->r().ntasks.as<uint32_t>(), wa, p, oc);
     return op_end(c);
   });
 }
diff --git a/roaringbitmap_amd/csrc/engine_synth.cpp b/roaringbitmap_amd/csrc/engine_synth.cpp
--- a/roaringbitmap_amd/csrc/engine_synth.cpp
+++ b/roaringbitmap_amd/csrc/engine_synth.cpp
@@ -98,8 +98,9 @@
   CHK(b.bm_off.ensure(8));
   HIPCHK(hipMemcpyAsync(b.key_off.p, key_off.data(), 4 * (kMaxKeys + 1), hipMemcpyHostToDevice, s));
   if (kind == 1) {
-    CHK(c->scratch.ensure(16 * (size_t)kMaxKeys));
-    unsigned long long* kb = c->scratch.as<unsigned long long>();
+    CHK(main_set(c));
+    CHK(c->r().scratch.ensure(16 * (size_t)kMaxKeys));
+    unsigned long long* kb = c->r().scratch.as<unsigned long long>();
     launch_synth_c3u(s, seed, (uint32_t)n, key_lo, nkeys, kb, nullptr, nullptr, nullptr, nullptr, nullptr, 0);
     std::vector<unsigned long long> bytes(nkeys + 1, 0);
     if (nkeys) HIPCHK(hipMemcpyAsync(bytes.data(), kb, 8 * nkeys, hipMemcpyDeviceToHost, s));
@@ -216,8 +217,9 @@
   const int nkeys = std::max(0, key_hi - key_lo);
   hipStream_t s = c->stream;
   const size_t G = (size_t)nkeys * nin;
-  CHK(c->scratch.ensure(8 * G + 64));
-  uint32_t* cards = c->scratch.as<uint32_t>();
+  CHK(main_set(c));
+  CHK(c->r().scratch.ensure(8 * G + 64));
+  uint32_t* cards = c->r().scratch.as<uint32_t>();
   uint32_t* pos = cards + G;
   unsigned int* mm = reinterpret_cast<unsigned int*>(c->scalar.p);
   const unsigned int mm0[2] = {0xFFFFFFFFu, 0u};
diff --git a/roaringbitmap_amd/csrc/engine_wide.cpp b/roaringbitmap_amd/csrc/engine_wide.cpp
--- a/roaringbitmap_amd/csrc/engine_wide.cpp
+++ b/roaringbitmap_amd/csrc/engine_wide.cpp
@@ -140,23 +140,23 @@
   const size_t ub = std::min<size_t>(kMaxKeys, std::max<size_t>(B->n_ctr, 1));
   OutCtx oc;
   CHK(prepare_output(c, ub, kStagedMax * ub + B->max_ser, &oc, false));
-  c->pending_src = {id};
+  c->r().pending_src = {id};
   c->mark(0);
   launch_plan_wide(s, N ? 0 : 1, B->key_off.as<uint32_t>(), N ? (uint32_t)N : 0xFFFFFFFFu, 0, kMaxKeys,
                    c->by_key.as<Task>(), c->flag.as<uint8_t>(), c->wg_count.as<uint32_t>(), c->zlb, c->ztile);
-  launch_compact(s, c->flag.as<uint8_t>(), c->by_key.as<Task>(), c->wg_count.as<uint32_t>(), c->tasks.as<Task>(),
-                 c->ntasks.as<uint32_t>());
+  launch_compact(s, c->flag.as<uint8_t>(), c->by_key.as<Task>(), c->wg_count.as<uint32_t>(), c->r().tasks.as<Task>(),
+                 c->r().ntasks.as<uint32_t>());
   c->mark(1);
   if (!N) {
     c->mark(2);
-    launch_place(s, c->ntasks.as<uint32_t>(), oc, c->info.as<ResultInfo>());
-    c->last = 1;
+    launch_place(s, c->r().ntasks.as<uint32_t>(), oc, c->r().info.as<ResultInfo>());
+    c->r().last = 1;
     c->mark(3);
     HIPCHK(hipGetLastError());
     return RBG_OK;
   }
   uint32_t h_nt = 0;
-  HIPCHK(hipMemcpyAsync(&h_nt, c->ntasks.p, 4, hipMemcpyDeviceToHost, s));
+  HIPCHK(hipMemcpyAsync(&h_nt, c->r().ntasks.p, 4, hipMemcpyDeviceToHost, s));
   std::vector<unsigned long long> leaf(N);
   DevBuf dsz;
   CHK(dsz.ensure(8 * N));
@@ -170,7 +170,7 @@
   const size_t stride = std::max<uint32_t>(h_nt, 1);
   const size_t st_bytes = n_slots * stride * sizeof(PQState);
   std::vector<Task> h_tasks(h_nt);
-  if (h_nt) HIPCHK(hipMemcpyAsync(h_tasks.data(), c->tasks.p, sizeof(Task) * h_nt, hipMemcpyDeviceToHost, s));
+  if (h_nt) HIPCHK(hipMemcpyAsync(h_tasks.data(), c->r().tasks.p, sizeof(Task) * h_nt, hipMemcpyDeviceToHost, s));
   HIPCHK(hipStreamSynchronize(s));
   std::vector<uint32_t> kbase(stride, 0);
   std::vector<int32_t> ktop(stride, 0);
@@ -258,13 +258,13 @@
   const PQArgs pa{B->desc.as<CDesc>(), B->bm.as<uint32_t>(), B->payload.as<uint8_t>()};
   const int grid = grid_for(h_nt, 65536);
   for (size_t k = 0; k + 1 < N; k++) {
-    launch_pq_step(s, grid, c->tasks.as<Task>(), c->ntasks.as<uint32_t>(), pa, D);
+    launch_pq_step(s, grid, c->r().tasks.as<Task>(), c->r().ntasks.as<uint32_t>(), pa, D);
     if ((k & 1023) == 1023) HIPCHK(hipGetLastError());
   }
   c->mark(2);
-  launch_pq_final(s, grid, c->tasks.as<Task>(), c->ntasks.as<uint32_t>(), pa, op == RBG_WIDE_PQ_OR ? 1 : 0, D, oc);
+  launch_pq_final(s, grid, c->r().tasks.as<Task>(), c->r().ntasks.as<uint32_t>(), pa, op == RBG_WIDE_PQ_OR ? 1 : 0, D, oc);
   HIPCHK(hipGetLastError());
-  launch_place(s, c->ntasks.as<uint32_t>(), oc, c->info.as<ResultInfo>());
+  launch_place(s, c->r().ntasks.as<uint32_t>(), oc, c->r().info.as<ResultInfo>());
   PQCtl done{};
   HIPCHK(hipMemcpyAsync(&done, mb, sizeof(done), hipMemcpyDeviceToHost, s));
   HIPCHK(hipStreamSynchronize(s));
@@ -273,7 +273,7 @@
                      : std::string("priorityqueue: the device queue did not finish"));
     return done.err ? RBG_ERR_OUT_OF_MEMORY : RBG_ERR_DEVICE;
   }
-  c->last = 1;
+  c->r().last = 1;
   c->mark(3);
   HIPCHK(hipGetLastError());
   return RBG_OK;
@@ -333,7 +333,8 @@
       const int64_t cc = N ? B->h_bm_card[0] : 0;
       *host_card_out = (int32_t)(uint32_t)(uint64_t)cc;
       *host_card_valid = true;
-      c->last = 2;
+      CHK(main_set(c));
+      c->r().last = 2;
       return RBG_OK;
     }
     if (op == RBG_WIDE_CARD_AND && N >= 2) {
@@ -397,8 +398,8 @@
     const size_t ub = std::min<size_t>(kMaxKeys, std::max<size_t>(B->n_ctr, 1));
     OutCtx oc;
     CHK(prepare_output(c, ub, kStagedMax * ub + B->max_ser + big.cap, &oc, card_only));
-    if (!card_only && (mode == WIDE_OR || mode == WIDE_LAZY_CHAIN)) oc.spec = c->pending.spec = 1;
-    c->pending_src = {id};
+    if (!card_only && (mode == WIDE_OR || mode == WIDE_LAZY_CHAIN)) oc.spec = c->r().pending.spec = 1;
+    c->r().pending_src = {id};
     if (!skip.empty()) {
       CHK(c->skip.ensure(skip.size()));
       HIPCHK(hipMemcpyAsync(c->skip.p, skip.data(), skip.size(), hipMemcpyHostToDevice, s));
@@ -407,8 +408,8 @@
     c->mark(0);
     launch_plan_wide(s, plan_mode == 0 ? 0 : 1, B->key_off.as<uint32_t>(), n_req, key_lo, key_hi,
                      c->by_key.as<Task>(), c->flag.as<uint8_t>(), c->wg_count.as<uint32_t>(), c->zlb, c->ztile);
-    launch_compact(s, c->flag.as<uint8_t>(), c->by_key.as<Task>(), c->wg_count.as<uint32_t>(), c->tasks.as<Task>(),
-                   c->ntasks.as<uint32_t>());
+    launch_compact(s, c->flag.as<uint8_t>(), c->by_key.as<Task>(), c->wg_count.as<uint32_t>(), c->r().tasks.as<Task>(),
+                   c->r().ntasks.as<uint32_t>());
     WideArgs wa{};
     wa.desc = B->desc.as<CDesc>();
     wa.bm = B->bm.as<uint32_t>();
@@ -423,12 +424,12 @@
     wa.buffer = buffer ? 1u : 0u;
     wa.big = big;
     c->mark(1);
-    launch_wide(s, mode, grid_for(ub, 65536), c->tasks.as<Task>(), c->ntasks.as<uint32_t>(), wa, oc,
-                c->task_card.as<uint32_t>());
+    launch_wide(s, mode, grid_for(ub, 65536), c->r().tasks.as<Task>(), c->r().ntasks.as<uint32_t>(), wa, oc,
+                c->r().task_card.as<uint32_t>());
     c->mark(2);
     if (card_only) {
-      launch_reduce_card(s, c->task_card.as<uint32_t>(), c->ntasks.as<uint32_t>(), c->info.as<ResultInfo>(), oc.err);
-      c->last = 2;
+      launch_reduce_card(s, c->r().task_card.as<uint32_t>(), c->r().ntasks.as<uint32_t>(), c->r().info.as<ResultInfo>(), oc.err);
+      c->r().last = 2;
     } else {
       defer_place(c);
     }
```
